# nrontsis/PILCO

Measured on AMD Instinct MI355X. Metric: moment-matching rollouts/sec (N=1000,D=10,E=10,H=40), higher is better.
Workload: dtype f64; 1 GPU; BASELINE configs[1]: N=1000 D=10 E=10 H=40 full rollout + reward, control_dim=0 (D==E read literally), ExponentialReward(W=I,t=0), factorisation cached (R-fwd); one step = one host-synchronised pilco_rollout call (what PILCO.predict makes) with its result downloaded; parallelism=pairs1, exchange=none (one rank)

## Files before the change

### include/pilco_hip_dev.h

```cpp
#ifndef PILCO_HIP_DEV_H
#define PILCO_HIP_DEV_H
#include "pilco_hip.h"

#ifdef __cplusplus
extern "C" {
#endif

int pilco_set_pair_kernel(pilco_ctx* ctx, int variant);
int pilco_set_fused_step(pilco_ctx* ctx, int on);
int pilco_set_small_step(pilco_ctx* ctx, int on);
int pilco_set_grad_mode(pilco_ctx* ctx, int mode);
int pilco_set_reverse_chain(pilco_ctx* ctx, int on_device);
int pilco_set_use_graph(pilco_ctx* ctx, int on);
int pilco_set_inline_policy(pilco_ctx* ctx, int on);

int pilco_rollout_tape(pilco_ctx* ctx, const pilco_policy* policy, const pilco_reward_term* rewards, int n_rewards,
                       const double* m0, const double* S0, int H, double* mH, double* SH, double* reward, double* traj,
                       double* tape);

int pilco_shard_owner_of_pair(const pilco_ctx* ctx, int pair_index);
int pilco_shard_plan(int E, int D, int nranks, int rank, int* out5);
int pilco_shard_pair_slot(int E, int D, int nranks, int a, int b);
int pilco_shard_output_slot(int E, int D, int nranks, int a);
int pilco_peer_attached(const pilco_ctx* ctx);
int pilco_comm_count(const pilco_ctx* ctx);

int pilco_rollout_timed(pilco_ctx* ctx, const pilco_policy* policy, const pilco_reward_term* rewards, int n_rewards,
                        const double* m0, const double* S0, int H, int reps, double* mH, double* SH, double* reward,
                        float* ms_total, float* ms_pair, int* n_pair_launches);
int pilco_set_pair_timing(pilco_ctx* ctx, int on);
int pilco_get_pair_timing(pilco_ctx* ctx, float* ms_pair, int* n_pair_launches);
int pilco_debug_timestamps(pilco_ctx* ctx, unsigned long long* out32);
int pilco_debug_last_route(const pilco_ctx* ctx, int* out, int n);
#define PILCO_GEOMETRY_WORDS 14
int pilco_debug_geometry(pilco_ctx* ctx, int* out, int n);
int pilco_debug_particle_actions(pilco_ctx* ctx, const pilco_policy* policy, const double* x, int P, double* u);
int pilco_debug_blocks(pilco_ctx* ctx, unsigned long long* out, int n);
int pilco_debug_buffer(pilco_ctx* ctx, int slot, int which, double* out, long n);
int pilco_debug_poison(pilco_ctx* ctx, int slot, int which);
int pilco_debug_sk_boundary(int w, int waves, int nd, int tdiag, int toff, int ud, int uo, int n_pairs);
int pilco_debug_sk_pair_waves(int k, int waves, int nd, int tdiag, int toff, int ud, int uo, int n_pairs, int* out3);
int pilco_factorize_timed(pilco_ctx* ctx, int slot, int reps, float* ms_each);

#ifdef __cplusplus
}
#endif
#endif
```

### pilco_amd/_lib.py

```python
from __future__ import annotations

import ctypes as C
import os

import numpy as np

_HERE = os.path.dirname(os.path.abspath(__file__))
LIB_PATH = os.environ.get("PILCO_LIB", os.path.join(_HERE, "libpilco_hip.so"))

PILCO_OK = 0
STATUS_NAMES = {1: "PILCO_E_SHAPE", 2: "PILCO_E_NOT_PD", 3: "PILCO_E_HIP", 4: "PILCO_E_RCCL",
                5: "PILCO_E_STATE", 6: "PILCO_E_ALLOC"}
SLOT_DYNAMICS, SLOT_POLICY = 0, 1
POLICY_NONE, POLICY_LINEAR, POLICY_RBF = 0, 1, 2
REWARD_EXPONENTIAL, REWARD_LINEAR = 1, 2
MAX_EVENTS, MAX_EVENT_CLAUSES = 8, 4
COMM_ID_BYTES = 128
PEER_HANDLE_BYTES = 64

_dp = C.POINTER(C.c_double)


class PilcoError(RuntimeError):
    def __init__(self, code, msg):
        super().__init__(f"{STATUS_NAMES.get(code, code)}: {msg}")
        self.code = code


class NotPositiveDefiniteError(PilcoError):
    """The reference raises tf.errors.InvalidArgumentError here (tests/test_cascade.py:22)."""


class PolicyStruct(C.Structure):
    _fields_ = [("kind", C.c_int), ("state_dim", C.c_int), ("control_dim", C.c_int),
                ("W", _dp), ("b", _dp), ("max_action", _dp), ("squash", C.c_int)]


class RewardTerm(C.Structure):
    _fields_ = [("kind", C.c_int), ("coef", C.c_double), ("W", _dp), ("t", _dp)]


class EventClause(C.Structure):
    _fields_ = [("dim", C.c_int), ("low", C.c_double), ("high", C.c_double)]


class Event(C.Structure):
    _fields_ = [("n_clauses", C.c_int), ("complement", C.c_int), ("clause", EventClause * MAX_EVENT_CLAUSES)]


def event_spec_of(ev):
    spec = ev.event_spec() if hasattr(ev, "event_spec") else ev
    if not isinstance(spec, dict) or "clauses" not in spec:
        raise TypeError("an event is a dict(clauses=[(dim, low, high), ...], complement=bool) or offers event_spec()")
    return spec


_vp = C.c_void_p
SEED_FN = C.CFUNCTYPE(None, C.c_void_p, C.c_int, C.c_int, C.POINTER(C.c_double), C.POINTER(C.c_double))
SIGNATURES = {
    "pilco_abi_version": (C.c_int, []),
    "pilco_ctx_create": (C.c_int, [C.c_int, C.POINTER(_vp)]),
    "pilco_ctx_destroy": (C.c_int, [_vp]),
    "pilco_last_error": (C.c_char_p, [_vp]),
    "pilco_last_not_pd_output": (C.c_int, [_vp]),
    "pilco_set_pair_kernel": (C.c_int, [_vp, C.c_int]),
    "pilco_set_reverse_chain": (C.c_int, [_vp, C.c_int]),
    "pilco_debug_poison": (C.c_int, [_vp, C.c_int, C.c_int]),
    "pilco_selftest": (C.c_int, [_vp]),
    "pilco_set_fused_step": (C.c_int, [_vp, C.c_int]),
    "pilco_set_grad_mode": (C.c_int, [_vp, C.c_int]),
    "pilco_set_small_step": (C.c_int, [_vp, C.c_int]),
    "pilco_set_use_graph": (C.c_int, [_vp, C.c_int]),
    "pilco_set_inline_policy": (C.c_int, [_vp, C.c_int]),
    "pilco_gp_set_data": (C.c_int, [_vp, C.c_int, _dp, _dp, C.c_int, C.c_int, C.c_int]),
    "pilco_gp_set_hyp": (C.c_int, [_vp, C.c_int, _dp, _dp, _dp]),
    "pilco_gp_set_inducing": (C.c_int, [_vp, C.c_int, _dp, C.c_int]),
    "pilco_gp_gram": (C.c_int, [_vp, C.c_int, _dp, C.c_int, _dp, C.c_int, _dp]),
    "pilco_gp_factorize": (C.c_int, [_vp, C.c_int]),
    "pilco_gp_nlml": (C.c_int, [_vp, C.c_int, _dp, _dp]),
    "pilco_gp_fitc_nlml": (C.c_int, [_vp, C.c_int, _dp, C.c_int, _dp, _dp, _dp]),
    "pilco_gp_num_points": (C.c_int, [_vp, C.c_int]),
    "pilco_gp_get_factors": (C.c_int, [_vp, C.c_int, _dp, _dp]),
    "pilco_gp_set_factors": (C.c_int, [_vp, C.c_int, _dp, _dp]),
    "pilco_gp_predict": (C.c_int, [_vp, C.c_int, _dp, _dp, _dp, _dp, _dp]),
    "pilco_gp_predict_points": (C.c_int, [_vp, C.c_int, _dp, C.c_int, C.c_int, _dp, _dp, _dp]),
    "pilco_gp_predict_points_jac": (C.c_int, [_vp, C.c_int, _dp, C.c_int, C.c_int, _dp, _dp, _dp, _dp, _dp]),
    "pilco_rollout": (C.c_int, [_vp, C.POINTER(PolicyStruct), C.POINTER(RewardTerm), C.c_int, _dp, _dp, C.c_int,
                                _dp, _dp, _dp, _dp]),
    "pilco_rollout_particles": (C.c_int, [_vp, C.POINTER(PolicyStruct), C.POINTER(RewardTerm), C.c_int, _dp, C.c_int, C.c_int,
                                          _dp, C.c_ulonglong, C.c_int, _dp, _dp, _dp, _dp, _dp]),
    "pilco_rollout_particles_events": (C.c_int, [_vp, C.POINTER(PolicyStruct), C.POINTER(RewardTerm), C.c_int, _dp, C.c_int, C.c_int,
                                                 _dp, C.c_ulonglong, C.c_int, _dp, _dp, _dp, _dp, _dp,
                                                 C.POINTER(Event), C.c_int, C.POINTER(C.c_longlong), C.POINTER(C.c_int)]),
    "pilco_gp_predict_vjp": (C.c_int, [_vp, C.c_int, _dp, _dp, _dp, _dp, _dp, _dp, _dp]),
    "pilco_rollout_tape": (C.c_int, [_vp, C.POINTER(PolicyStruct), C.POINTER(RewardTerm), C.c_int, _dp, _dp, C.c_int,
                                     _dp, _dp, _dp, _dp, _dp]),
    "pilco_rollout_grad": (C.c_int, [_vp, C.POINTER(PolicyStruct), C.POINTER(RewardTerm), C.c_int, _dp, _dp, C.c_int,
                                     _dp, _dp, _dp]),
    "pilco_rollout_grad_rbf": (C.c_int, [_vp, C.POINTER(PolicyStruct), C.POINTER(RewardTerm), C.c_int, _dp, _dp, C.c_int,
                                         _dp, _dp, _dp, _dp, C.c_int, _dp, _dp, _dp, _dp]),
    "pilco_rollout_grad_seeded": (C.c_int, [_vp, C.POINTER(PolicyStruct), C.POINTER(RewardTerm), C.c_int, _dp, _dp, C.c_int,
                                            SEED_FN, _vp, _dp, _dp, _dp]),
    "pilco_rollout_grad_rbf_seeded": (C.c_int, [_vp, C.POINTER(PolicyStruct), C.POINTER(RewardTerm), C.c_int, _dp, _dp, C.c_int,
                                                _dp, _dp, _dp, _dp, C.c_int, SEED_FN, _vp, _dp, _dp, _dp, _dp]),
    "pilco_propagate": (C.c_int, [_vp, C.POINTER(PolicyStruct), _dp, _dp, _dp, _dp]),
    "pilco_rollout_batch": (C.c_int, [_vp, C.c_int, C.POINTER(PolicyStruct), C.POINTER(RewardTerm), C.c_int, _dp, _dp, C.c_int, _dp, _dp, _dp]),
    "pilco_rollout_grad_batch": (C.c_int, [_vp, C.c_int, C.POINTER(PolicyStruct), C.POINTER(RewardTerm), C.c_int, _dp, _dp, C.c_int, _dp, _dp, _dp]),
    "pilco_rollout_grad_rbf_batch": (C.c_int, [_vp, C.c_int, C.POINTER(PolicyStruct), C.POINTER(RewardTerm), C.c_int, _dp, _dp, C.c_int,
                                               _dp, _dp, _dp, _dp, C.c_int, _dp, _dp, _dp, _dp]),
    "pilco_rollout_grad_batch_seeded": (C.c_int, [_vp, C.c_int, C.POINTER(PolicyStruct), C.POINTER(RewardTerm), C.c_int, _dp, _dp, C.c_int,
                                                  SEED_FN, C.POINTER(C.c_void_p), _dp, _dp, _dp]),
    "pilco_rollout_grad_rbf_batch_seeded": (C.c_int, [_vp, C.c_int, C.POINTER(PolicyStruct), C.POINTER(RewardTerm), C.c_int, _dp, _dp, C.c_int,
                                                      _dp, _dp, _dp, _dp, C.c_int, SEED_FN, C.POINTER(C.c_void_p), _dp, _dp, _dp, _dp]),
    "pilco_policy_action": (C.c_int, [_vp, C.POINTER(PolicyStruct), _dp, _dp, _dp, _dp, _dp]),
    "pilco_reward_eval": (C.c_int, [_vp, C.POINTER(RewardTerm), C.c_int, C.c_int, _dp, _dp, _dp, _dp]),
    "pilco_rollout_timed": (C.c_int, [_vp, C.POINTER(PolicyStruct), C.POINTER(RewardTerm), C.c_int, _dp, _dp,
                                      C.c_int, C.c_int, _dp, _dp, _dp, C.POINTER(C.c_float),
                                      C.POINTER(C.c_float), C.POINTER(C.c_int)]),
    "pilco_factorize_timed": (C.c_int, [_vp, C.c_int, C.c_int, C.POINTER(C.c_float)]),
    "pilco_set_pair_timing": (C.c_int, [_vp, C.c_int]),
    "pilco_get_pair_timing": (C.c_int, [_vp, C.POINTER(C.c_float), C.POINTER(C.c_int)]),
    "pilco_debug_timestamps": (C.c_int, [_vp, C.POINTER(C.c_ulonglong)]),
    "pilco_debug_blocks": (C.c_int, [_vp, C.POINTER(C.c_ulonglong), C.c_int]),
    "pilco_debug_last_route": (C.c_int, [_vp, C.POINTER(C.c_int), C.c_int]),
    "pilco_debug_geometry": (C.c_int, [_vp, C.POINTER(C.c_int), C.c_int]),
    "pilco_debug_particle_actions": (C.c_int, [_vp, C.POINTER(PolicyStruct), _dp, C.c_int, _dp]),
    "pilco_debug_buffer": (C.c_int, [_vp, C.c_int, C.c_int, _dp, C.c_long]),
    "pilco_debug_sk_boundary": (C.c_int, [C.c_int] * 8),
    "pilco_debug_sk_pair_waves": (C.c_int, [C.c_int] * 8 + [C.POINTER(C.c_int)]),
    "pilco_comm_unique_id": (C.c_int, [_vp]),
    "pilco_comm_init": (C.c_int, [_vp, _vp, C.c_int, C.c_int]),
    "pilco_shard_set": (C.c_int, [_vp, C.c_int, C.c_int]),
    "pilco_peer_export": (C.c_int, [_vp, _vp]),
    "pilco_peer_attach": (C.c_int, [_vp, _vp, C.c_int]),
    "pilco_group_peer_attach": (C.c_int, [_vp, C.c_int]),
    "pilco_peer_detach": (C.c_int, [_vp]),
    "pilco_peer_attached": (C.c_int, [_vp]),
    "pilco_shard_owner_of_pair": (C.c_int, [_vp, C.c_int]),
    "pilco_shard_plan": (C.c_int, [C.c_int, C.c_int, C.c_int, C.c_int, C.POINTER(C.c_int)]),
    "pilco_shard_pair_slot": (C.c_int, [C.c_int, C.c_int, C.c_int, C.c_int, C.c_int]),
    "pilco_shard_output_slot": (C.c_int, [C.c_int, C.c_int, C.c_int, C.c_int]),
    "pilco_gp_shard_pack": (C.c_int, [_vp, C.c_int, _dp, _dp, _dp]),
    "pilco_gp_shard_finish": (C.c_int, [_vp, C.c_int, _dp, _dp, _dp, _dp]),
    "pilco_rollout_grad_group": (C.c_int, [C.POINTER(_vp), C.c_int, C.POINTER(PolicyStruct), C.POINTER(RewardTerm), C.c_int, _dp, _dp, C.c_int, _dp, _dp, _dp]),
    "pilco_rollout_grad_rbf_group": (C.c_int, [C.POINTER(_vp), C.c_int, C.POINTER(PolicyStruct), C.POINTER(RewardTerm), C.c_int, _dp, _dp, C.c_int,
                                               _dp, _dp, _dp, _dp, C.c_int, _dp, _dp, _dp, _dp]),
    "pilco_rollout_group": (C.c_int, [C.POINTER(_vp), C.c_int, C.POINTER(PolicyStruct), C.POINTER(RewardTerm), C.c_int, _dp, _dp,
                            C.c_int, _dp, _dp, _dp, _dp, C.POINTER(C.c_int)]),
    "pilco_group_sync_model": (C.c_int, [C.POINTER(_vp), C.c_int, C.c_int]),
    "pilco_gp_beta_rows": (C.c_int, [_vp, C.c_int, C.POINTER(C.c_int), C.POINTER(C.c_int)]),
    "pilco_gp_beta_export": (C.c_int, [_vp, C.c_int, _dp]),
    "pilco_gp_beta_import": (C.c_int, [_vp, C.c_int, _dp]),
    "pilco_comm_rank": (C.c_int, [_vp]),
    "pilco_comm_size": (C.c_int, [_vp]),
    "pilco_comm_count": (C.c_int, [_vp]),
}

_lib = None


def load_library():
    global _lib
    if _lib is not None:
        return _lib
    if not os.path.exists(LIB_PATH):
        raise RuntimeError(
            f"{LIB_PATH} is missing: build the HIP extension first "
            "(python -c 'import __graft_entry__ as g; g.build()' or make -C pilco_amd/csrc). "
            "pilco_amd has no CPU fallback.")
    lib = C.CDLL(LIB_PATH)
    for name, (res, args) in SIGNATURES.items():
        fn = getattr(lib, name)
        fn.restype = res
        fn.argtypes = args
    _lib = lib
    return lib


def _f64(a, shape=None):
    a = np.ascontiguousarray(np.asarray(a, dtype=np.float64))
    if shape is not None:
        a = a.reshape(shape)
    return a


def _ptr(a):
    return a.ctypes.data_as(_dp) if a is not None else None


class Context:

    def __init__(self, device=None):
        self.lib = load_library()
        if device is None:
            device = int(os.environ.get("PILCO_DEVICE", os.environ.get("LOCAL_RANK", "0")))
        h = _vp()
        rc = self.lib.pilco_ctx_create(int(device), C.byref(h))
        if rc != PILCO_OK or not h:
            raise PilcoError(rc, f"cannot create a HIP context on device {device} "
                                 "(no MI355X visible?). pilco_amd has no CPU fallback.")
        self.h = h
        self.device = int(device)
        self._keep = []
        self._slot_owner = {}
        self._settings = {}
        self.nranks, self.has_comm = 1, False

    def close(self):
        if getattr(self, "h", None):
            self.lib.pilco_ctx_destroy(self.h)
            self.h = None

    def __del__(self):
        try:
            self.close()
        except Exception:
            pass

    def _chk(self, rc):
        if rc != PILCO_OK:
            msg = self.lib.pilco_last_error(self.h).decode("utf-8", "replace")
            if rc == 2:
                exc = NotPositiveDefiniteError(rc, msg)
                exc.output = int(self.lib.pilco_last_not_pd_output(self.h))
                raise exc
            raise PilcoError(rc, msg)

    def selftest(self):
        self._chk(self.lib.pilco_selftest(self.h))

    def set_fused_step(self, on):
        self._chk(self.lib.pilco_set_fused_step(self.h, 1 if on else 0))
        self._settings["set_fused_step"] = (on,)

    def set_small_step(self, on):
        self._chk(self.lib.pilco_set_small_step(self.h, 1 if on else 0))
        self._settings["set_small_step"] = (on,)

    def set_grad_mode(self, mode):
        self._chk(self.lib.pilco_set_grad_mode(self.h, int(mode)))
        self._settings["set_grad_mode"] = (mode,)

    def use_graph(self, on):
        self._chk(self.lib.pilco_set_use_graph(self.h, 1 if on else 0))
        self._settings["use_graph"] = (on,)

    def set_inline_policy(self, on):
        self._chk(self.lib.pilco_set_inline_policy(self.h, 1 if on else 0))
        self._settings["set_inline_policy"] = (on,)

    def debug_poison(self, slot, which):
        self._chk(self.lib.pilco_debug_poison(self.h, int(slot), int(which)))

    def set_reverse_chain(self, on_device):
        self._chk(self.lib.pilco_set_reverse_chain(self.h, int(bool(on_device))))
        self._settings["set_reverse_chain"] = (on_device,)

    def set_pair_kernel(self, variant):
        self._chk(self.lib.pilco_set_pair_kernel(self.h, int(variant)))
        self._settings["set_pair_kernel"] = (variant,)

    def gp_set_data(self, slot, X, Y, owner=None):
        self._slot_owner[slot] = owner
        X = _f64(X)
        Y = _f64(Y)
        if X.ndim != 2 or Y.ndim != 2 or X.shape[0] != Y.shape[0]:
            raise ValueError("data must be (X (N,D), Y (N,E))")
        self._chk(self.lib.pilco_gp_set_data(self.h, slot, _ptr(X), _ptr(Y), X.shape[0], X.shape[1], Y.shape[1]))

    def gp_set_hyp(self, slot, lengthscales, variance, noise, owner=None):
        self._slot_owner[slot] = owner
        ls, var, nz = _f64(lengthscales), _f64(variance).reshape(-1), _f64(noise).reshape(-1)
        self._chk(self.lib.pilco_gp_set_hyp(self.h, slot, _ptr(ls), _ptr(var), _ptr(nz)))

    def gp_set_inducing(self, slot, Z, owner=None):
        self._slot_owner[slot] = owner
        if Z is None:
            self._chk(self.lib.pilco_gp_set_inducing(self.h, slot, None, 0))
        else:
            Z = _f64(Z)
            self._chk(self.lib.pilco_gp_set_inducing(self.h, slot, _ptr(Z), Z.shape[0]))

    def gp_gram(self, slot, X1, X2, E):
        X1 = _f64(X1)
        X2a = None if X2 is None else _f64(X2)
        n2 = X1.shape[0] if X2a is None else X2a.shape[0]
        out = np.empty((E, X1.shape[0], n2))
        self._chk(self.lib.pilco_gp_gram(self.h, slot, _ptr(X1), X1.shape[0], _ptr(X2a), n2, _ptr(out)))
        return out

    def gp_factorize(self, slot):
        self._chk(self.lib.pilco_gp_factorize(self.h, slot))

    def gp_nlml(self, slot, D, E, want_grad=True):
        nlml = np.empty(E)
        grad = np.empty((E, D + 2)) if want_grad else None
        self._chk(self.lib.pilco_gp_nlml(self.h, slot, _ptr(nlml), _ptr(grad)))
        return nlml, grad

    def gp_fitc_nlml(self, slot, Z_all, D, E, want_grad=True):
        Z_all = _f64(Z_all)
        M = Z_all.shape[1]
        Z_all = _f64(Z_all, (E, M, D))
        nlml = np.empty(E)
        gh = np.empty((E, D + 2)) if want_grad else None
        gz = np.empty((E, M, D)) if want_grad else None
        self._chk(self.lib.pilco_gp_fitc_nlml(self.h, slot, _ptr(Z_all), M, _ptr(nlml), _ptr(gh), _ptr(gz)))
        return nlml, gh, gz

    def gp_num_points(self, slot):
        return self.lib.pilco_gp_num_points(self.h, slot)

    def gp_get_factors(self, slot, E, want_iK=True):
        n = self.gp_num_points(slot)
        iK = np.empty((E, n, n)) if want_iK else None
        beta = np.empty((E, n))
        self._chk(self.lib.pilco_gp_get_factors(self.h, slot, _ptr(iK), _ptr(beta)))
        return iK, beta

    def gp_set_factors(self, slot, iK, beta, owner=None):
        self._slot_owner[slot] = owner
        iKa = None if iK is None else _f64(iK)
        beta = _f64(beta)
        self._chk(self.lib.pilco_gp_set_factors(self.h, slot, _ptr(iKa), _ptr(beta)))

    def gp_predict(self, slot, m, s, D, E):
        m = _f64(m, (D,))
        s = _f64(s, (D, D))
        M = np.empty((1, E))
        S = np.empty((E, E))
        V = np.empty((D, E))
        self._chk(self.lib.pilco_gp_predict(self.h, slot, _ptr(m), _ptr(s), _ptr(M), _ptr(S), _ptr(V)))
        return M, S, V

    def gp_predict_points(self, slot, Xs, D, E, output=-1, Z_all=None):
        Xs = _f64(Xs)
        if Xs.ndim != 2 or Xs.shape[1] != D:
            raise ValueError(f"test inputs must be (Nt, {D})")
        Nt = Xs.shape[0]
        Za = None
        if Z_all is not None:
            Za = _f64(Z_all)
            Za = _f64(Za, (E, Za.shape[-2], D))
        rows = E if output < 0 else 1
        mean = np.empty((rows, Nt))
        var = np.empty((rows, Nt))
        self._chk(self.lib.pilco_gp_predict_points(self.h, slot, _ptr(Xs), Nt, int(output), _ptr(Za), _ptr(mean), _ptr(var)))
        return mean, var

    def gp_predict_points_jac(self, slot, Xs, D, E, output=-1, Z_all=None):
        Xs = _f64(Xs)
        if Xs.ndim != 2 or Xs.shape[1] != D:
            raise ValueError(f"test inputs must be (Nt, {D})")
        Nt = Xs.shape[0]
        Za = None
        if Z_all is not None:
            Za = _f64(Z_all)
            Za = _f64(Za, (E, Za.shape[-2], D))
        rows = E if output < 0 else 1
        mean, var = np.empty((rows, Nt)), np.empty((rows, Nt))
        dmean, dvar = np.empty((rows, Nt, D)), np.empty((rows, Nt, D))
        self._chk(self.lib.pilco_gp_predict_points_jac(self.h, slot, _ptr(Xs), Nt, int(output), _ptr(Za), _ptr(mean), _ptr(var),
                                                       _ptr(dmean), _ptr(dvar)))
        return mean, var, dmean, dvar

    def _policy(self, spec):
        keep = []
        p = PolicyStruct()
        p.kind = spec["kind"]
        p.state_dim = spec["state_dim"]
        p.control_dim = spec["control_dim"]
        p.squash = 1 if spec.get("squash", True) else 0
        U, E = p.control_dim, p.state_dim
        if spec["kind"] == POLICY_LINEAR:
            W = _f64(spec["W"], (U, E))
            b = _f64(spec["b"], (U,))
            keep += [W, b]
            p.W, p.b = _ptr(W), _ptr(b)
        ma = spec.get("max_action", None)
        if ma is not None and U > 0:
            ma = _f64(np.broadcast_to(np.asarray(ma, np.float64).reshape(-1) if np.ndim(ma) else np.float64(ma), (U,)))
            keep.append(ma)
            p.max_action = _ptr(ma)
        return p, keep

    def _rewards(self, terms, E):
        arr = (RewardTerm * max(len(terms), 1))()
        keep = []
        for i, t in enumerate(terms):
            arr[i].kind = t["kind"]
            arr[i].coef = float(t.get("coef", 1.0))
            if t["kind"] == REWARD_EXPONENTIAL:
                W = _f64(t["W"], (E, E))
                tg = _f64(t["t"], (E,)) if t.get("t") is not None else None
                keep += [W, tg]
                arr[i].W, arr[i].t = _ptr(W), _ptr(tg)
            else:
                W = _f64(t["W"], (E,))
                keep.append(W)
                arr[i].W = _ptr(W)
        return arr, keep

    def rollout(self, policy, rewards, m0, S0, H, want_traj=False):
        E = policy["state_dim"]
        p, k1 = self._policy(policy)
        r, k2 = self._rewards(rewards, E)
        m0 = _f64(m0, (E,))
        S0 = _f64(S0, (E, E))
        mH = np.empty((1, E))
        SH = np.empty((E, E))
        rew = np.zeros((1, 1))
        traj = np.empty((H + 1, E + E * E)) if want_traj else None
        self._chk(self.lib.pilco_rollout(self.h, C.byref(p), r, len(rewards), _ptr(m0), _ptr(S0), int(H),
                                         _ptr(mH), _ptr(SH), _ptr(rew), _ptr(traj)))
        if want_traj:
            return mH, SH, rew, traj
        return mH, SH, rew

    @staticmethod
    def _events(events):
        arr = (Event * max(len(events), 1))()
        for k, ev in enumerate(events):
            spec = event_spec_of(ev)
            clauses = list(spec["clauses"])
            if len(clauses) > MAX_EVENT_CLAUSES:
                raise ValueError(f"an event has at most {MAX_EVENT_CLAUSES} clauses")
            arr[k].n_clauses = len(clauses)
            arr[k].complement = 1 if spec.get("complement", False) else 0
            for j, (dim, low, high) in enumerate(clauses):
                arr[k].clause[j].dim = int(dim)
                arr[k].clause[j].low = -np.inf if low is None else float(low)
                arr[k].clause[j].high = np.inf if high is None else float(high)
        return arr

    def rollout_particles(self, policy, rewards, x0, H, eps=None, seed=0, observation_noise=False, want_particles=False,
                          events=None):
        E = policy["state_dim"]
        p, k1 = self._policy(policy)
        r, k2 = self._rewards(rewards, E)
        x0 = _f64(x0)
        if x0.ndim != 2 or x0.shape[1] != E:
            raise ValueError(f"initial particles must be (P, {E})")
        P, H = x0.shape[0], int(H)
        if eps is not None:
            eps = _f64(eps)
            if eps.shape != (H, P, E):
                raise ValueError(f"draws must be ({H}, {P}, {E})")
        mean = np.empty((H + 1, E))
        cov = np.empty((H + 1, E, E))
        rew = np.empty((max(H, 0),))
        parts = np.empty((H + 1, P, E)) if want_particles else None
        used = np.empty((H, P, E))
        args = (self.h, C.byref(p), r, len(rewards), _ptr(x0), P, H, _ptr(eps), C.c_ulonglong(int(seed) & 0xFFFFFFFFFFFFFFFF),
                1 if observation_noise else 0, _ptr(mean), _ptr(cov), _ptr(rew), _ptr(parts), _ptr(used))
        if events is None:
            self._chk(self.lib.pilco_rollout_particles(*args))
            return mean, cov, rew, parts, used
        events = list(events)
        K = len(events)
        ev = self._events(events)
        counts = np.zeros((H + 1, K), np.int64)
        first = np.full((P, K), -1, np.int32)
        self._chk(self.lib.pilco_rollout_particles_events(*args, ev, K, counts.ctypes.data_as(C.POINTER(C.c_longlong)),
                                                          first.ctypes.data_as(C.POINTER(C.c_int))))
        return mean, cov, rew, parts, used, counts, first

    def particle_actions(self, policy, x):
        E, U = policy["state_dim"], policy["control_dim"]
        p, k1 = self._policy(policy)
        x = _f64(x).reshape(-1, E)
        u = np.empty((x.shape[0], U))
        self._chk(self.lib.pilco_debug_particle_actions(self.h, C.byref(p), _ptr(x), x.shape[0], _ptr(u)))
        return u

    def rollout_batch(self, policies, rewards, m0, S0, H):
        B = len(policies)
        E = policies[0]["state_dim"]
        arr, keep = self._policy_array(policies)
        r, k2 = self._rewards(rewards, E)
        m0 = _f64(m0, (B, E))
        S0 = _f64(S0, (B, E, E))
        mH = np.empty((B, E))
        SH = np.empty((B, E, E))
        rew = np.zeros(B)
        self._chk(self.lib.pilco_rollout_batch(self.h, B, arr, r, len(rewards), _ptr(m0), _ptr(S0), int(H), _ptr(mH), _ptr(SH), _ptr(rew)))
        return mH, SH, rew

    def _policy_array(self, policies):
        arr = (PolicyStruct * len(policies))()
        keep = []
        for i, spec in enumerate(policies):
            p, k = self._policy(spec)
            keep.append((p, k))
            arr[i] = p
        return arr, keep

    @staticmethod
    def _lane_seed_callback(seed_fns, errors):
        def cb(user, H, E, traj_p, seeds_p):
            n = (H + 1) * (E + E * E)
            out = np.ctypeslib.as_array(seeds_p, shape=(n,))
            try:
                traj = np.ctypeslib.as_array(traj_p, shape=(n,)).reshape(H + 1, E + E * E).copy()
                out[:] = np.asarray(seed_fns[int(user) - 1](traj), dtype=np.float64).reshape(n)
            except BaseException as exc:
                errors.append(exc)
                out[:] = np.nan
        return SEED_FN(cb)

    lane_seeds = True

    def rollout_grad_batch(self, policies, rewards, m0, S0, H, seed_fns=None):
        B = len(policies)
        E, U = policies[0]["state_dim"], policies[0]["control_dim"]
        arr, keep = self._policy_array(policies)
        r, k2 = self._rewards(rewards, E)
        m0 = _f64(m0, (B, E)); S0 = _f64(S0, (B, E, E))
        rew = np.zeros(B); dW = np.empty((B, U, E)); db = np.empty((B, U))
        if seed_fns is None:
            self._chk(self.lib.pilco_rollout_grad_batch(self.h, B, arr, r, len(rewards), _ptr(m0), _ptr(S0), int(H), _ptr(rew), _ptr(dW), _ptr(db)))
            return rew, dW, db
        errors = []
        cb = self._lane_seed_callback(seed_fns, errors)
        users = (C.c_void_p * B)(*[i + 1 for i in range(B)])
        rc = self.lib.pilco_rollout_grad_batch_seeded(self.h, B, arr, r, len(rewards), _ptr(m0), _ptr(S0), int(H), cb, users,
                                                      _ptr(rew), _ptr(dW), _ptr(db))
        if errors:
            raise errors[0]
        self._chk(rc)
        return rew, dW, db

    def rollout_grad_rbf_batch(self, policies, rewards, m0, S0, H, Xp, Yp, lsp, noisep, seed_fns=None):
        B = len(policies)
        E, U = policies[0]["state_dim"], policies[0]["control_dim"]
        arr, keep = self._policy_array(policies)
        r, k2 = self._rewards(rewards, E)
        m0 = _f64(m0, (B, E)); S0 = _f64(S0, (B, E, E))
        Xp = _f64(Xp); bf = Xp.shape[1]
        Xp = _f64(Xp, (B, bf, E)); Yp = _f64(Yp, (B, bf, U)); lsp = _f64(lsp, (B, U, E)); noisep = _f64(noisep, (B, U))
        rew = np.zeros(B); dX = np.empty((B, bf, E)); dY = np.empty((B, bf, U)); dls = np.empty((B, U, E))
        self._slot_owner[SLOT_POLICY] = None
        if seed_fns is None:
            self._chk(self.lib.pilco_rollout_grad_rbf_batch(self.h, B, arr, r, len(rewards), _ptr(m0), _ptr(S0), int(H), _ptr(Xp), _ptr(Yp),
                                                            _ptr(lsp), _ptr(noisep), bf, _ptr(rew), _ptr(dX), _ptr(dY), _ptr(dls)))
            return rew, dX, dY, dls
        errors = []
        cb = self._lane_seed_callback(seed_fns, errors)
        users = (C.c_void_p * B)(*[i + 1 for i in range(B)])
        rc = self.lib.pilco_rollout_grad_rbf_batch_seeded(self.h, B, arr, r, len(rewards), _ptr(m0), _ptr(S0), int(H), _ptr(Xp), _ptr(Yp),
                                                          _ptr(lsp), _ptr(noisep), bf, cb, users, _ptr(rew), _ptr(dX), _ptr(dY), _ptr(dls))
        if errors:
            raise errors[0]
        self._chk(rc)
        return rew, dX, dY, dls

    def gp_predict_vjp(self, slot, m, s, Mbar, Sbar, Vbar, D, E):
        m = _f64(m, (D,)); s = _f64(s, (D, D))
        Mb = _f64(Mbar, (E,)); Sb = _f64(Sbar, (E, E)); Vb = _f64(Vbar, (D, E))
        mbar = np.empty((1, D)); sbar = np.empty((D, D))
        self._chk(self.lib.pilco_gp_predict_vjp(self.h, slot, _ptr(m), _ptr(s), _ptr(Mb), _ptr(Sb), _ptr(Vb), _ptr(mbar), _ptr(sbar)))
        return mbar, sbar

    def rollout_tape(self, policy, rewards, m0, S0, H):
        E = policy["state_dim"]; D = E + policy["control_dim"]
        p, k1 = self._policy(policy)
        r, k2 = self._rewards(rewards, E)
        m0 = _f64(m0, (E,)); S0 = _f64(S0, (E, E))
        mH = np.empty((1, E)); SH = np.empty((E, E)); rew = np.zeros((1, 1))
        traj = np.empty((H + 1, E + E * E))
        TS = D + D * D + E * D + E + E * E + D * E
        tape = np.zeros((max(H, 1), TS))
        self._chk(self.lib.pilco_rollout_tape(self.h, C.byref(p), r, len(rewards), _ptr(m0), _ptr(S0), int(H),
                                              _ptr(mH), _ptr(SH), _ptr(rew), _ptr(traj), _ptr(tape)))
        return mH, SH, rew, traj, tape[:H]

    @staticmethod
    def _seed_callback(seed_fn, errors):
        def cb(_user, H, E, traj_p, seeds_p):
            n = (H + 1) * (E + E * E)
            out = np.ctypeslib.as_array(seeds_p, shape=(n,))
            try:
                traj = np.ctypeslib.as_array(traj_p, shape=(n,)).reshape(H + 1, E + E * E).copy()
                out[:] = np.asarray(seed_fn(traj), dtype=np.float64).reshape(n)
            except BaseException as exc:
                errors.append(exc)
                out[:] = np.nan
        return SEED_FN(cb)

    def rollout_grad(self, policy, rewards, m0, S0, H, seed_fn=None):
        E = policy["state_dim"]; U = policy["control_dim"]
        p, k1 = self._policy(policy)
        r, k2 = self._rewards(rewards, E)
        m0 = _f64(m0, (E,)); S0 = _f64(S0, (E, E))
        rew = np.zeros((1, 1)); dW = np.empty((U, E)); db = np.empty((U,))
        errors = []
        cb = self._seed_callback(seed_fn, errors) if seed_fn is not None else SEED_FN()
        rc = self.lib.pilco_rollout_grad_seeded(self.h, C.byref(p), r, len(rewards), _ptr(m0), _ptr(S0), int(H), cb, None,
                                                _ptr(rew), _ptr(dW), _ptr(db))
        if errors:
            raise errors[0]
        self._chk(rc)
        return float(rew[0, 0]), dW, db

    def rollout_grad_rbf(self, policy, rewards, m0, S0, H, Xp, Yp, lsp, noisep, seed_fn=None):
        E = policy["state_dim"]; U = policy["control_dim"]
        p, k1 = self._policy(policy)
        r, k2 = self._rewards(rewards, E)
        m0 = _f64(m0, (E,)); S0 = _f64(S0, (E, E))
        Xp = _f64(Xp); bf = Xp.shape[0]
        Xp = _f64(Xp, (bf, E)); Yp = _f64(Yp, (bf, U)); lsp = _f64(lsp, (U, E)); noisep = _f64(noisep, (U,))
        rew = np.zeros((1, 1)); dX = np.empty((bf, E)); dY = np.empty((bf, U)); dls = np.empty((U, E))
        errors = []
        cb = self._seed_callback(seed_fn, errors) if seed_fn is not None else SEED_FN()
        rc = self.lib.pilco_rollout_grad_rbf_seeded(self.h, C.byref(p), r, len(rewards), _ptr(m0), _ptr(S0), int(H),
                                                    _ptr(Xp), _ptr(Yp), _ptr(lsp), _ptr(noisep), bf, cb, None,
                                                    _ptr(rew), _ptr(dX), _ptr(dY), _ptr(dls))
        if errors:
            raise errors[0]
        self._chk(rc)
        return float(rew[0, 0]), dX, dY, dls

    def propagate(self, policy, m_x, s_x):
        E = policy["state_dim"]
        p, k1 = self._policy(policy)
        m_x = _f64(m_x, (E,))
        s_x = _f64(s_x, (E, E))
        M = np.empty((1, E))
        S = np.empty((E, E))
        self._chk(self.lib.pilco_propagate(self.h, C.byref(p), _ptr(m_x), _ptr(s_x), _ptr(M), _ptr(S)))
        return M, S

    def policy_action(self, policy, m, s):
        E, U = policy["state_dim"], policy["control_dim"]
        p, k1 = self._policy(policy)
        m = _f64(m, (E,))
        s = _f64(s, (E, E))
        M = np.empty((1, U))
        S = np.empty((U, U))
        V = np.empty((E, U))
        self._chk(self.lib.pilco_policy_action(self.h, C.byref(p), _ptr(m), _ptr(s), _ptr(M), _ptr(S), _ptr(V)))
        return M, S, V

    def reward_eval(self, rewards, E, m, s):
        r, k2 = self._rewards(rewards, E)
        m = _f64(m, (E,))
        s = _f64(s, (E, E))
        mu = C.c_double()
        var = C.c_double()
        self._chk(self.lib.pilco_reward_eval(self.h, r, len(rewards), E, _ptr(m), _ptr(s), C.byref(mu), C.byref(var)))
        return np.array([[mu.value]]), np.array([[var.value]])

    def rollout_timed(self, policy, rewards, m0, S0, H, reps, time_pair=True):
        E = policy["state_dim"]
        p, k1 = self._policy(policy)
        r, k2 = self._rewards(rewards, E)
        m0 = _f64(m0, (E,))
        S0 = _f64(S0, (E, E))
        mH = np.empty((1, E))
        SH = np.empty((E, E))
        rew = np.zeros((1, 1))
        ms_total = C.c_float()
        ms_pair = C.c_float()
        npair = C.c_int()
        self._chk(self.lib.pilco_rollout_timed(self.h, C.byref(p), r, len(rewards), _ptr(m0), _ptr(S0), int(H),
                                               int(reps), _ptr(mH), _ptr(SH), _ptr(rew), C.byref(ms_total),
                                               C.byref(ms_pair) if time_pair else None, C.byref(npair)))
        return dict(mH=mH, SH=SH, reward=rew, ms_total=ms_total.value, ms_pair=ms_pair.value,
                    n_pair_launches=npair.value)

    def factorize_timed(self, slot, reps):
        ms = C.c_float()
        self._chk(self.lib.pilco_factorize_timed(self.h, slot, int(reps), C.byref(ms)))
        return ms.value

    def set_pair_timing(self, on=True):
        self._chk(self.lib.pilco_set_pair_timing(self.h, 1 if on else 0))

    def get_pair_timing(self):
        ms = C.c_float()
        n = C.c_int()
        self._chk(self.lib.pilco_get_pair_timing(self.h, C.byref(ms), C.byref(n)))
        return ms.value, n.value

    def debug_buffer(self, slot, which, n):
        out = np.empty(int(n))
        self._chk(self.lib.pilco_debug_buffer(self.h, int(slot), int(which), _ptr(out), int(n)))
        return out

    def debug_timestamps(self, read=True):
        buf = (C.c_ulonglong * 64)()
        self._chk(self.lib.pilco_debug_timestamps(self.h, buf if read else None))
        return list(buf)

    ROUTE_FIELDS = ("entry", "step", "policy", "DT", "KP", "vsep", "pair", "tape", "H", "npad", "chain", "rev_lds", "exchange")

    def last_route(self):
        buf = (C.c_int * len(self.ROUTE_FIELDS))()
        self._chk(self.lib.pilco_debug_last_route(self.h, buf, len(buf)))
        return {name: int(buf[i]) for i, name in enumerate(self.ROUTE_FIELDS)}

    GEOMETRY_FIELDS = ("npad", "PL", "EL", "NCH", "NCHM", "NT", "sk_waves", "sk_total", "sk_nd", "sk_maxw", "sk_capacity", "cus",
                       "NCS_reward", "NCS_no_reward")

    def geometry(self):
        buf = (C.c_int * len(self.GEOMETRY_FIELDS))()
        self._chk(self.lib.pilco_debug_geometry(self.h, buf, len(buf)))
        return {name: int(buf[i]) for i, name in enumerate(self.GEOMETRY_FIELDS)}

    def debug_blocks(self, n):
        buf = (C.c_ulonglong * n)()
        self._chk(self.lib.pilco_debug_blocks(self.h, buf, n))
        return list(buf)

    def comm_unique_id(self):
        buf = C.create_string_buffer(COMM_ID_BYTES)
        rc = self.lib.pilco_comm_unique_id(buf)
        if rc != PILCO_OK:
            raise PilcoError(rc, "ncclGetUniqueId failed")
        return bytes(buf.raw)

    def comm_init(self, id_bytes, rank, nranks):
        buf = C.create_string_buffer(bytes(id_bytes), COMM_ID_BYTES)
        self._chk(self.lib.pilco_comm_init(self.h, buf, int(rank), int(nranks)))
        self.nranks, self.has_comm = int(nranks), True

    def shard_pack(self, slot, m, s, D, E, nranks, rank):
        plan = shard_plan(E, D, nranks, rank)
        m = _f64(m, (D,))
        s = _f64(s, (D, D))
        seg = np.zeros(plan["SEG"])
        self._chk(self.lib.pilco_gp_shard_pack(self.h, slot, _ptr(m), _ptr(s), _ptr(seg)))
        return seg

    def shard_finish(self, slot, gathered, D, E):
        g = _f64(gathered).reshape(-1)
        M = np.empty((1, E))
        S = np.empty((E, E))
        V = np.empty((D, E))
        self._chk(self.lib.pilco_gp_shard_finish(self.h, slot, _ptr(g), _ptr(M), _ptr(S), _ptr(V)))
        return M, S, V

    def shard_set(self, rank, nranks):
        self._chk(self.lib.pilco_shard_set(self.h, int(rank), int(nranks)))
        self.nranks = int(nranks)

    def beta_export(self, slot=0):
        el, npad = C.c_int(0), C.c_int(0)
        self._chk(self.lib.pilco_gp_beta_rows(self.h, slot, C.byref(el), C.byref(npad)))
        rows = np.zeros((el.value, npad.value))
        self._chk(self.lib.pilco_gp_beta_export(self.h, slot, _ptr(rows)))
        return rows

    def beta_import(self, all_rows, slot=0):
        all_rows = np.ascontiguousarray(all_rows, dtype=np.float64)
        self._chk(self.lib.pilco_gp_beta_import(self.h, slot, _ptr(all_rows)))

    def peer_export(self):
        buf = C.create_string_buffer(PEER_HANDLE_BYTES)
        self._chk(self.lib.pilco_peer_export(self.h, buf))
        return bytes(buf.raw)

    def peer_attach(self, handles, share_gpu=False):
        blob = b"".join(bytes(h) for h in handles)
        buf = C.create_string_buffer(blob, len(blob))
        self._chk(self.lib.pilco_peer_attach(self.h, buf, 1 if share_gpu else 0))

    def comm_count(self):
        return int(self.lib.pilco_comm_count(self.h))

    def peer_detach(self):
        self._chk(self.lib.pilco_peer_detach(self.h))

    def peer_attached(self):
        return bool(self.lib.pilco_peer_attached(self.h))


def rollout_grad_group(ctxs, policy, rewards, m0, S0, H):
    c0 = ctxs[0]
    n = len(ctxs)
    E, U = policy["state_dim"], policy["control_dim"]
    p, k1 = c0._policy(policy)
    r, k2 = c0._rewards(rewards, E)
    m0 = _f64(m0, (E,)); S0 = _f64(S0, (E, E))
    arr = (_vp * n)(*[c.h for c in ctxs])
    rew, dW, db = np.zeros(n), np.empty((n, U, E)), np.empty((n, U))
    c0._chk(c0.lib.pilco_rollout_grad_group(arr, n, C.byref(p), r, len(rewards), _ptr(m0), _ptr(S0), int(H), _ptr(rew), _ptr(dW), _ptr(db)))
    return rew, dW, db


def rollout_grad_rbf_group(ctxs, policy, rewards, m0, S0, H, Xp, Yp, lsp, noisep):
    c0 = ctxs[0]
    n = len(ctxs)
    E, U = policy["state_dim"], policy["control_dim"]
    p, k1 = c0._policy(policy)
    r, k2 = c0._rewards(rewards, E)
    m0 = _f64(m0, (E,)); S0 = _f64(S0, (E, E))
    Xp = _f64(Xp); bf = Xp.shape[0]
    Xp = _f64(Xp, (bf, E)); Yp = _f64(Yp, (bf, U)); lsp = _f64(lsp, (U, E)); noisep = _f64(noisep, (U,))
    arr = (_vp * n)(*[c.h for c in ctxs])
    rew, dX, dY, dls = np.zeros(n), np.empty((n, bf, E)), np.empty((n, bf, U)), np.empty((n, U, E))
    c0._chk(c0.lib.pilco_rollout_grad_rbf_group(arr, n, C.byref(p), r, len(rewards), _ptr(m0), _ptr(S0), int(H), _ptr(Xp), _ptr(Yp), _ptr(lsp),
                                                _ptr(noisep), bf, _ptr(rew), _ptr(dX), _ptr(dY), _ptr(dls)))
    return rew, dX, dY, dls


def group_nlml(ctxs, slot, D, E):
    nlml, grad = np.full(E, np.nan), np.full((E, D + 2), np.nan)
    for c in ctxs:
        n, g = c.gp_nlml(slot, D, E)
        own = ~np.isnan(n)
        assert not np.any(own & ~np.isnan(nlml)), "two ranks claim the same output"
        nlml[own], grad[own] = n[own], g[own]
    return nlml, grad


def group_fitc_nlml(ctxs, slot, Z_all, D, E):
    Z_all = np.asarray(Z_all, np.float64)
    nlml, gh, gz = np.full(E, np.nan), np.full((E, D + 2), np.nan), np.full(Z_all.shape, np.nan)
    for c in ctxs:
        n, h, z = c.gp_fitc_nlml(slot, Z_all, D, E)
        own = ~np.isnan(n)
        assert not np.any(own & ~np.isnan(nlml)), "two ranks claim the same output"
        nlml[own], gh[own], gz[own] = n[own], h[own], z[own]
    return nlml, gh, gz


def group_sync_model(ctxs, slot=0):
    arr = (_vp * len(ctxs))(*[c.h for c in ctxs])
    ctxs[0]._chk(ctxs[0].lib.pilco_group_sync_model(arr, len(ctxs), int(slot)))


def group_peer_attach(ctxs):
    arr = (_vp * len(ctxs))(*[c.h for c in ctxs])
    ctxs[0]._chk(ctxs[0].lib.pilco_group_peer_attach(arr, len(ctxs)))


def rollout_group(ctxs, policy, rewards, m0, S0, H, want_traj=False):
    c0 = ctxs[0]
    E = policy["state_dim"]
    p, k1 = c0._policy(policy)
    r, k2 = c0._rewards(rewards, E)
    m0 = _f64(m0, (E,))
    S0 = _f64(S0, (E, E))
    mH, SH, rew = np.empty((1, E)), np.empty((E, E)), np.zeros((1, 1))
    traj = np.empty((H + 1, E + E * E)) if want_traj else None
    arr = (_vp * len(ctxs))(*[c.h for c in ctxs])
    mm = C.c_int(0)
    c0._chk(c0.lib.pilco_rollout_group(arr, len(ctxs), C.byref(p), r, len(rewards), _ptr(m0), _ptr(S0), int(H), _ptr(mH), _ptr(SH),
                                       _ptr(rew), _ptr(traj), C.byref(mm)))
    return (mH, SH, rew, traj, mm.value) if want_traj else (mH, SH, rew, mm.value)


def shard_plan(E, D, nranks, rank):
    lib = load_library()
    out = (C.c_int * 5)()
    rc = lib.pilco_shard_plan(int(E), int(D), int(nranks), int(rank), out)
    if rc != PILCO_OK:
        raise PilcoError(rc, "bad shard plan arguments")
    return dict(PL=out[0], EL=out[1], SEG=out[2], OUTOFF=out[3], P=out[4])


def shard_pair_slot(E, D, nranks, a, b):
    return load_library().pilco_shard_pair_slot(int(E), int(D), int(nranks), int(a), int(b))


def shard_output_slot(E, D, nranks, a):
    return load_library().pilco_shard_output_slot(int(E), int(D), int(nranks), int(a))


_default_ctx = None


def get_context():
    global _default_ctx
    if _default_ctx is None:
        _default_ctx = Context()
    return _default_ctx


def set_context(ctx):
    global _default_ctx
    _default_ctx = ctx
    _ctx_pool[:] = []


_ctx_pool = []


def resolve_ctx(obj):
    ref = getattr(obj, "_ctx_owner", None)
    owner = ref() if ref is not None else None
    return owner.ctx if owner is not None else get_context()


def context_adopted(ctx, owner):
    import weakref
    for ent in _ctx_pool:
        if ent[0] is ctx and (ent[1] is None or ent[1]() is None):
            ent[1] = weakref.ref(owner)


def context_for(owner):
    import weakref
    d = get_context()
    if os.environ.get("PILCO_CTX_POOL", "1") == "0":
        return d
    if getattr(d, "nranks", 1) != 1 or getattr(d, "has_comm", False):
        return d
    if not _ctx_pool or _ctx_pool[0][0] is not d:
        _ctx_pool[:] = [[d, None]]
    for ent in _ctx_pool:
        holder = ent[1]() if ent[1] is not None else None
        if holder is None or holder is owner:
            ent[1] = weakref.ref(owner)
            return ent[0]
    try:
        c = type(d)(device=getattr(d, "device", None))
    except TypeError:
        c = type(d)()
    for name, arg in getattr(d, "_settings", {}).items():
        getattr(c, name)(*arg)
    _ctx_pool.append([c, weakref.ref(owner)])
    return c
```

### pilco_amd/csrc/api.hip

```cpp
#include "ctx.h"

int fail(pilco_ctx* c, int code, const std::string& msg) {
    if (c) c->err = msg;
    return code;
}

int check_slot(pilco_ctx* ctx, int slot) {
    if (!ctx) return PILCO_E_SHAPE;
    if (slot < 0 || slot > 1) return fail(ctx, PILCO_E_SHAPE, "slot must be 0 (dynamics) or 1 (policy)");
    return PILCO_OK;
}

std::vector<int> deal_pairs(int E, int nranks) {
    const int P = E * (E + 1) / 2;
    std::vector<int> owner(P, 0);
    int k = 0;
    for (int a = 0; a < E; ++a) owner[a * (a + 1) / 2 + a] = (k++) % nranks;
    for (int a = 0; a < E; ++a)
        for (int b = 0; b < a; ++b) owner[a * (a + 1) / 2 + b] = (k++) % nranks;
    return owner;
}

int build_work(pilco_ctx* ctx, Slot& s) {
    if (s.wk_valid && s.wk_variant == ctx->variant) return PILCO_OK;
    const int E = s.E, D = s.D, npad = s.npad;
    const int P = E * (E + 1) / 2;
    const int W = ctx->nranks, rank = ctx->rank;
    s.pair_owner = deal_pairs(E, W);
    const int PLcap = (P + W - 1) / W, ELcap = (E + W - 1) / W;
    MMWork& wk = s.wk;
    wk.PL = (rank < P) ? (P - rank + W - 1) / W : 0;
    wk.EL = (rank < E) ? (E - rank + W - 1) / W : 0;
    wk.P = P;
    wk.KP = mm_kp(D);
    wk.vsep = mm_vsep(D) ? 1 : 0;
    mm_prep_chunks(npad, std::max(wk.PL, 1), wk.EL, &wk.NCH, &wk.NCHM);
    if (W > 1) {
        int nch_g;
        mm_prep_chunks(npad, P, E, &nch_g, &wk.NCHM);
        wk.NCHM = std::min(wk.NCHM, wk.NCH);
    }
    wk.NT = mm_pair_nt(npad, ctx->variant, std::max(wk.PL, 1));
    wk.OUTOFF = PLcap;
    wk.SEG = PLcap + ELcap * (1 + D);
    wk.rank = rank;
    wk.nranks = W;
#ifdef PILCO_DEV
    wk.abl = getenv("PILCO_ABL") ? atoi(getenv("PILCO_ABL")) : 0;
#else
    wk.abl = 0;
#endif
    const int PLa = std::max(wk.PL, 1);
    wk.sk_waves = 0;
    wk.sk_maxw = 0;
    wk.sk_pls = 0;
    if (ctx->variant == 0 && wk.PL > 0) {
        int tdiag, toff;
        mm_pair_sk_steps(npad, &tdiag, &toff);
        int nd = 0;
        const bool no_iK = s.iK_null || s.ignore_iK;
        if (!no_iK)
            for (int pl = 0; pl < wk.PL; ++pl)
                if (pl * W + rank < E) ++nd;
        if (no_iK) tdiag = toff;
        const long T = (long)nd * tdiag + (long)(wk.PL - nd) * toff;
        auto cut = [&](int cap) { return (long)cap > T ? (int)std::max<long>(4, (T + 3) / 4 * 4) : cap; };
        int waves = cut(mm_pair_sk_capacity(wk.KP, wk.vsep != 0, true));
        int ud = 5, uo = 4;
        if (const char* env = getenv("PILCO_SK_UNITS")) {
            int a = 0, b = 0;
            if (sscanf(env, "%d,%d", &a, &b) == 2 && a > 0 && b > 0) { ud = a; uo = b; }
        }
        if (mm_sk_max_pairs(waves, nd, tdiag, toff, wk.PL, ud, uo) > 2) {
            waves = cut(mm_pair_sk_capacity(wk.KP, wk.vsep != 0, false));
            ud = 5;
            uo = 4;
            if (mm_sk_max_pairs(waves, nd, tdiag, toff, wk.PL, ud, uo) > 2) waves = (int)std::max<long>(4, (T + 3) / 4 * 4);
        }
        wk.sk_waves = waves;
        wk.sk_total = (int)T;
        wk.sk_nd = nd;
        wk.sk_tdiag = tdiag;
        wk.sk_toff = toff;
        wk.sk_ud = ud;
        wk.sk_uo = uo;
        wk.sk_maxw = mm_sk_maxw(wk);
        wk.sk_pls = round_up(wk.PL, 16);
    }
    ENSURE(s.w_in, (size_t)D + D * D + E + E * E + D * E);
    const size_t wt_blocks = npad <= 256 ? (size_t)std::max(E, PLa) : (size_t)E;
    ENSURE(s.w_At, (size_t)PLa * wk.KP * npad);
    ENSURE(s.w_Wt, (wt_blocks * wk.KP + PLa) * npad);
    const size_t n_small = (size_t)PLa + (size_t)E * wk.NCHM * (1 + D);
    ENSURE(s.w_small, 2 * n_small);
    ENSURE(s.w_part, std::max((size_t)PLa * wk.NT * 2, (size_t)std::max(wk.sk_pls, 16) * std::max(wk.sk_maxw, 4)));
    ENSURE(s.w_fpart, (size_t)2 * PLa * wk.NCH * 4 * 2);
    wk.fuse_pair = 0;
    wk.wt_R = wt_rows_per_pair_of(E, D, wk.PL);
    wk.wt_deal = (wk.wt_R <= mm_prep_dt(D) && npad / wk.NCH <= 256) ? 1 : 0;
    wk.NCS = 1;
    wk.share_cu = 0;
    ENSURE(s.w_gath, (size_t)W * wk.SEG);
    ENSURE(s.w_out, (size_t)E + E * E + D * E);
    wk.in_m = s.w_in.p;
    wk.in_s = s.w_in.p + D;
    wk.At = s.w_At.p;
    wk.Wt = s.w_Wt.p;
    wk.vcol = wk.Wt + wt_blocks * wk.KP * npad;
    HIPCHK(hipMemsetAsync(wk.At, 0, sizeof(double) * (size_t)PLa * wk.KP * npad, ctx->st));
    HIPCHK(hipMemsetAsync(wk.Wt, 0, sizeof(double) * (wt_blocks * wk.KP + PLa) * npad, ctx->st));
    launch_const_rows(ctx->st, wk.vsep ? nullptr : wk.At + (size_t)(D + 1) * npad, PLa, wk.Wt + (size_t)D * npad, (int)wt_blocks, (long)wk.KP * npad, npad,
                      s.n);
    wk.pair_isdet = s.w_small.p;
    wk.mean_part = wk.pair_isdet + PLa;
    s.alt_isdet = s.w_small.p + n_small;
    s.alt_mean = s.alt_isdet + PLa;
    wk.pair_part = s.w_part.p;
    wk.sk_part = s.w_part.p;
    wk.gath = s.w_gath.p;
    wk.out_M = s.w_out.p;
    wk.out_S = wk.out_M + E;
    wk.out_V = wk.out_S + E * E;
    wk.exp_tab = ctx->exp_tab.p;
    wk.dbg = ctx->dbg;
    HIPCHK(hipMemsetAsync(s.w_gath.p, 0, sizeof(double) * W * wk.SEG, ctx->st));
    if (wk.sk_waves > 0) HIPCHK(hipMemsetAsync(s.w_part.p, 0, sizeof(double) * wk.sk_pls * wk.sk_maxw, ctx->st));
    s.wk_valid = true;
    s.wk_variant = ctx->variant;
    return PILCO_OK;
}

MMModel model_of(const Slot& s) {
    MMModel md{};
    md.Pt = s.M > 0 ? s.Zt.p : s.Xt.p;
    md.ls = s.ls.p;
    md.var = s.var.p;
    md.lvar = s.var.p + s.E;
    md.beta = s.beta.p;
    md.iK = (s.iK_null || s.ignore_iK) ? nullptr : s.iK.p;
    md.bW = s.shW > 0 ? s.shW : 1;
    md.bEL = s.shW > 1 ? s.shEL : s.E;
    md.n = s.n;
    md.npad = s.npad;
    md.D = s.D;
    md.E = s.E;
    return md;
}

static int group_exchange(pilco_ctx* ctx, Slot& s) {
    PeerGroup& grp = *ctx->group;
    const int slot_idx = (int)(&s - &ctx->slot[0]);
    HIPCHK(hipStreamSynchronize(ctx->st));
    if (!grp.arrive_and_wait()) return fail(ctx, PILCO_E_STATE, "group exchange: another member failed");
    const size_t seg = (size_t)s.wk.SEG;
    for (int j = 0; j < (int)grp.ctxs.size(); ++j) {
        if (j == ctx->rank) continue;
        const double* src = grp.ctxs[j]->slot[slot_idx].wk.gath + (size_t)j * seg;
        HIPCHK(hipMemcpyAsync(s.wk.gath + (size_t)j * seg, src, sizeof(double) * seg, hipMemcpyDefault, ctx->st));
    }
    HIPCHK(hipStreamSynchronize(ctx->st));
    if (!grp.arrive_and_wait()) return fail(ctx, PILCO_E_STATE, "group exchange: another member failed");
    return PILCO_OK;
}

int all_gather_segments(pilco_ctx* ctx, Slot& s) {
    if (ctx->nranks == 1 && !ctx->comm) return PILCO_OK;
    if (ctx->group) return group_exchange(ctx, s);
    if (!ctx->comm) return fail(ctx, PILCO_E_STATE, "sharded context without communicator: use pilco_gp_shard_pack / pilco_gp_shard_finish");
    double* base = s.wk.gath;
    ncclResult_t r = ncclAllGather(base + (size_t)ctx->rank * s.wk.SEG, base, s.wk.SEG, ncclDouble, ctx->comm, ctx->st);
    if (r != ncclSuccess) return fail(ctx, PILCO_E_RCCL, std::string("ncclAllGather: ") + ncclGetErrorString(r));
    return PILCO_OK;
}

int prepare_own(pilco_ctx* ctx, Slot& s, OwnView& o) {
    o.W = ctx->nranks;
    o.rank = ctx->rank;
    if (&s == &ctx->slot[PILCO_SLOT_POLICY]) {
        o.W = 1;
        o.rank = 0;
    }
    const int E = s.E, D = s.D, Np = s.Npad;
    o.ELcap = (E + o.W - 1) / o.W;
    o.EL = (o.rank < E) ? (E - o.rank + o.W - 1) / o.W : 0;
    if (o.W == 1) {
        o.ls = s.ls.p; o.var = s.var.p; o.noise = s.noise.p; o.Yt = s.Yt.p;
        return PILCO_OK;
    }
    const int ELa = std::max(o.EL, 1);
    ENSURE(s.own, (size_t)ELa * (D + 2) + (size_t)ELa * Np);
    double* pls = s.own.p;
    double* pvar = pls + (size_t)ELa * D;
    double* pnz = pvar + ELa;
    double* pY = pnz + ELa;
    if (o.EL > 0) {
        hipStream_t st = ctx->st;
        HIPCHK(hipMemcpy2DAsync(pls, sizeof(double) * D, s.ls.p + (size_t)o.rank * D, sizeof(double) * D * o.W, sizeof(double) * D, o.EL, hipMemcpyDeviceToDevice, st));
        HIPCHK(hipMemcpy2DAsync(pvar, sizeof(double), s.var.p + o.rank, sizeof(double) * o.W, sizeof(double), o.EL, hipMemcpyDeviceToDevice, st));
        HIPCHK(hipMemcpy2DAsync(pnz, sizeof(double), s.noise.p + o.rank, sizeof(double) * o.W, sizeof(double), o.EL, hipMemcpyDeviceToDevice, st));
        HIPCHK(hipMemcpy2DAsync(pY, sizeof(double) * Np, s.Yt.p + (size_t)o.rank * Np, sizeof(double) * Np * o.W, sizeof(double) * Np, o.EL, hipMemcpyDeviceToDevice, st));
    }
    o.ls = pls; o.var = pvar; o.noise = pnz; o.Yt = pY;
    return PILCO_OK;
}

static int gather_beta(pilco_ctx* ctx, Slot& s, const OwnView& o, int npad) {
    s.shW = o.W; s.shEL = o.ELcap; s.shOwn = o.EL; s.shRank = o.rank;
    s.beta_complete = true;
    if (o.W == 1) return PILCO_OK;
    if (ctx->comm) {
        const size_t blk = (size_t)o.ELcap * npad;
        ncclResult_t r = ncclAllGather(s.beta.p + (size_t)o.rank * blk, s.beta.p, blk, ncclDouble, ctx->comm, ctx->st);
        if (r != ncclSuccess) return fail(ctx, PILCO_E_RCCL, std::string("ncclAllGather(beta): ") + ncclGetErrorString(r));
        HIPCHK(hipStreamSynchronize(ctx->st));
        return PILCO_OK;
    }
    s.beta_complete = false;
    return PILCO_OK;
}

int agree_not_pd(pilco_ctx* ctx, int W, int bad, int* agreed) {
    *agreed = bad;
    if (W <= 1 || !ctx->comm) return PILCO_OK;
    int* d = ctx->d_info + 64;
    const int mine = bad + 1;
    HIPCHK(hipMemcpyAsync(d, &mine, sizeof(int), hipMemcpyHostToDevice, ctx->st));
    ncclResult_t r = ncclAllReduce(d, d + 1, 1, ncclInt, ncclMax, ctx->comm, ctx->st);
    if (r != ncclSuccess) return fail(ctx, PILCO_E_RCCL, std::string("ncclAllReduce(not positive definite): ") + ncclGetErrorString(r));
    int all = 0;
    HIPCHK(hipMemcpyAsync(&all, d + 1, sizeof(int), hipMemcpyDeviceToHost, ctx->st));
    HIPCHK(hipStreamSynchronize(ctx->st));
    *agreed = all - 1;
    return PILCO_OK;
}

int factorize_exact(pilco_ctx* ctx, Slot& s) {
    OwnView o{};
    if (int r = prepare_own(ctx, s, o)) return r;
    const int EL = o.EL, ELa = std::max(EL, 1), npad = s.Npad;
    const size_t mat = (size_t)npad * npad;
    ENSURE(s.K, ELa * mat);
    ENSURE(s.Linv, ELa * mat);
    ENSURE(s.iK, ELa * mat);
    ENSURE(s.beta, (size_t)o.W * o.ELcap * npad);
    ENSURE(s.vec, (size_t)ELa * npad);
    hipStream_t st = ctx->st;
    double* beta_own = s.beta.p + (size_t)o.rank * o.ELcap * npad;
    const std::vector<unsigned long long> key = {(unsigned long long)(uintptr_t)s.K.p, (unsigned long long)(uintptr_t)s.Linv.p,
        (unsigned long long)(uintptr_t)s.iK.p, (unsigned long long)(uintptr_t)s.beta.p,
        (unsigned long long)(uintptr_t)s.vec.p, (unsigned long long)(uintptr_t)s.Xt.p, (unsigned long long)(uintptr_t)o.ls,
        (unsigned long long)(uintptr_t)o.var, (unsigned long long)(uintptr_t)o.noise, (unsigned long long)(uintptr_t)o.Yt,
        (unsigned long long)(uintptr_t)ctx->d_info, (unsigned long long)npad, (unsigned long long)s.N, (unsigned long long)s.D,
        (unsigned long long)EL, (unsigned long long)o.W, (unsigned long long)o.rank, (unsigned long long)o.ELcap};
    auto chain = [&]() -> int {
    HIPCHK(hipMemsetAsync(ctx->d_info, 0, sizeof(int) * 64, st));
    if (o.W > 1) HIPCHK(hipMemsetAsync(s.beta.p, 0, sizeof(double) * (size_t)o.W * o.ELcap * npad, st));
    if (EL > 0) {
        launch_gram(st, s.Xt.p, npad, s.N, s.Xt.p, npad, s.N, s.D, o.ls, o.var, EL, s.K.p, npad, npad, 1, o.noise, 0.0);
        launch_potrf(st, s.K.p, npad, EL, s.Linv.p, ctx->d_info, false);
        launch_trtri(st, s.K.p, npad, EL, s.Linv.p, s.iK.p, (long)mat);
        GemmDesc g{};
        g.A = s.Linv.p; g.lda = npad; g.sA = (long)mat;
        g.B = s.Linv.p; g.ldb = npad; g.sB = (long)mat;
        g.C = s.iK.p; g.ldc = npad; g.sC = (long)mat;
        g.M = npad; g.N = npad; g.K = npad; g.alpha = 1.0; g.beta = 0.0; g.k_mode = 1;
        g.tile_mode = 2;
        launch_gemm(st, g, true, false, EL);
        launch_clear_padding(st, s.iK.p, npad, s.N, EL);
        launch_matvec(st, s.Linv.p, npad, EL, o.Yt, s.vec.p, false);
        launch_matvec(st, s.Linv.p, npad, EL, s.vec.p, beta_own, true);
    }
    return PILCO_OK;
    };
    if (int r = run_chain_graph(ctx, s.g_fact, key, chain)) return r;
    int info[64];
    HIPCHK(hipMemcpyAsync(info, ctx->d_info, sizeof(int) * std::min(ELa, 64), hipMemcpyDeviceToHost, st));
    HIPCHK(hipStreamSynchronize(st));
    int bad = -1, pivot = 0, agreed = -1;
    for (int al = 0; al < std::min(EL, 64) && bad < 0; ++al)
        if (info[al] != 0) bad = al * o.W + o.rank, pivot = info[al];
    if (int r = agree_not_pd(ctx, o.W, bad, &agreed)) return r;
    if (agreed >= 0) {
        ctx->not_pd = agreed;
        return fail(ctx, PILCO_E_NOT_PD, "Cholesky failed: K + noise*I of output " + std::to_string(agreed) + " is not positive definite" +
                                             (agreed == bad ? " (pivot " + std::to_string(pivot) + ")" : std::string(" (on another rank)")));
    }
    s.n = s.N;
    s.npad = npad;
    s.iK_null = false;
    return gather_beta(ctx, s, o, npad);
}


extern "C" {

int pilco_abi_version(void) { return PILCO_HIP_ABI_VERSION; }

int pilco_ctx_create(int device, pilco_ctx** out) {
    if (!out) return PILCO_E_SHAPE;
    *out = nullptr;
    int count = 0;
    if (hipGetDeviceCount(&count) != hipSuccess || count <= 0) return PILCO_E_HIP;
    if (device < 0 || device >= count) return PILCO_E_SHAPE;
    if (hipSetDevice(device) != hipSuccess) return PILCO_E_HIP;
    pilco_ctx* ctx = new pilco_ctx();
    ctx->device = device;
    ctx->slot[PILCO_SLOT_POLICY].ignore_iK = true;
    if (hipStreamCreateWithFlags(&ctx->st, hipStreamNonBlocking) != hipSuccess ||
        hipMalloc(&ctx->d_info, 72 * sizeof(int)) != hipSuccess || hipEventCreate(&ctx->ev0) != hipSuccess ||
        hipEventCreate(&ctx->ev1) != hipSuccess) {
        delete ctx;
        return PILCO_E_HIP;
    }
    {
        const int tn = mm_exp_table_size();
        std::vector<double> tab(tn);
        mm_exp_table_fill(tab.data());
        if (ctx->exp_tab.ensure(tn) != hipSuccess ||
            hipMemcpy(ctx->exp_tab.p, tab.data(), sizeof(double) * tn, hipMemcpyHostToDevice) != hipSuccess) {
            delete ctx;
            return PILCO_E_HIP;
        }
    }
    if (const char* eg = getenv("PILCO_NO_GRAPH")) ctx->use_graph = (atoi(eg) == 0);
    if (const char* ei = getenv("PILCO_INLINE_POLICY")) ctx->inline_policy = (atoi(ei) != 0);
    if (const char* ef = getenv("PILCO_FUSED")) ctx->fused = (atoi(ef) != 0);
    if (const char* ef = getenv("PILCO_SMALL_STEP")) ctx->fuse_small = (atoi(ef) != 0);
    if (const char* ef = getenv("PILCO_HOST_CHAIN")) ctx->dev_chain = (atoi(ef) == 0);
    if (const char* env = getenv("PILCO_PAIR_KERNEL")) {
        ctx->variant = (atoi(env) >= 0 && atoi(env) <= 2) ? atoi(env) : 0;
#ifndef PILCO_DEV
        if (ctx->variant == 1) ctx->variant = 0;
#endif
        ctx->variant_user = true;
    }
    *out = ctx;
    return PILCO_OK;
}

int pilco_ctx_destroy(pilco_ctx* ctx) {
    if (!ctx) return PILCO_OK;
    for (pilco_ctx* lane : ctx->lanes) (void)pilco_ctx_destroy(lane);
    ctx->lanes.clear();
    (void)hipSetDevice(ctx->device);
    (void)hipStreamSynchronize(ctx->st);
    (void)peer_detach(ctx);
    for (auto& ge : ctx->graph_cache) (void)hipGraphExecDestroy(ge.second);
    for (Slot& sl : ctx->slot)
        for (ChainGraph* cg : {&sl.g_fact, &sl.g_fitc, &sl.g_fitc_nlml}) chain_graph_release(*cg);
    if (ctx->comm) ncclCommDestroy(ctx->comm);
    for (Slot& s : ctx->slot) {
        predict_release(s);
        for (DevBuf* b : {&s.Xt, &s.Yt, &s.Zt, &s.ls, &s.var, &s.noise, &s.K, &s.Linv, &s.iK, &s.beta, &s.Tscr, &s.ksplit_ws,
                          &s.vec, &s.Kmn, &s.V2, &s.bwd_mom, &s.bwd_cp, &s.bwd_part, &s.bwd_out, &s.bwd_cnt, &s.jac_rowmom, &s.jac_cpart, &s.jac_head, &s.jac_part, &s.jac_np, &s.own, &s.Am, &s.AmInv, &s.iAt, &s.G, &s.w_in, &s.w_At, &s.w_Wt, &s.w_small, &s.w_fpart,
                          &s.w_part, &s.w_gath, &s.w_out, &s.ft_P, &s.ft_T3, &s.ft_Z})
            b->release();
    }
    ctx->state.release();
    ctx->params.release();
    ctx->traj.release();
    ctx->tape.release();
    ctx->jrec.release();
    ctx->jgath.release();
    ctx->revloc.release();
    ctx->revseeds.release();
    ctx->revmat.release();
    ctx->selftest.release();
    ctx->exp_tab.release();
    for (hipEvent_t e : ctx->pair_events) (void)hipEventDestroy(e);
    if (ctx->ev0) (void)hipEventDestroy(ctx->ev0);
    if (ctx->ev1) (void)hipEventDestroy(ctx->ev1);
    if (ctx->d_info) (void)hipFree(ctx->d_info);
    if (ctx->pin) (void)hipHostFree(ctx->pin);
    if (ctx->pin_io) (void)hipHostFree(ctx->pin_io);
    if (ctx->jpin) (void)hipHostFree(ctx->jpin);
    for (hipEvent_t e : ctx->jwait_ev)
        if (e) (void)hipEventDestroy(e);
    if (ctx->st) (void)hipStreamDestroy(ctx->st);
    delete ctx;
    return PILCO_OK;
}

const char* pilco_last_error(const pilco_ctx* ctx) { return ctx ? ctx->err.c_str() : "null context"; }
int pilco_last_not_pd_output(const pilco_ctx* ctx) { return ctx ? ctx->not_pd : -1; }

int pilco_set_pair_kernel(pilco_ctx* ctx, int variant) {
    if (!ctx || variant < 0 || variant > 2) return PILCO_E_SHAPE;
#ifndef PILCO_DEV
// ... 610 lines not shown
```

### pilco_amd/csrc/ctx.h

```cpp
#pragma once
#include <rccl/rccl.h>

#include <algorithm>
#include <array>
#include <chrono>
#include <condition_variable>
#include <memory>
#include <mutex>
#include <cmath>
#include <cstdint>

#include "grad_layout.h"
#include "moment.h"

using namespace pilco;

struct ChainGraph {
    std::vector<unsigned long long> key;
    hipGraphExec_t exec = nullptr;
    bool failed = false;
};

struct PredictWork;

enum RouteWord {
    ROUTE_ENTRY = 0,
    ROUTE_STEP = 1,
    ROUTE_POLICY = 2,
    ROUTE_DT = 3,
    ROUTE_KP = 4,
    ROUTE_VSEP = 5,
    ROUTE_PAIR = 6,
    ROUTE_TAPE = 7,
    ROUTE_H = 8,
    ROUTE_NPAD = 9,
    ROUTE_CHAIN = 10,
    ROUTE_REV_LDS = 11,
    ROUTE_EXCHANGE = 12,
    PILCO_ROUTE_WORDS = 13,
};
enum StepKind { STEP_NONE = 0, STEP_FUSED = 1, STEP_SMALL = 2, STEP_THREE = 3, STEP_FUSED_RBF = 4, STEP_PEER = 5 };

struct Slot {
    ChainGraph g_fact, g_fitc, g_fitc_nlml;
    int N = 0, D = 0, E = 0, M = 0;
    int Npad = 0;
    int n = 0, npad = 0;
    bool has_data = false, has_hyp = false, factor_valid = false, user_factors = false, iK_null = false;
    bool ignore_iK = false;
    DevBuf bwd_mom, bwd_cp, bwd_part, bwd_out, bwd_cnt;
    DevBuf jac_rowmom, jac_cpart, jac_head, jac_part, jac_np;
    DevBuf Xt, Yt, Zt, ls, var, noise;
    DevBuf K, Linv, iK, beta, Tscr, vec;
    DevBuf ksplit_ws;
    DevBuf Kmn, V2, Am, AmInv, iAt, G;
    DevBuf ft_P, ft_T3, ft_Z;
    long Zstride = 0;
    PredictWork* pred = nullptr;
    DevBuf own;
    int shW = 1, shEL = 0, shOwn = 0, shRank = 0;
    bool beta_complete = true;
    DevBuf w_in, w_At, w_Wt, w_small, w_part, w_gath, w_out;
    DevBuf w_fpart;
    MMWork wk{};
    double* alt_isdet = nullptr;
    double* alt_mean = nullptr;
    bool wk_valid = false;
    int wk_variant = -1;
    std::vector<int> pair_owner;
};


struct PeerGroup {
    std::vector<struct pilco_ctx*> ctxs;
    std::mutex mu;
    std::condition_variable cv;
    int waiting = 0;
    unsigned long generation = 0;
    bool failed = false;
    int first_failed = -1;
    bool arrive_and_wait() {
        std::unique_lock<std::mutex> lk(mu);
        if (failed) return false;
        const unsigned long gen = generation;
        if (++waiting == (int)ctxs.size()) {
            waiting = 0;
            ++generation;
            cv.notify_all();
            return true;
        }
        cv.wait(lk, [&] { return generation != gen || failed; });
        return !failed;
    }
    void fail_all(int rank) {
        std::lock_guard<std::mutex> lk(mu);
        if (!failed) first_failed = rank;
        failed = true;
        cv.notify_all();
    }
};

struct PeerXch {
    int W = 0, cap = 0;
    unsigned long long* local = nullptr;
    std::vector<unsigned long long*> mapped;
    std::vector<char> opened;
    unsigned long long** d_peers = nullptr;
    unsigned long long epoch = 0;
    unsigned long long* pin = nullptr;
    unsigned ring = 0;
    bool ready = false, wait_kernel = false;
    std::shared_ptr<std::vector<struct pilco_ctx*>> members;
};

constexpr int PILCO_DBG_WORDS = 16384;
struct pilco_ctx {
    int device = 0;
    hipStream_t st = nullptr;
    std::string err;
    int not_pd = -1;
    int variant = 0;
    bool variant_user = false;
    int rank = 0, nranks = 1;
    ncclComm_t comm = nullptr;
    std::shared_ptr<PeerGroup> group;
    PeerXch xq;
    Slot slot[2];
    int* d_info = nullptr;
    DevBuf state;
    DevBuf params;
    DevBuf traj;
    DevBuf tape;
    DevBuf jrec;
    DevBuf jgath;
    DevBuf revloc, revseeds, revmat;
    bool dev_chain = true;
    double* jpin = nullptr;
    size_t jpin_cap = 0;
    hipEvent_t jwait_ev[8] = {nullptr, nullptr, nullptr, nullptr, nullptr, nullptr, nullptr, nullptr};
    DevBuf selftest;
    DevBuf exp_tab;
    unsigned long long* dbg = nullptr;
    hipGraphExec_t graph = nullptr;
    std::vector<unsigned long long> graph_key;
    std::vector<std::pair<std::vector<unsigned long long>, hipGraphExec_t>> graph_cache;
    bool use_graph = true;
    std::array<int, PILCO_ROUTE_WORDS> route{};
    bool inline_policy = true;
    bool fused = true;
    bool fuse_small = true;
    bool graph_rccl_failed = false;
    int grad_mode = 1;
    hipEvent_t ev0 = nullptr, ev1 = nullptr;
    std::vector<hipEvent_t> pair_events;
    bool time_pairs = false;
    int timed_pairs = 0;
    double* pin = nullptr;
    size_t pin_cap = 0;
    double* pin_io = nullptr;
    size_t pin_io_cap = 0;
    const double* params_dev = nullptr;
    std::vector<double> params_host;
    std::vector<pilco_ctx*> lanes;
    bool is_lane = false;
    int share_cu = 0;
};

int fail(pilco_ctx* c, int code, const std::string& msg);
int agree_not_pd(pilco_ctx* ctx, int W, int bad, int* agreed);

#define HIPCHK(call)                                                                                       \
    do {                                                                                                   \
        hipError_t e_ = (call);                                                                            \
        if (e_ != hipSuccess)                                                                              \
            return fail(ctx, PILCO_E_HIP, std::string(#call) + ": " + hipGetErrorString(e_));              \
    } while (0)

#define ENSURE(buf, count)                                                                                 \
    do {                                                                                                   \
        if ((buf).ensure(count) != hipSuccess) return fail(ctx, PILCO_E_ALLOC, "hipMalloc failed: " #buf); \
    } while (0)

inline void chain_graph_release(ChainGraph& cg) {
    if (cg.exec) (void)hipGraphExecDestroy(cg.exec);
    cg.exec = nullptr;
    cg.key.clear();
}
inline void chain_graph_note() {
    static bool said = false;
    if (!said) fprintf(stderr, "libpilco_hip: a launch chain could not be captured as a hipGraph; it stays on eager launches\n");
    said = true;
}
template <class F>
int run_chain_graph(pilco_ctx* ctx, ChainGraph& cg, const std::vector<unsigned long long>& key, F&& enqueue) {
    if (!ctx->use_graph || ctx->dbg || cg.failed) return enqueue();
    if (cg.exec && cg.key == key) {
        HIPCHK(hipGraphLaunch(cg.exec, ctx->st));
        return PILCO_OK;
    }
    chain_graph_release(cg);
    if (int r = enqueue()) return r;
    hipGraph_t graph = nullptr;
    if (hipStreamBeginCapture(ctx->st, hipStreamCaptureModeThreadLocal) != hipSuccess) {
        (void)hipGetLastError();
        cg.failed = true;
        chain_graph_note();
        return PILCO_OK;
    }
    const int rc = enqueue();
    const hipError_t e = hipStreamEndCapture(ctx->st, &graph);
    if (rc != PILCO_OK || e != hipSuccess || !graph || hipGraphInstantiate(&cg.exec, graph, nullptr, nullptr, 0) != hipSuccess) {
        (void)hipGetLastError();
        cg.exec = nullptr;
        cg.failed = true;
        chain_graph_note();
    } else {
        cg.key = key;
    }
    if (graph) (void)hipGraphDestroy(graph);
    return PILCO_OK;
}

struct OwnView {
    int W, rank, EL, ELcap;
    const double *ls, *var, *noise, *Yt;
};
int prepare_own(pilco_ctx* ctx, Slot& s, OwnView& o);
int check_slot(pilco_ctx* ctx, int slot);
int build_work(pilco_ctx* ctx, Slot& s);
MMModel model_of(const Slot& s);
int all_gather_segments(pilco_ctx* ctx, Slot& s);
int pilco_factorize_fitc(pilco_ctx* ctx, void* slot_ptr);
void predict_release(Slot& s);

struct StepRoute {
    int step = STEP_NONE;
    int policy = 0;
    int pair = -1;
    int ncs = 0;
    bool timed = false;
};
struct RolloutPlan {
    GlueArgs g{};
    double* st[2] = {nullptr, nullptr};
    double* s1b[2] = {nullptr, nullptr};
    int E = 0, D = 0, U = 0;
    double* jrec = nullptr;
    size_t jstride = 0;
    StepRoute route;
};
int rollout_run(pilco_ctx* ctx, RolloutPlan& plan, int H, const double* m0, const double* S0);
enum GradChain {
    GRAD_CHAIN_DEVICE,
    GRAD_CHAIN_RECORDS,
    GRAD_CHAIN_ADJOINT,
};
enum GradExchange { GRAD_XCH_NONE, GRAD_XCH_COMM, GRAD_XCH_GROUP };
struct GradRoute {
    GradChain chain = GRAD_CHAIN_RECORDS;
    GradExchange exchange = GRAD_XCH_NONE;
    bool seeds = false;
    int rev_lds = 0;
};
struct GradCall {
    GradRoute route;
    RolloutPlan plan;
    int H = 0;
    double *traj = nullptr, *tape = nullptr, *jrec = nullptr, *reward = nullptr;
    size_t JS = 0;
    std::vector<double> traj_v, tape_v;
    bool arrived = false;
    int wait_t0[8] = {0, 0, 0, 0, 0, 0, 0, 0}, wait_n = 0, wait_next = 0, wait_from = 0;
    RevArgs ra{};
    size_t n_seeds = 0;
    double* h_seeds = nullptr;
    const double* h_out = nullptr;
    std::chrono::steady_clock::time_point tm0, tm1;
};
int plan_grad(pilco_ctx* ctx, const pilco_policy* policy, const pilco_reward_term* rewards, int n_rewards, int H, bool linear, bool seeds,
              const GradRoute* decided, GradCall& gc);
int grad_forward(pilco_ctx* ctx, const pilco_policy* policy, const pilco_reward_term* rewards, int n_rewards, const double* m0, const double* S0,
                 double* reward, bool defer, GradCall& gc);
int grad_arrive(pilco_ctx* ctx, GradCall& gc, double* reward);
int grad_wait(pilco_ctx* ctx, GradCall& gc, int t);
int grad_device_finish(pilco_ctx* ctx, GradCall& gc, pilco_seed_fn seed_fn, void* seed_user, double* reward, double* dW, double* db);
void grad_route_record(pilco_ctx* ctx, const GradRoute& route);
int rollout_lanes(pilco_ctx* ctx, int B, std::vector<pilco_ctx*>& lane, const char* who);
void rollout_lanes_done(pilco_ctx* ctx);
struct LanesGuard {
    pilco_ctx* c;
    ~LanesGuard() { rollout_lanes_done(c); }
};
template <class Begin, class Finish>
int run_lanes(pilco_ctx* ctx, const std::vector<pilco_ctx*>& lane, bool drain, Begin&& begin, Finish&& finish) {
    const int B = (int)lane.size();
    int err = PILCO_OK, begun = 0;
    auto note = [&](int i, int r) {
        if (!r || err) return;
        err = r;
        if (i > 0) ctx->err = "lane " + std::to_string(i) + ": " + lane[i]->err;
    };
    for (; begun < B; ++begun) {
        note(begun, begin(begun));
        if (err) break;
    }
    for (int i = 0; i < begun; ++i) note(i, finish(i));
    if (err && drain)
        for (pilco_ctx* l : lane) (void)hipStreamSynchronize(l->st);
    return err;
}
int setup_rollout(pilco_ctx* ctx, const pilco_policy* pol, const pilco_reward_term* rw, int n_rw, int H, bool want_traj,
                  RolloutPlan& plan);
void launch_peer_wait(hipStream_t st, unsigned long long* area, int k, int W, int spin);
int peer_detach(pilco_ctx* ctx);
```

### pilco_amd/csrc/glue.hip

```cpp
#include "glue_device.h"

namespace pilco {

size_t glue_lds_doubles_for(const GlueArgs& g) {
    double* const base = reinterpret_cast<double*>(uintptr_t{1} << 20);
    GlueLds L;
    glue_lds_carve(g, base, L);
    return (size_t)(L.pol - base) + (((g.flags & GF_POLICY) && g.pol_inline) ? (size_t)g.pol_lds : 0);
}
size_t glue_lds_bytes(int E, int D) {
    GlueArgs g{};
    g.E = E;
    g.D = D;
    return sizeof(double) * glue_lds_doubles_for(g);
}

int rbf_inline_lds_doubles(int E, int U, int bf) { return link_rbf_inline_lds_doubles(E, U, bf); }

__global__ __launch_bounds__(256) void k_const_rows(double* a_row, int nA, double* b_row, int nB, long bs, int npad, int n) {
    const int i = blockIdx.x * 256 + threadIdx.x, blk = blockIdx.y;
    if (i >= npad) return;
    const double v = i < n ? 1.0 : 0.0;
    if (a_row && blk < nA) a_row[(long)blk * bs + i] = v;
    if (blk < nB) b_row[(long)blk * bs + i] = v;
}
void launch_const_rows(hipStream_t st, double* a_row, int nA, double* b_row, int nB, long bs, int npad, int n) {
    const int nb = nA > nB ? nA : nB;
    if (nb <= 0) return;
    hipLaunchKernelGGL(k_const_rows, dim3((npad + 255) / 256, nb), dim3(256), 0, st, a_row, nA, b_row, nB, bs, npad, n);
}

__global__ __launch_bounds__(256) void k_glue(GlueArgs g) {
    extern __shared__ __attribute__((aligned(16))) double sm[];
    kernarg_warm<(int)sizeof(GlueArgs) + 64>();
    const int E = g.E, t = threadIdx.x;
    GlueLds L;
    glue_lds_carve(g, sm, L);
    if (blockIdx.x == 1) {
        DBG_STAMP(g.wk, 20, t == 0);
        double* ws = L.seg;
        const LoadSeg sg[2] = {{0, g.m_x, E}, {L.o_sx, g.s_x, E * E}};
        multi_load<2, 4>(L.mx, sg);
        __syncthreads();
        double mu, var;
        reward_eval(g.n_rewards, g.rw, E, L.mx, L.sx, ws, g.rew_out != nullptr, mu, var);
        if (t == 0) {
            if (g.rew_out) {
                g.rew_out[0] = mu;
                g.rew_out[1] = var;
            } else {
                g.reward[0] += mu;
            }
        }
        DBG_STAMP(g.wk, 21, t == 0);
        return;
    }
    glue_body(g, L, true);
}

__global__ void k_stamp(unsigned long long* dbg, int slot) {
    if (threadIdx.x == 0) dbg[slot] = wall_clock64();
}
void launch_stamp(hipStream_t st, unsigned long long* dbg, int slot) {
    hipLaunchKernelGGL(k_stamp, dim3(1), dim3(64), 0, st, dbg, slot);
}

void launch_glue(hipStream_t st, const GlueArgs& g, bool with_reward_block) {
    launch_lds<k_glue>(dim3(with_reward_block ? 2 : 1), dim3(256), sizeof(double) * glue_lds_doubles_for(g), st, g);
}

}
```

### pilco_amd/csrc/moment.h

```cpp
#pragma once
#include "common.h"

namespace pilco {

constexpr int MAX_REWARD_TERMS = 4;
#ifdef PILCO_DEV
#define MM_ABL(wk_, bit_) (((wk_).abl & (bit_)) != 0)
#else
#define MM_ABL(wk_, bit_) false
#endif
constexpr int MAX_D = 32;

struct MMModel {
    const double* Pt;
    const double* ls;
    const double* var;
    const double* lvar;
    const double* beta;
    const double* iK;
    int n, npad, D, E;
    int bW, bEL;
};

struct MMWork {
    double* in_m;
    double* in_s;
    double* At;
    double* Wt;
    double* vcol;
    int vsep;
    int wt_R, wt_deal;
    double* pair_isdet;
    double* mean_part;
    double* pair_part;
    double* gath;
    double* out_M;
    double* out_S;
    double* out_V;
    double* sk_part;
    int sk_waves, sk_total, sk_nd, sk_tdiag, sk_toff, sk_maxw;
    int sk_pls;
    unsigned long long* dbg;
    int abl;
    int sk_ud, sk_uo;
    int fuse_pair;
    double* sw_gpart;
    int share_cu;
    int NCS;
    const double* exp_tab;
    int PL, EL, P, KP, NCH, NCHM, NT, SEG, OUTOFF, rank, nranks;
};

struct RewardDev {
    int kind;
    double coef;
    const double* W;
    const double* t;
    const double* F;
    int rank;
};

struct PrepReward {
    int n;
    int E;
    RewardDev rw[MAX_REWARD_TERMS];
    const double* m_x;
    const double* s_x;
    double* reward;
};

enum GlueFlags {
    GF_PACK = 1,
    GF_ASSEMBLE = 2,
    GF_PROPAGATE = 4,
    GF_TRAJ = 8,
    GF_POLICY = 32,
    GF_RBF_POST = 64,
    GF_RBF_PRE = 128
};

struct GlueArgs {
    int flags;
    int E;
    int D;
    int U;
    MMWork wk;
    const double* var;
    MMWork pwk;
    const double* pvar;
    const double* m_x;
    const double* s_x;
    double* m_out;
    double* s_out;
    double* s1;
    double* s1_out;
    double* reward;
    double* traj;
    double* tape;
    int step;
    int dbg_off;
    MMModel pmd;
    int pol_inline;
    int pol_lds;
    int pol_kind;
    const double* W;
    const double* b;
    const double* maxact;
    int squash;
    int n_rewards;
    RewardDev rw[MAX_REWARD_TERMS];
    double* act_out;
    double* rew_out;
    unsigned long long* xq;
    unsigned long long** xq_peers;
    int xq_k;
    int xq_W;
    int xq_cap;
    int xq_spin;
};

__host__ __device__ inline int xq_data_off(int W) { return (8 + 2 * W + 7) & ~7; }
__host__ __device__ inline size_t xq_area_words(int W, int cap) { return (size_t)xq_data_off(W) + (size_t)2 * W * cap; }

bool mm_fused_head_fits(const MMModel& md, int reward_E, const GlueArgs& ga);
void launch_mm_prep(hipStream_t st, const MMModel& md, const MMWork& wk, const PrepReward* pr = nullptr,
                    const GlueArgs* fused = nullptr);
size_t glue_lds_doubles_for(const GlueArgs& g);
int rbf_inline_lds_doubles(int state_dim, int control_dim, int bf);
void launch_mm_pair(hipStream_t st, const MMModel& md, const MMWork& wk, int variant);
int mm_pair_sk_capacity(int KP, bool vsep, bool allow_env = true);
void mm_pair_sk_steps(int npad, int* tdiag, int* toff);
int mm_sk_boundary(int w, int waves, int nd_steps, int total, int ud, int uo);
int mm_sk_maxw(const MMWork& wk);
int mm_sk_max_pairs(int waves, int nd, int tdiag, int toff, int n_pairs, int ud, int uo);
void mm_sk_pair_waves(int k, int waves, int nd, int tdiag, int toff, int total, int ud, int uo, int* wlo, int* fslot, int* whi);
void launch_glue(hipStream_t st, const GlueArgs& g, bool with_reward_block = false);
size_t glue_lds_bytes(int E, int D);
int mm_pair_nt(int npad, int variant, int PL);
void mm_prep_chunks(int npad, int PL, int EL, int* nch, int* nchm);
inline int wt_rows_per_pair_of(int E, int D, int PL) { return (E * D + (PL > 1 ? PL : 1) - 1) / (PL > 1 ? PL : 1); }
int mm_prep_dt(int D);
__host__ __device__ constexpr bool mm_vsep(int D) { return (D + 2) % 4 == 1; }
__host__ __device__ constexpr int mm_kp(int D) { return mm_vsep(D) ? D + 1 : (D + 2 + 3) / 4 * 4; }
void launch_stamp(hipStream_t st, unsigned long long* dbg, int slot);
void launch_const_rows(hipStream_t st, double* a_row, int nA, double* b_row, int nB, long bs, int npad, int n);
void launch_mm_bwd(hipStream_t st, const MMModel& md, const MMWork& wk, double* rowmom, double* cpart, double* part,
                   const double* bars, double* head, double* out, unsigned* done, double* sum_out);
void mm_bwd_geometry(int npad, int Pg, int* njs, int* nrb);
void mm_bwd_split(int npad, int Pg, int kp, int* njs, int* nrb);
void launch_mm_sweep(hipStream_t st, const MMModel& md, const MMWork& wk, double* rowmom, double* cpart, double* head,
                     double* npart);
void launch_mm_jac_finish(hipStream_t st, const MMModel& md, const MMWork& wk, int H, const double* rowmom, const double* cpart,
                          double* head, double* part, const double* tape, size_t tape_stride, double* jrec, int small_nch = 0,
                          const struct RevLocalArgs* rl = nullptr);
size_t mm_jac_rec_size(int D, int E, int P);
size_t mm_jac_part_size(int D, int E, int P, int npad);
size_t mm_jac_rowmom_size(int npad, int P);
size_t mm_bwd_gpart_size(int npad, int P, int D);
size_t mm_bwd_cpart_size(int npad, int P);
size_t mm_jac_cpart_size(int npad, int P, int E);
size_t mm_jac_head_size(int D, int E, int P);
int mm_jac_nt(int npad, int Pg, int kp);
int mm_jac_ns(int D);
int mm_bwd_rc(int npad);
struct RevRewards {
    RewardDev rw[MAX_REWARD_TERMS];
};
struct RevLocalArgs {
    int n, E, U;
    RevRewards rs;
    const double *traj, *Wp, *bp, *maxact;
    double* loc;
};
struct RevArgs {
    int E, U, D, H, P;
    const double* jrec;
    int W;
    long gblk, gstep, out_off;
    const double* traj;
    const double* tape;
    long TS;
    const double* loc;
    const double* seeds;
    const double* Wp;
    const double* reward_dev;
    double* amat;
    double* out;
};
bool rev_chain_supported(int E, int U, int D);
size_t rev_step_lds_bytes(int E, int U, int D);
size_t rev_loc_doubles(int E, int U);
RevLocalArgs rev_local_args(int n, const RewardDev* rw, int E, int U, const double* traj, const double* Wp, const double* bp, const double* maxact,
                            double* loc);
void launch_rev_chain(hipStream_t st, const RevArgs& a);
int mm_exp_table_size();
void mm_exp_table_fill(double* tab);
int launch_selftest_mfma(hipStream_t st, double* dbuf, double* hbuf, const double* exp_tab);

}
```

### pilco_amd/csrc/pair.hip

```cpp
#include "pair_device.h"

namespace pilco {

template <int KC, bool VSEP>
__global__ __launch_bounds__(256, PAIR_MINW) void k_mm_pair_tiled(MMModel md, MMWork wk, int NJB) {
    __shared__ double red[4];
    __shared__ double tab[FEXP_TN];
    kernarg_warm<(int)(sizeof(MMModel) + sizeof(MMWork)) + 8 + 64>();
    for (int e = threadIdx.x; e < FEXP_TN; e += blockDim.x) tab[e] = wk.exp_tab[e];
    __syncthreads();
    const int npad = md.npad;
    const int lane = threadIdx.x & 63, w = threadIdx.x >> 6;
    const int jb = blockIdx.x % NJB, ti = blockIdx.x / NJB, pl = blockIdx.y;
    int a, b;
    local_pair_ab(wk, md.E, pl, a, b);
    const bool diag = (a == b) && (md.iK != nullptr);
    const PairOps po = pair_ops(wk, md.D, npad, pl, b);
    const double* beta_a = md.beta + mm_beta_row(md, a) * npad;
    const double* beta_b = md.beta + mm_beta_row(md, b) * npad;
    const int i0 = ti * 16 * PAIR_RT;
    const int JB = npad / NJB, JW = JB / 4;
    const int jbeg = jb * JB + w * JW;
    double t1;
    if (diag)
        t1 = pair_wave<KC, true, VSEP>(po, nullptr, nullptr, nullptr, beta_a, beta_b, md.iK + mm_ik_blk(md, a) * npad * npad, tab, npad, i0, jbeg, jbeg + JW, lane);
    else
        t1 = pair_wave<KC, false, VSEP>(po, nullptr, nullptr, nullptr, beta_a, beta_b, nullptr, tab, npad, i0, jbeg, jbeg + JW, lane);
    for (int off = 32; off > 0; off >>= 1) t1 += __shfl_down(t1, off);
    if (lane == 0) red[w] = t1;
    __syncthreads();
    if (threadIdx.x == 0) {
        double* out = wk.pair_part + ((long)pl * wk.NT + ti * NJB + jb) * 2;
        out[0] = (red[0] + red[1]) + (red[2] + red[3]);
        out[1] = 0.0;
    }
}

int mm_sk_maxw(const MMWork& wk) {
    int m = 4;
    for (int k = 0; k < wk.PL; ++k) {
        int wlo, fs, whi;
        sk_pair_waves(k, wk.sk_waves, wk.sk_nd, wk.sk_tdiag, wk.sk_toff, wk.sk_total, wk.sk_ud, wk.sk_uo, wlo, fs, whi);
        m = std::max(m, whi - wlo + 1);
    }
    return (m + 3) / 4 * 4;
}
int mm_sk_boundary(int w, int waves, int nd_steps, int total, int ud, int uo) {
    return sk_boundary_of(w, waves, nd_steps, total, ud, uo);
}
int mm_sk_max_pairs(int waves, int nd, int tdiag, int toff, int n_pairs, int ud, int uo) {
    return sk_max_pairs_per_wave(waves, nd, tdiag, toff, n_pairs, ud, uo);
}
void mm_sk_pair_waves(int k, int waves, int nd, int tdiag, int toff, int total, int ud, int uo, int* wlo, int* fslot, int* whi) {
    sk_pair_waves(k, waves, nd, tdiag, toff, total, ud, uo, *wlo, *fslot, *whi);
}

template <int KC, bool VSEP>
__global__ __launch_bounds__(256, (KC <= 4 && PAIR_MINW < 3) ? 3 : PAIR_MINW) void k_mm_pair_sk(MMModel md, MMWork wk) {
    __shared__ double tab[FEXP_TN];
    kernarg_warm<(int)(sizeof(MMModel) + sizeof(MMWork)) + 64>();
    TabArrival ta;
    ta.request(wk.exp_tab, tab);
    const int lane = threadIdx.x & 63;
    int bpos = blockIdx.x;
    if ((gridDim.x & 7) == 0) bpos = (blockIdx.x & 7) * (gridDim.x >> 3) + (blockIdx.x >> 3);
    const int w = __builtin_amdgcn_readfirstlane(bpos * 4 + (threadIdx.x >> 6));
#ifdef PAIR_WAVE_TRACE
    if (wk.dbg && lane == 0) {
        unsigned hw, xcc;
        asm volatile("s_getreg_b32 %0, hwreg(HW_REG_HW_ID)" : "=s"(hw));
        asm volatile("s_getreg_b32 %0, hwreg(HW_REG_XCC_ID)" : "=s"(xcc));
        wk.dbg[4096 + w] = wall_clock64();
        wk.dbg[4096 + 2 * 3072 + w] = ((unsigned long long)xcc << 32) | hw;
    }
#endif
    DBG_STAMP(wk, 16, w == 0 && lane == 0);
    if (wk.dbg && w == 0 && lane == 0) wk.dbg[32] = clock64();
    const int nd_steps = wk.sk_nd * wk.sk_tdiag;
    double out0, out1;
    int p0, p1;
    sk_wave_range<KC, VSEP>(md, wk, tab, w, lane, out0, out1, p0, p1, &ta, PAIR_FAIR != 0);
    ta.land();
    for (int off = 32; off > 0; off >>= 1) {
        out0 += __shfl_down(out0, off);
        out1 += __shfl_down(out1, off);
    }
    if (lane == 0) {
        if (p0 >= 0) {
            const long S0 = (p0 < wk.sk_nd) ? (long)p0 * wk.sk_tdiag : (long)wk.sk_nd * wk.sk_tdiag + (long)(p0 - wk.sk_nd) * wk.sk_toff;
            const int wlo = sk_wave_of(S0, wk.sk_waves, nd_steps, wk.sk_total, wk.sk_ud, wk.sk_uo);
            wk.sk_part[(long)(w - wlo) * wk.sk_pls + p0] = out0;
        }
        if (p1 >= 0) wk.sk_part[p1] = out1;
    }
    DBG_STAMP(wk, 17, w == 0 && lane == 0);
    if (wk.dbg && w == 0 && lane == 0) wk.dbg[33] = clock64();
    DBG_STAMP(wk, 18, w == wk.sk_waves - 1 && lane == 0);
    if (wk.dbg && lane == 0 && (w & 7) == 0) wk.dbg[1024 + (w >> 3)] = wall_clock64();
#ifdef PAIR_WAVE_TRACE
    if (wk.dbg && lane == 0) wk.dbg[4096 + 3072 + w] = wall_clock64();
#endif
}


#ifdef PILCO_DEV
template <int KPT>
__global__ __launch_bounds__(256) void k_mm_pair_valu(MMModel md, MMWork wk) {
    __shared__ double Bs[KPT][64];
    __shared__ double bbs[64];
    __shared__ double vs[64];
    __shared__ double red[8];
    const int npad = md.npad;
    const int t = threadIdx.x, lane = t & 63, w = t >> 6;
    const int ncb = npad / 64;
    const int tj = blockIdx.x % ncb, ti = blockIdx.x / ncb, pl = blockIdx.y;
    int a, b;
    local_pair_ab(wk, md.E, pl, a, b);
    const bool diag = (a == b) && (md.iK != nullptr);
    const int KP = wk.KP;
    const PairOps po = pair_ops(wk, md.D, npad, pl, b);
    const int i = ti * 256 + t;
    const bool rowok = i < npad;
    double av[KPT];
#pragma unroll
    for (int k = 0; k < KPT; ++k) av[k] = (k < KP && rowok) ? po.At[(long)k * npad + i] : 0.0;
    const int j0 = tj * 64;
    for (int e = t; e < KPT * 64; e += 256) {
        const int k = e >> 6, j = e & 63;
        Bs[k][j] = (k < KP) ? (wk.vsep ? colop_row<true>(po, npad, k) : colop_row<false>(po, npad, k))[j0 + j] : 0.0;
    }
    if (t < 64) {
        bbs[t] = md.beta[mm_beta_row(md, b) * npad + j0 + t];
        vs[t] = wk.vsep ? wk.vcol[(long)pl * npad + j0 + t] : 0.0;
    }
    __syncthreads();
    double s1 = 0.0, s2 = 0.0;
    if (rowok) {
        const double* iKrow = diag ? md.iK + (mm_ik_blk(md, a) * npad + i) * npad + j0 : nullptr;
        for (int j = 0; j < 64; ++j) {
            double e = vs[j];
#pragma unroll
            for (int k = 0; k < KPT; ++k) e = fma(av[k], Bs[k][j], e);
            const double L = exp(e);
            s1 = fma(bbs[j], L, s1);
            if (diag) s2 = fma(iKrow[j], L, s2);
        }
        s1 *= md.beta[mm_beta_row(md, a) * npad + i];
    }
    for (int off = 32; off > 0; off >>= 1) {
        s1 += __shfl_down(s1, off);
        s2 += __shfl_down(s2, off);
    }
    if (lane == 0) {
        red[2 * w] = s1;
        red[2 * w + 1] = s2;
    }
    __syncthreads();
    if (t == 0) {
        double* out = wk.pair_part + ((long)pl * wk.NT + ti * ncb + tj) * 2;
        out[0] = ((red[0] + red[2]) + red[4]) + red[6];
        out[1] = ((red[1] + red[3]) + red[5]) + red[7];
    }
}
#endif

static int pair_njb(int npad, int PL) {
    const int nb = npad / 64;
    int njb = 1;
    while (njb * 2 <= nb && nb % (njb * 2) == 0 && (long)PL * (npad / (16 * PAIR_RT)) * njb < 1536) njb *= 2;
    const char* env = getenv("PILCO_PAIR_NJB");
    if (env) {
        const int v = atoi(env);
        if (v >= 1 && v <= nb && nb % v == 0) njb = v;
    }
    return njb;
}

int mm_pair_nt(int npad, int variant, int PL) {
    if (variant == 1) return ((npad + 255) / 256) * (npad / 64);
    if (variant == 2) {
        const int nb = npad / 64;
        int njb = 1;
        while (njb * 2 <= nb && nb % (njb * 2) == 0 && njb < 4) njb *= 2;
        return (npad / (16 * PAIR_RT)) * njb;
    }
    return (npad / (16 * PAIR_RT)) * pair_njb(npad, PL);
}

void mm_pair_sk_steps(int npad, int* tdiag, int* toff) {
    const int NS = npad / 16, NTI = npad / (16 * PAIR_RT);
    *toff = NTI * NS;
    *tdiag = NTI * NS - PAIR_RT * NTI * (NTI - 1) / 2;
}

template <int KC, bool VSEP>
static int sk_capacity_of() {
    int nb = 0;
    if (hipOccupancyMaxActiveBlocksPerMultiprocessor(&nb, k_mm_pair_sk<KC, VSEP>, 256, 0) != hipSuccess || nb <= 0) nb = 2;
    return nb * device_cus() * 4;
}

int mm_pair_sk_capacity(int KP, bool vsep, bool allow_env) {
    const char* env = allow_env ? getenv("PILCO_SK_WAVES") : nullptr;
    if (env && atoi(env) >= 4) return atoi(env) / 4 * 4;
    switch (KP / 4) {
        case 1: return vsep ? sk_capacity_of<1, true>() : sk_capacity_of<1, false>();
        case 2: return vsep ? sk_capacity_of<2, true>() : sk_capacity_of<2, false>();
        case 3: return vsep ? sk_capacity_of<3, true>() : sk_capacity_of<3, false>();
        case 4: return vsep ? sk_capacity_of<4, true>() : sk_capacity_of<4, false>();
        case 5: return vsep ? sk_capacity_of<5, true>() : sk_capacity_of<5, false>();
        case 6: return vsep ? sk_capacity_of<6, true>() : sk_capacity_of<6, false>();
        case 7: return vsep ? sk_capacity_of<7, true>() : sk_capacity_of<7, false>();
        case 8: return vsep ? sk_capacity_of<8, true>() : sk_capacity_of<8, false>();
        default: return vsep ? sk_capacity_of<9, true>() : sk_capacity_of<9, false>();
    }
}

void launch_mm_pair(hipStream_t st, const MMModel& md, const MMWork& wk, int variant) {
    const int KP = wk.KP;
#ifdef PILCO_DEV
    if (variant == 1) {
        dim3 grid(((md.npad + 255) / 256) * (md.npad / 64), wk.PL);
#define PV(K_) hipLaunchKernelGGL((k_mm_pair_valu<K_>), grid, dim3(256), 0, st, md, wk)
        if (KP <= 4) PV(4);
        else if (KP <= 8) PV(8);
        else if (KP <= 12) PV(12);
        else if (KP <= 16) PV(16);
        else if (KP <= 24) PV(24);
        else PV(36);
#undef PV
        return;
    }
#endif
    if (variant == 2) {
        const int NJB = wk.NT / (md.npad / (16 * PAIR_RT));
        dim3 grid((md.npad / (16 * PAIR_RT)) * NJB, wk.PL);
#define PM(K_)                                                                                        \
    do {                                                                                              \
        if (wk.vsep) hipLaunchKernelGGL((k_mm_pair_tiled<K_, true>), grid, dim3(256), 0, st, md, wk, NJB);  \
        else hipLaunchKernelGGL((k_mm_pair_tiled<K_, false>), grid, dim3(256), 0, st, md, wk, NJB);         \
    } while (0)
        switch (KP / 4) {
            case 1: PM(1); break;
            case 2: PM(2); break;
            case 3: PM(3); break;
            case 4: PM(4); break;
            case 5: PM(5); break;
            case 6: PM(6); break;
            case 7: PM(7); break;
            case 8: PM(8); break;
            default: PM(9); break;
        }
#undef PM
        return;
    }
    dim3 grid(wk.sk_waves / 4);
#define PS(K_)                                                                                 \
    do {                                                                                       \
        if (wk.vsep) hipLaunchKernelGGL((k_mm_pair_sk<K_, true>), grid, dim3(256), 0, st, md, wk);   \
        else hipLaunchKernelGGL((k_mm_pair_sk<K_, false>), grid, dim3(256), 0, st, md, wk);          \
    } while (0)
    switch (KP / 4) {
        case 1: PS(1); break;
        case 2: PS(2); break;
        case 3: PS(3); break;
        case 4: PS(4); break;
        case 5: PS(5); break;
        case 6: PS(6); break;
        case 7: PS(7); break;
        case 8: PS(8); break;
        default: PS(9); break;
    }
#undef PS
}

__global__ void k_selftest_mfma(double* out) {
    const int lane = threadIdx.x;
    const int i = lane & 15, k = lane >> 4;
    const double a = (double)(i + 1 + 100 * k);
    const double b = (k == 0) ? (double)((lane & 15) + 1) : 0.0;
    d4 acc = {0.0, 0.0, 0.0, 0.0};
    acc = __builtin_amdgcn_mfma_f64_16x16x4f64(a, b, acc, 0, 0, 0);
    MFMA_KEEP_ALIVE(a);
    MFMA_KEEP_ALIVE(b);
    for (int r = 0; r < 4; ++r) out[lane * 4 + r] = acc[r];
}

__global__ void k_selftest_fexp(const double* tab_g, double* out) {
    __shared__ double tab[FEXP_TN];
    for (int e = threadIdx.x; e < FEXP_TN; e += blockDim.x) tab[e] = tab_g[e];
    __syncthreads();
    double worst = 0.0;
    for (int i = threadIdx.x; i < 200000; i += blockDim.x) {
        const double x = -720.0 + 1420.0 * ((double)i + 0.37) / 200000.0;
        const double ref = exp(fmax(x, -700.0));
        const double got = fexp(x, tab);
        const double rel = fabs(got - ref) / ref / (2.3e-16 + 1.2e-16 * fabs(x));
        worst = fmax(worst, rel);
    }
    for (int off = 32; off > 0; off >>= 1) worst = fmax(worst, __shfl_down(worst, off));
    if ((threadIdx.x & 63) == 0) out[threadIdx.x >> 6] = worst;
}

int mm_exp_table_size() { return FEXP_TN; }

void mm_exp_table_fill(double* tab) {
    for (int j = 0; j < FEXP_TN; ++j) {
        const double v = std::exp2((double)j / (double)FEXP_TN);
        uint64_t u;
        std::memcpy(&u, &v, 8);
        const uint32_t hi = (uint32_t)(u >> 32) - ((uint32_t)j << (20 - FEXP_TB));
        u = ((uint64_t)hi << 32) | (u & 0xffffffffull);
        std::memcpy(&tab[j], &u, 8);
    }
}

int launch_selftest_mfma(hipStream_t st, double* dbuf, double* hbuf, const double* exp_tab) {
    hipLaunchKernelGGL(k_selftest_fexp, dim3(1), dim3(256), 0, st, exp_tab, dbuf);
    if (hipMemcpyAsync(hbuf, dbuf, 4 * sizeof(double), hipMemcpyDeviceToHost, st) != hipSuccess) return -1;
    if (hipStreamSynchronize(st) != hipSuccess) return -1;
    for (int w = 0; w < 4; ++w)
        if (!(hbuf[w] < 1.0)) return 100000;
    hipLaunchKernelGGL(k_selftest_mfma, dim3(1), dim3(64), 0, st, dbuf);
    if (hipMemcpyAsync(hbuf, dbuf, 256 * sizeof(double), hipMemcpyDeviceToHost, st) != hipSuccess) return -1;
    if (hipStreamSynchronize(st) != hipSuccess) return -1;
    for (int lane = 0; lane < 64; ++lane)
        for (int r = 0; r < 4; ++r) {
            const int row = (lane >> 4) + 4 * r, col = lane & 15;
            if (hbuf[lane * 4 + r] != (double)((row + 1) * (col + 1))) return 1 + lane * 4 + r;
        }
    return 0;
}

}
```

### pilco_amd/csrc/pair_device.h

```cpp
#pragma once
#include "mm_device.h"

namespace pilco {

#ifndef PAIR_RT
#define PAIR_RT 2
#endif
#if !defined(PILCO_DEV) && defined(PAIR_ABL)
#error "PAIR_ABL is a developer experiment: build with -DPILCO_DEV (tools/ only)"
#endif
#ifndef PAIR_ABL
#define PAIR_ABL 0
#endif
#if PAIR_ABL == 2
#define PAIR_ABL_TAB(v) (1.0 + 1e-9 * (double)(__double2loint(tt[i]) & (FEXP_TN - 1)))
#else
#define PAIR_ABL_TAB(v) (v)
#endif
#if PAIR_ABL == 3
#define PAIR_ABL_MFMA(a_, b_, e_) (d4{e_[0] + a_ * b_, e_[1] - a_, e_[2] + b_, e_[3] * 0.5})
#else
#define PAIR_ABL_MFMA(a_, b_, e_) __builtin_amdgcn_mfma_f64_16x16x4f64(a_, b_, e_, 0, 0, 0)
#endif
#ifndef PAIR_PF
#define PAIR_PF 2
#endif
#ifndef PAIR_FAIR
#define PAIR_FAIR 1
#endif
#ifndef PAIR_MINW
#define PAIR_MINW 1
#endif
struct TabArrival {
    static constexpr int NV = (FEXP_TN + 255) / 256;
    double v[NV];
    double* lds;
    bool pending;
    __device__ __forceinline__ void request(const double* __restrict__ g, double* l) {
#pragma unroll
        for (int k = 0; k < NV; ++k) v[k] = (FEXP_TN % 256 == 0 || threadIdx.x + 256 * k < FEXP_TN) ? g[threadIdx.x + 256 * k] : 0.0;
        lds = l;
        pending = true;
    }
    __device__ __forceinline__ void land() {
        if (pending) {
#pragma unroll
            for (int k = 0; k < NV; ++k)
                if (FEXP_TN % 256 == 0 || threadIdx.x + 256 * k < FEXP_TN) lds[threadIdx.x + 256 * k] = v[k];
            __syncthreads();
            pending = false;
        }
    }
};
#ifndef PAIR_FAIR_LEVELS
#define PAIR_FAIR_LEVELS 4
#endif
struct WaveProgress {
    int done, total, level;
    __device__ __forceinline__ void tick(int steps) {
        done += steps;
        const int lv = (PAIR_FAIR_LEVELS - 1) - min(PAIR_FAIR_LEVELS - 1, (PAIR_FAIR_LEVELS * done) / max(total, 1));
        if (lv != level) {
            level = lv;
            if (lv == 3) __builtin_amdgcn_s_setprio(3);
            else if (lv == 2) __builtin_amdgcn_s_setprio(2);
            else if (lv == 1) __builtin_amdgcn_s_setprio(1);
            else __builtin_amdgcn_s_setprio(0);
        }
    }
};
template <int KC, bool DIAG, bool VSEP, bool FENCE = false, bool LDSOP = false, bool BTAB = true>
__device__ __forceinline__ double pair_wave(const PairOps& po, const double* __restrict__ At, const double* __restrict__ Bt,
                                            const double* __restrict__ vcol,
                                            const double* __restrict__ beta_a, const double* __restrict__ beta_b,
                                            const double* __restrict__ iKa, const double* __restrict__ tab, int npad, int i0,
                                            int jbeg, int jend, int lane, int lda = 0, int ldb = 0, int i0l = 0, TabArrival* ta = nullptr, WaveProgress* wp = nullptr) {
    constexpr int NE = 4 * PAIR_RT;
    static_assert(PAIR_PF == 2, "the column loop is unrolled over a two-slot operand ring");
    const int lr = lane >> 4, lc = lane & 15;
    double af[PAIR_RT][KC];
#pragma unroll
    for (int rt = 0; rt < PAIR_RT; ++rt)
#pragma unroll
        for (int c = 0; c < KC; ++c) {
            if (LDSOP) af[rt][c] = At[(4 * c + lr) * lda + i0l + 16 * rt + lc];
            else af[rt][c] = po.At[(long)(4 * c + lr) * npad + i0 + 16 * rt + lc];
        }
    double acc[NE];
    double bi[NE];
    unsigned ik_off[NE];
#pragma unroll
    for (int i = 0; i < NE; ++i) {
        acc[i] = 0.0;
        const int row = i0 + 16 * (i >> 2) + lr + 4 * (i & 3);
        bi[i] = beta_a[row];
        ik_off[i] = ((unsigned)(row - i0) * (unsigned)npad + (unsigned)lc) * 8u;
    }
    unsigned b_off[KC];
#pragma unroll
    for (int c = 0; c < KC; ++c) {
        b_off[c] = ((unsigned)(4 * c + lr) * (unsigned)npad + (unsigned)lc) * 8u;
        if (!VSEP && !LDSOP && 4 * c + lr == po.D + 1) b_off[c] = po.v0 - po.w0 + (unsigned)lc * 8u;
    }
    const unsigned bb_off = (unsigned)lc * 8u;
    const unsigned sB = LDSOP ? 0u : po.w0, sV = LDSOP ? 0u : po.v0;
    const __amdgpu_buffer_rsrc_t rB = buf_rsrc(LDSOP ? beta_b : po.Wt), rbeta = buf_rsrc(beta_b);
    const __amdgpu_buffer_rsrc_t rIK = buf_rsrc(DIAG ? iKa + (long)i0 * npad : beta_b);
    if (DIAG && jbeg < i0) jbeg = i0;
    double total = 0.0;
    double ring[2][KC + 2];
#pragma unroll
    for (int p = 0; p < 2; ++p) {
#pragma unroll
        for (int c = 0; c <= KC + 1; ++c) ring[p][c] = 0.0;
        if (jbeg + 16 * p < jend) {
#pragma unroll
            for (int c = 0; c < KC; ++c) {
                if (LDSOP) ring[p][c] = Bt[(4 * c + lr) * ldb + jbeg + 16 * p + lc];
                else ring[p][c] = buf_ld(rB, b_off[c], sB + (unsigned)(jbeg + 16 * p) * 8u);
            }
            ring[p][KC] = buf_ld(rbeta, bb_off, (unsigned)(jbeg + 16 * p) * 8u);
            if (VSEP) {
                if (LDSOP) ring[p][KC + 1] = vcol[jbeg + 16 * p + lc];
                else ring[p][KC + 1] = buf_ld(rB, bb_off, sV + (unsigned)(jbeg + 16 * p) * 8u);
            }
        }
    }
    if (ta) ta->land();
    auto step = [&](double (&rg)[KC + 2], const int j0) {
        double bf[KC];
#pragma unroll
        for (int c = 0; c < KC; ++c) bf[c] = rg[c];
        const double bb = rg[KC];
        const double vv = rg[KC + 1];
        double ik[NE];
        if (DIAG) {
#pragma unroll
            for (int i = 0; i < NE; ++i) ik[i] = buf_ld(rIK, ik_off[i], (unsigned)j0 * 8u);
        }
        double x[NE], tt[NE], tv[NE], pm[NE];
#pragma unroll
        for (int rt = 0; rt < PAIR_RT; ++rt) {
            d4 e = {0.0, 0.0, 0.0, 0.0};
#pragma unroll
            for (int c = 0; c < KC; ++c) e = PAIR_ABL_MFMA(af[rt][c], bf[c], e);
            MFMA_KEEP_ALIVE(af[rt][0]);
            MFMA_KEEP_ALIVE(bf[0]);
            if (FENCE) MFMA_RESULT_FENCE(e);
#pragma unroll
            for (int r = 0; r < 4; ++r) x[4 * rt + r] = VSEP ? e[r] + vv : e[r];
        }
        if (PAIR_ABL != 4 && j0 + 32 < jend) {
#pragma unroll
            for (int c = 0; c < KC; ++c) {
                if (LDSOP) rg[c] = Bt[(4 * c + lr) * ldb + j0 + 32 + lc];
                else rg[c] = buf_ld(rB, b_off[c], sB + (unsigned)(j0 + 32) * 8u);
            }
            rg[KC] = buf_ld(rbeta, bb_off, (unsigned)(j0 + 32) * 8u);
            if (VSEP) {
                if (LDSOP) rg[KC + 1] = vcol[j0 + 32 + lc];
                else rg[KC + 1] = buf_ld(rB, bb_off, sV + (unsigned)(j0 + 32) * 8u);
            }
        }
#pragma unroll
        for (int i = 0; i < NE; ++i) {
            x[i] = fexp_clamp(x[i]);
            tt[i] = fexp_t(x[i]);
        }
#pragma unroll
        for (int i = 0; i < NE; ++i) tv[i] = PAIR_ABL_TAB(tab[__double2loint(tt[i]) & (FEXP_TN - 1)]);
#if !(PAIR_OPT & 4)
        __builtin_amdgcn_sched_barrier(0);
#endif
        double rr[NE];
#pragma unroll
        for (int i = 0; i < NE; ++i) rr[i] = fma(tt[i] - FEXP_MAGIC, -FEXP_LN2_64, x[i]);
        if (FEXP_DEG == 5) {
#pragma unroll
            for (int i = 0; i < NE; ++i) pm[i] = fma(rr[i], 1.0 / 120.0, 1.0 / 24.0);
#pragma unroll
            for (int i = 0; i < NE; ++i) pm[i] = fma(rr[i], pm[i], 1.0 / 6.0);
#pragma unroll
            for (int i = 0; i < NE; ++i) pm[i] = fma(rr[i], pm[i], 0.5);
        } else if (FEXP_DEG == 4) {
#pragma unroll
            for (int i = 0; i < NE; ++i) pm[i] = fma(rr[i], 1.0 / 24.0, 1.0 / 6.0);
#pragma unroll
            for (int i = 0; i < NE; ++i) pm[i] = fma(rr[i], pm[i], 0.5);
        } else {
#pragma unroll
            for (int i = 0; i < NE; ++i) pm[i] = fma(rr[i], 1.0 / 6.0, 0.5);
        }
#pragma unroll
        for (int i = 0; i < NE; ++i) pm[i] = fma(rr[i], pm[i], 1.0);
#pragma unroll
        for (int i = 0; i < NE; ++i) pm[i] = rr[i] * pm[i];
        __builtin_amdgcn_sched_barrier(0);
#if PAIR_ABL == 1
#pragma unroll
        for (int i = 0; i < NE; ++i) { tv[i] = x[i]; pm[i] = 0.0; tt[i] = 0.0; }
#define FEXP_FINISH(a_, b_, c_) (a_)
#else
#define FEXP_FINISH(a_, b_, c_) (BTAB ? fexp_finish(a_, b_, c_) : fexp_finish_ub(a_, b_, c_))
#endif
        if (DIAG) {
            double st[4] = {0.0, 0.0, 0.0, 0.0};
#pragma unroll
            for (int i = 0; i < NE; ++i)
                st[i & 3] = fma(fma(bi[i], bb, -ik[i]), FEXP_FINISH(tv[i], pm[i], tt[i]), st[i & 3]);
            const double wgt = (j0 >= i0 + 16 * PAIR_RT) ? 2.0 : 1.0;
            total = fma(wgt, (st[0] + st[1]) + (st[2] + st[3]), total);
        } else {
#pragma unroll
            for (int i = 0; i < NE; ++i) acc[i] = fma(bb, FEXP_FINISH(tv[i], pm[i], tt[i]), acc[i]);
        }
    };
    for (int j0 = jbeg; j0 < jend; j0 += 32) {
        if (wp) wp->tick(2);
        step(ring[0], j0);
        if (j0 + 16 < jend) step(ring[1], j0 + 16);
    }
    if (!DIAG) {
#pragma unroll
        for (int i = 0; i < NE; ++i) total = fma(bi[i], acc[i], total);
    }
    return total;
}

__host__ __device__ inline long div_floor(long a, long b) {
    long q = (long)((double)a / (double)b);
    while (q * b > a) --q;
    while ((q + 1) * b <= a) ++q;
    return q;
}
__host__ __device__ inline int sk_boundary_of(int w, int waves, int nd_steps, int total, int ud, int uo) {
    const long Ud = (long)nd_steps * ud;
    const long C = Ud + (long)(total - nd_steps) * uo;
    if (w >= waves) return total;
    const long x = div_floor((long)w * C, waves);
    if (x <= Ud) return (int)div_floor(x + ud - 1, ud);
    return nd_steps + (int)div_floor(x - Ud + uo - 1, uo);
}
__host__ __device__ inline int sk_wave_of(long x, int waves, int nd_steps, int total, int ud, int uo) {
    const long Ud = (long)nd_steps * ud;
    const long C = Ud + (long)(total - nd_steps) * uo;
    const long cx = (x <= nd_steps) ? x * ud : Ud + (x - nd_steps) * uo;
    long w = div_floor((cx + 1) * waves + C - 1, C) - 1;
    if (w > waves - 1) w = waves - 1;
    return (int)w;
}
__host__ __device__ inline void sk_pair_waves(int k, int waves, int nd, int tdiag, int toff, int total, int ud, int uo,
                                              int& wlo, int& fslot, int& whi) {
    const long S0 = (k < nd) ? (long)k * tdiag : (long)nd * tdiag + (long)(k - nd) * toff;
    const long S1 = S0 + ((k < nd) ? tdiag : toff);
    const int nd_steps = nd * tdiag;
    wlo = sk_wave_of(S0, waves, nd_steps, total, ud, uo);
    fslot = sk_boundary_of(wlo, waves, nd_steps, total, ud, uo) < S0 ? 1 : 0;
    whi = sk_wave_of(S1 - 1, waves, nd_steps, total, ud, uo);
}
inline int sk_max_pairs_per_wave(int waves, int nd, int tdiag, int toff, int n_pairs, int ud, int uo) {
    const int nd_steps = nd * tdiag, total = nd_steps + (n_pairs - nd) * toff;
    auto pair_of = [&](int step) { return step < nd_steps ? step / tdiag : nd + (step - nd_steps) / toff; };
    int most = 0;
    for (int w = 0; w < waves; ++w) {
        const int b0 = sk_boundary_of(w, waves, nd_steps, total, ud, uo), b1 = sk_boundary_of(w + 1, waves, nd_steps, total, ud, uo);
        const int n = pair_of(b1 - 1) - pair_of(b0) + 1;
        if (b1 > b0 && n > most) most = n;
    }
    return most;
}
__device__ __forceinline__ int sk_boundary(const MMWork& wk, int w) {
    return sk_boundary_of(w, wk.sk_waves, wk.sk_nd * wk.sk_tdiag, wk.sk_total, wk.sk_ud, wk.sk_uo);
}
template <int KC, bool VSEP, bool FENCE = false>
__device__ __forceinline__ void sk_wave_range(const MMModel& md, const MMWork& wk, const double* __restrict__ tab, int w, int lane,
                                              double& out0, double& out1, int& p0, int& p1, TabArrival* ta = nullptr, bool fair = false) {
    const int npad = md.npad, NS = npad / 16;
    const int nd_steps = wk.sk_nd * wk.sk_tdiag;
    int step = sk_boundary(wk, w);
    const int end = sk_boundary(wk, w + 1);
    WaveProgress prog{0, end - step, -1};
    WaveProgress* wp = fair ? &prog : nullptr;
    out0 = 0.0;
    out1 = 0.0;
    p0 = -1;
    p1 = -1;
    double cur = 0.0;
    int cur_pl = -1;
    while (step < end) {
        int pl, q, ti, sidx, cnt;
        const bool dg = step < nd_steps;
        if (dg) {
            pl = step / wk.sk_tdiag;
            q = step - pl * wk.sk_tdiag;
            ti = 0;
            int c = NS;
            while (q >= c) {
                q -= c;
                ++ti;
                c -= PAIR_RT;
            }
            sidx = ti * PAIR_RT + q;
            cnt = c - q;
        } else {
            const int r = step - nd_steps;
            pl = wk.sk_nd + r / wk.sk_toff;
            q = r - (pl - wk.sk_nd) * wk.sk_toff;
            ti = q / NS;
            sidx = q - ti * NS;
            cnt = NS - sidx;
        }
        const int seg = (cnt < end - step) ? cnt : (end - step);
        if (pl != cur_pl) {
            if (cur_pl >= 0) {
                out0 = cur;
                p0 = cur_pl;
            }
            cur_pl = pl;
            cur = 0.0;
        }
        int a, b;
        local_pair_ab(wk, md.E, pl, a, b);
        const PairOps po = pair_ops(wk, md.D, npad, pl, b);
        const double* beta_a = md.beta + mm_beta_row(md, a) * npad;
        const double* beta_b = md.beta + mm_beta_row(md, b) * npad;
        const int i0 = ti * 16 * PAIR_RT, jbeg = sidx * 16, jend = jbeg + seg * 16;
        if (dg)
            cur += pair_wave<KC, true, VSEP, FENCE>(po, nullptr, nullptr, nullptr, beta_a, beta_b, md.iK + mm_ik_blk(md, a) * npad * npad, tab, npad, i0, jbeg, jend, lane, 0, 0, 0, ta, wp);
        else
            cur += pair_wave<KC, false, VSEP, FENCE>(po, nullptr, nullptr, nullptr, beta_a, beta_b, nullptr, tab, npad, i0, jbeg, jend, lane, 0, 0, 0, ta, wp);
        step += seg;
    }
    if (cur_pl >= 0) {
        if (p0 < 0) {
            out0 = cur;
            p0 = cur_pl;
        } else {
            out1 = cur;
            p1 = cur_pl;
        }
    }
}

}
```

### pilco_amd/csrc/rollout.hip

```cpp
#include "ctx.h"
#include "reward_factor.h"

namespace {

constexpr size_t GLUE_LDS_LIMIT = 160 * 1024;

int stage_rewards(pilco_ctx* ctx, const pilco_reward_term* rw, int n_rw, int E, std::vector<double>& hp, size_t& off,
                  const double* dev_base, RewardDev* out) {
    for (int i = 0; i < n_rw; ++i) {
        out[i].kind = rw[i].kind;
        out[i].coef = rw[i].coef;
        out[i].F = nullptr;
        out[i].rank = -1;
        if (!rw[i].W) return fail(ctx, PILCO_E_SHAPE, "reward: W is required");
        if (rw[i].kind == PILCO_REWARD_EXPONENTIAL) {
            hp.resize(std::max(hp.size(), off + (size_t)2 * E * E + E));
            memcpy(&hp[off], rw[i].W, sizeof(double) * E * E);
            out[i].W = dev_base + off; off += (size_t)E * E;
            if (rw[i].t) memcpy(&hp[off], rw[i].t, sizeof(double) * E);
            else std::fill(hp.begin() + off, hp.begin() + off + E, 0.0);
            out[i].t = dev_base + off; off += E;
            std::vector<double> F;
            const int r = pilco::psd_factor(rw[i].W, E, F);
            out[i].rank = r;
            if (r > 0) {
                memcpy(&hp[off], F.data(), sizeof(double) * E * r);
                out[i].F = dev_base + off;
            } else if (r == 0) {
                out[i].F = dev_base + off;
            }
            off += (size_t)E * E;
        } else if (rw[i].kind == PILCO_REWARD_LINEAR) {
            hp.resize(std::max(hp.size(), off + (size_t)E));
            memcpy(&hp[off], rw[i].W, sizeof(double) * E);
            out[i].W = dev_base + off; off += E;
            out[i].t = out[i].W;
        } else {
            return fail(ctx, PILCO_E_SHAPE, "reward: unknown kind");
        }
    }
    return PILCO_OK;
}

}

int setup_rollout(pilco_ctx* ctx, const pilco_policy* pol, const pilco_reward_term* rw, int n_rw, int H, bool want_traj,
                  RolloutPlan& plan) {
    Slot& s = ctx->slot[0];
    if (!s.factor_valid) return fail(ctx, PILCO_E_STATE, "rollout: dynamics model has no current factorisation");
    if (!s.beta_complete) return fail(ctx, PILCO_E_STATE, "rollout: beta of the other ranks is missing (attach a communicator before factorising, or pilco_group_sync_model)");
    if (s.shW != ctx->nranks || s.shRank != ctx->rank) return fail(ctx, PILCO_E_STATE, "rollout: the model was factorised under a different rank layout; factorise again");
    if (!pol) return fail(ctx, PILCO_E_SHAPE, "rollout: null policy");
    const int E = s.E, D = s.D, U = D - E;
    if (pol->state_dim != E || pol->control_dim != U || U < 0)
        return fail(ctx, PILCO_E_SHAPE, "rollout: policy dims do not match the model (state_dim must be E, control_dim D-E)");
    if (pol->kind == PILCO_POLICY_NONE && U != 0) return fail(ctx, PILCO_E_SHAPE, "rollout: policy NONE needs D == E");
    if (pol->kind == PILCO_POLICY_LINEAR && (U == 0 || !pol->W || !pol->b)) return fail(ctx, PILCO_E_SHAPE, "rollout: linear policy needs W, b and control_dim > 0");
    if (pol->kind == PILCO_POLICY_RBF) {
        Slot& ps = ctx->slot[PILCO_SLOT_POLICY];
        if (!ps.factor_valid) return fail(ctx, PILCO_E_STATE, "rollout: RBF policy slot has no current factorisation");
        if (ps.D != E || ps.E != U || U == 0) return fail(ctx, PILCO_E_SHAPE, "rollout: RBF policy GP must map state_dim -> control_dim");
        if (ctx->nranks != 1 && !(ctx->inline_policy && rbf_inline_lds_doubles(E, U, ps.n) > 0))
            return fail(ctx, PILCO_E_STATE, "rollout: with several ranks an RbfController must be small enough for the inline evaluation (pilco_set_inline_policy)");
        if (int r = build_work(ctx, ps)) return r;
    }
    if (pol->kind < 0 || pol->kind > 2) return fail(ctx, PILCO_E_SHAPE, "rollout: unknown policy kind");
    if (n_rw < 0 || n_rw > MAX_REWARD_TERMS || (n_rw > 0 && !rw)) return fail(ctx, PILCO_E_SHAPE, "rollout: 0..4 reward terms supported");
    if (int r = build_work(ctx, s)) return r;
    ctx->route.fill(0);
    ctx->route[ROUTE_ENTRY] = 1;
    const size_t n_state = 2 * ((size_t)E + E * E) + 2 * (size_t)E * D + 1 + 8;
    ENSURE(ctx->state, n_state);
    const size_t n_par = (size_t)U * E + 2 * U + (size_t)MAX_REWARD_TERMS * (2 * E * E + E) + 8;
    ENSURE(ctx->params, n_par);
    if (want_traj) ENSURE(ctx->traj, (size_t)(H + 1) * (E + E * E));
    std::vector<double> hp(n_par, 0.0);
    size_t off = 0;
    GlueArgs& g = plan.g;
    g = GlueArgs{};
    g.E = E; g.D = D; g.U = U;
    g.wk = s.wk;
    g.var = s.var.p;
    plan.st[0] = ctx->state.p;
    plan.st[1] = ctx->state.p + (E + E * E);
    g.s1 = ctx->state.p + 2 * (E + E * E);
    plan.s1b[0] = g.s1;
    plan.s1b[1] = g.s1 + (size_t)E * D;
    g.reward = g.s1 + 2 * (size_t)E * D;
    g.traj = want_traj ? ctx->traj.p : nullptr;
    g.pol_kind = pol->kind;
    g.squash = pol->squash;
    if (pol->kind == PILCO_POLICY_RBF) {
        g.pwk = ctx->slot[PILCO_SLOT_POLICY].wk;
        g.pvar = ctx->slot[PILCO_SLOT_POLICY].var.p;
        g.pmd = model_of(ctx->slot[PILCO_SLOT_POLICY]);
        g.pol_lds = rbf_inline_lds_doubles(E, U, ctx->slot[PILCO_SLOT_POLICY].n);
        for (int u = 0; u < U; ++u) hp[off + u] = pol->max_action ? pol->max_action[u] : 1.0;
        g.maxact = ctx->params.p + off; off += U;
    }
    if (pol->kind == PILCO_POLICY_LINEAR) {
        memcpy(&hp[off], pol->W, sizeof(double) * U * E);
        g.W = ctx->params.p + off; off += (size_t)U * E;
        memcpy(&hp[off], pol->b, sizeof(double) * U);
        g.b = ctx->params.p + off; off += U;
        for (int u = 0; u < U; ++u) hp[off + u] = pol->max_action ? pol->max_action[u] : 1.0;
        g.maxact = ctx->params.p + off; off += U;
    }
    g.n_rewards = n_rw;
    g.rew_out = nullptr;
    if (int r = stage_rewards(ctx, rw, n_rw, E, hp, off, ctx->params.p, g.rw)) return r;
    if (hp.size() > n_par) return fail(ctx, PILCO_E_ALLOC, "rollout: parameter staging overflow");
    if (ctx->params_dev != ctx->params.p || ctx->params_host.size() != n_par ||
        memcmp(ctx->params_host.data(), hp.data(), sizeof(double) * n_par) != 0) {
        HIPCHK(hipMemcpyAsync(ctx->params.p, hp.data(), sizeof(double) * n_par, hipMemcpyHostToDevice, ctx->st));
        HIPCHK(hipStreamSynchronize(ctx->st));
        ctx->params_host = hp;
        ctx->params_dev = ctx->params.p;
    }
    plan.E = E; plan.D = D; plan.U = U;
    return PILCO_OK;
}

static int xq_begin(pilco_ctx* ctx) {
    PeerXch& x = ctx->xq;
    unsigned long long* slot = x.pin + (x.ring++ & 127u);
    *slot = x.epoch;
    HIPCHK(hipMemcpyAsync(x.local, slot, sizeof(unsigned long long), hipMemcpyHostToDevice, ctx->st));
    return PILCO_OK;
}

static int small_col_splits(pilco_ctx* ctx, const Slot& s, bool rew) {
    if (s.npad / s.wk.NCH != 64 || s.wk.KP > 16) return 1;
    static const int forced = getenv("PILCO_SMALL_NCS") ? atoi(getenv("PILCO_SMALL_NCS")) : 0;
    const int cus = device_cus_of(ctx->device), spare = s.wk.EL * s.wk.NCHM + (rew ? 1 : 0);
    int ncs = 1;
    while (ncs * 2 <= s.wk.NCH && ncs * 2 <= 4 && s.wk.PL * s.wk.NCH * ncs * 2 + spare <= cus) ncs *= 2;
    if (forced > 0 && forced <= s.wk.NCH && (forced & (forced - 1)) == 0 && forced <= 4) ncs = forced;
    return ncs;
}

static int plan_route(pilco_ctx* ctx, RolloutPlan& plan, int H, bool timed) {
    const Slot& s = ctx->slot[0];
    const GlueArgs& g = plan.g;
    const bool rbf = g.pol_kind == PILCO_POLICY_RBF, jac = plan.jrec != nullptr;
    const bool one = ctx->nranks == 1 && !ctx->comm, steps = s.wk.PL > 0 && H > 0;
    auto fits = [&](bool inline_pol) {
        GlueArgs gl = g;
        gl.pol_inline = inline_pol ? 1 : 0;
        if (ctx->nranks > 1) {
            const int W = ctx->nranks, P = s.E * (s.E + 1) / 2;
            gl.wk.PL = (P + W - 1) / W;
            gl.wk.EL = (s.E + W - 1) / W;
            mm_prep_chunks(s.npad, std::max(gl.wk.PL, 1), gl.wk.EL, &gl.wk.NCH, &gl.wk.NCHM);
        } else if (s.wk.PL <= 0) {
            return true;
        }
        const bool rbf_k = rbf && !inline_pol;
        gl.flags = GF_TRAJ | GF_POLICY | GF_PACK | GF_ASSEMBLE | GF_PROPAGATE | (rbf_k ? (GF_RBF_PRE | GF_RBF_POST) : 0);
        const int rew_E = g.n_rewards > 0 ? plan.E : 0;
        return mm_fused_head_fits(model_of(s), rew_E, gl) &&
               (!rbf_k || mm_fused_head_fits(model_of(ctx->slot[PILCO_SLOT_POLICY]), rew_E, gl));
    };
    const bool eligible = rbf && ctx->inline_policy && g.pol_lds > 0;
    if (rbf && !one && !eligible)
        return fail(ctx, PILCO_E_STATE, "rollout: several ranks run an RbfController only with the inline policy (at most 256 basis functions, see pilco_set_inline_policy)");
    const bool inl = eligible && (!one || (ctx->fused && steps && fits(true)));
    const bool fit = fits(inl);
    StepRoute r;
    int step = STEP_THREE;
    if (one && ctx->fused && fit && steps && (!rbf || inl)) {
        step = STEP_FUSED;
        const int dt = mm_prep_dt(s.D);
        const bool small = ctx->fuse_small && !timed && !MM_ABL(s.wk, 255) && s.npad <= 256 && s.wk.KP == mm_kp(dt) &&
                           (s.wk.vsep != 0) == mm_vsep(dt) &&
                           (jac ? s.npad / s.wk.NCH == 64 && s.wk.KP <= 16 : (s.npad / s.wk.NCH) % 32 == 0 && ctx->variant == 0);
        if (small) {
            step = STEP_SMALL;
            r.ncs = small_col_splits(ctx, s, g.n_rewards > 0 && !MM_ABL(s.wk, 8));
        }
    } else if (ctx->xq.ready && ctx->nranks > 1 && ctx->xq.W == ctx->nranks && H > 0 && (!rbf || inl) && s.wk.SEG <= ctx->xq.cap &&
               !g.tape && !jac && fit) {
        step = STEP_PEER;
    } else if (one && ctx->fused && fit && rbf && steps && ctx->slot[PILCO_SLOT_POLICY].wk.PL > 0) {
        step = STEP_FUSED_RBF;
    }
    r.step = H > 0 ? step : STEP_NONE;
    r.policy = rbf ? (inl ? 1 : 2) : 0;
    r.pair = !steps ? -1 : step == STEP_SMALL ? (jac ? 5 : 3) : jac ? 4 : ctx->variant;
    r.timed = timed;
    plan.route = r;
    plan.g.pol_inline = inl ? 1 : 0;
    auto& w = ctx->route;
    w[ROUTE_STEP] = r.step;
    w[ROUTE_POLICY] = r.policy;
    w[ROUTE_DT] = mm_prep_dt(s.D);
    w[ROUTE_KP] = s.wk.KP;
    w[ROUTE_VSEP] = s.wk.vsep ? 1 : 0;
    w[ROUTE_PAIR] = r.pair;
    w[ROUTE_TAPE] = jac ? 2 : (g.tape ? 1 : 0);
    w[ROUTE_H] = H;
    w[ROUTE_NPAD] = s.npad;
    return PILCO_OK;
}

static PrepReward reward_arg(const RolloutPlan& plan, const double* m_x = nullptr) {
    PrepReward pr{};
    pr.n = plan.g.n_rewards;
    pr.E = plan.E;
    for (int i = 0; i < plan.g.n_rewards; ++i) pr.rw[i] = plan.g.rw[i];
    if (m_x) {
        pr.m_x = m_x;
        pr.s_x = m_x + plan.E;
    }
    pr.reward = plan.g.reward;
    return pr;
}
static GlueArgs head_args(const RolloutPlan& plan, const GlueArgs& g, int h, int flags) {
    GlueArgs gh = g;
    gh.step = h;
    gh.flags = flags;
    gh.m_x = plan.st[h > 0 ? (h - 1) & 1 : 0];
    gh.s_x = gh.m_x + plan.E;
    gh.m_out = h > 0 ? plan.st[h & 1] : nullptr;
    gh.s_out = h > 0 ? plan.st[h & 1] + plan.E : nullptr;
    gh.s1 = plan.s1b[(h + 1) & 1];
    gh.s1_out = plan.s1b[h & 1];
    return gh;
}
static GlueArgs closing_args(const RolloutPlan& plan, const GlueArgs& g, int H, int flags) {
    GlueArgs gf = g;
    gf.step = H;
    gf.flags = flags;
    gf.m_x = plan.st[(H - 1) & 1];
    gf.s_x = gf.m_x + plan.E;
    gf.m_out = plan.st[H & 1];
    gf.s_out = gf.m_out + plan.E;
    gf.s1 = plan.s1b[(H - 1) & 1];
    gf.s1_out = nullptr;
    return gf;
}
static int dyn_pairs(pilco_ctx* ctx, const RolloutPlan& plan, const MMModel& md, const MMWork& w, int t) {
    const Slot& s = ctx->slot[0];
    if (plan.route.timed) HIPCHK(hipEventRecord(ctx->pair_events[2 * t], ctx->st));
    if (plan.jrec)
        launch_mm_sweep(ctx->st, md, w, s.jac_rowmom.p + (size_t)t * mm_jac_rowmom_size(s.npad, s.wk.PL),
                        s.jac_cpart.p + (size_t)t * mm_jac_cpart_size(s.npad, s.wk.PL, s.wk.EL),
                        s.jac_head.p + (size_t)t * mm_jac_head_size(s.D, s.E, s.wk.PL), s.jac_np.p);
    else
        launch_mm_pair(ctx->st, md, w, ctx->variant);
    if (plan.route.timed) HIPCHK(hipEventRecord(ctx->pair_events[2 * t + 1], ctx->st));
    return PILCO_OK;
}

static int enqueue_fused(pilco_ctx* ctx, const RolloutPlan& plan, const GlueArgs& g, int H) {
    Slot& s = ctx->slot[0];
    const MMModel md = model_of(s);
    const bool small = plan.route.step == STEP_SMALL, jac = plan.jrec != nullptr, rew = g.n_rewards > 0 && !MM_ABL(s.wk, 8);
    MMWork wkb[2] = {g.wk, g.wk};
    wkb[1].pair_isdet = s.alt_isdet;
    wkb[1].mean_part = s.alt_mean;
    if (small)
        for (int k = 0; k < 2; ++k) {
            wkb[k].fuse_pair = jac ? 2 : 1;
            wkb[k].sk_waves = 0;
            wkb[k].NCS = plan.route.ncs;
            wkb[k].share_cu = ctx->share_cu;
            wkb[k].NT = g.wk.NCH * plan.route.ncs;
            wkb[k].pair_part = s.w_fpart.p + (size_t)k * std::max(g.wk.PL, 1) * g.wk.NCH * 4 * 2;
        }
    const PrepReward pr = reward_arg(plan);
    for (int h = 0; h < H; ++h) {
        GlueArgs gh = head_args(plan, g, h, GF_TRAJ | GF_POLICY | (h > 0 ? (GF_PACK | GF_ASSEMBLE | GF_PROPAGATE) : 0));
        gh.dbg_off = h > 0 ? 48 : 0;
        gh.wk = wkb[(h + 1) & 1];
        MMWork wh = wkb[h & 1];
        if (small && jac) wh.sw_gpart = s.jac_rowmom.p + (size_t)h * mm_jac_rowmom_size(s.npad, s.wk.PL);
        launch_mm_prep(ctx->st, md, wh, rew ? &pr : nullptr, &gh);
        if (!small)
            if (int r = dyn_pairs(ctx, plan, md, wkb[h & 1], h)) return r;
    }
    GlueArgs gf = closing_args(plan, g, H, GF_PACK | GF_ASSEMBLE | GF_PROPAGATE | GF_TRAJ);
    gf.wk = wkb[(H - 1) & 1];
    launch_glue(ctx->st, gf);
    return PILCO_OK;
}

static int enqueue_peer(pilco_ctx* ctx, const RolloutPlan& plan, const GlueArgs& g, int H) {
    Slot& s = ctx->slot[0];
    const MMModel md = model_of(s);
    const bool rew = g.n_rewards > 0 && !MM_ABL(s.wk, 8);
    PeerXch& x = ctx->xq;
    {
        hipStreamCaptureStatus cs = hipStreamCaptureStatusNone;
        HIPCHK(hipStreamIsCapturing(ctx->st, &cs));
        if (cs == hipStreamCaptureStatusNone) {
            if (int r = xq_begin(ctx)) return r;
            x.epoch += (unsigned long long)H;
        }
    }
    const int spin = 2000000;
    PeerGroup* lockstep = (x.wait_kernel && ctx->group) ? ctx->group.get() : nullptr;
    auto with_xq = [&](GlueArgs& ga, int k) {
        ga.xq = x.local;
        ga.xq_k = k;
        ga.xq_W = x.W;
        ga.xq_cap = x.cap;
        ga.xq_spin = x.wait_kernel ? 1000 : spin;
    };
    const PrepReward pr = reward_arg(plan);
    for (int h = 0; h < H; ++h) {
        GlueArgs gh = head_args(plan, g, h, GF_TRAJ | GF_POLICY | (h > 0 ? (GF_ASSEMBLE | GF_PROPAGATE) : 0));
        gh.wk = s.wk;
        if (h > 0) {
            with_xq(gh, h - 1);
            if (x.wait_kernel) launch_peer_wait(ctx->st, x.local, h - 1, x.W, spin);
        }
        if (s.wk.PL > 0) {
            launch_mm_prep(ctx->st, md, s.wk, rew ? &pr : nullptr, &gh);
            if (int r = dyn_pairs(ctx, plan, md, s.wk, h)) return r;
        } else {
            launch_glue(ctx->st, gh, rew && h > 0);
        }
        GlueArgs gp = g;
        gp.step = h + 1;
        gp.wk = s.wk;
        gp.flags = GF_PACK;
        with_xq(gp, h);
        gp.xq_peers = x.d_peers;
        launch_glue(ctx->st, gp);
        if (lockstep && !lockstep->arrive_and_wait()) return fail(ctx, PILCO_E_STATE, "rollout: another rank of the group failed");
    }
    GlueArgs gf = closing_args(plan, g, H, GF_ASSEMBLE | GF_PROPAGATE | GF_TRAJ);
    gf.wk = s.wk;
    with_xq(gf, H - 1);
    if (x.wait_kernel) launch_peer_wait(ctx->st, x.local, H - 1, x.W, spin);
    launch_glue(ctx->st, gf, rew && s.wk.PL == 0);
    return PILCO_OK;
}

static int enqueue_fused_rbf(pilco_ctx* ctx, const RolloutPlan& plan, const GlueArgs& g, int H) {
    Slot& s = ctx->slot[0];
    Slot& ps = ctx->slot[PILCO_SLOT_POLICY];
    const MMModel md = model_of(s), pmd = model_of(ps);
    const bool rew = g.n_rewards > 0 && !MM_ABL(s.wk, 8);
    const PrepReward pr = reward_arg(plan);
    for (int h = 0; h < H; ++h) {
        GlueArgs ga = head_args(plan, g, h, GF_TRAJ | GF_RBF_PRE | (h > 0 ? (GF_PACK | GF_ASSEMBLE | GF_PROPAGATE) : 0));
        ga.dbg_off = h > 0 ? 48 : 0;
        ga.s1 = g.s1;
        ga.s1_out = g.s1_out;
        launch_mm_prep(ctx->st, pmd, ps.wk, rew ? &pr : nullptr, &ga);
        launch_mm_pair(ctx->st, pmd, ps.wk, ctx->variant);
        GlueArgs gc = g;
        gc.step = h;
        gc.flags = GF_RBF_POST | GF_POLICY;
        gc.m_x = plan.st[h & 1];
        gc.s_x = gc.m_x + plan.E;
        gc.m_out = nullptr;
        gc.s_out = nullptr;
        launch_mm_prep(ctx->st, md, s.wk, nullptr, &gc);
        if (int r = dyn_pairs(ctx, plan, md, s.wk, h)) return r;
    }
    GlueArgs gf = closing_args(plan, g, H, GF_PACK | GF_ASSEMBLE | GF_PROPAGATE | GF_TRAJ);
    gf.s1 = g.s1;
    launch_glue(ctx->st, gf);
    return PILCO_OK;
}

static int enqueue_three_kernel(pilco_ctx* ctx, const RolloutPlan& plan, GlueArgs g, int H) {
    Slot& s = ctx->slot[0];
    Slot& ps = ctx->slot[PILCO_SLOT_POLICY];
    const bool rbf = g.pol_kind == PILCO_POLICY_RBF, rew = g.n_rewards > 0 && !MM_ABL(s.wk, 8);
    const MMModel md = model_of(s), pmd = rbf ? model_of(ps) : MMModel{};
    auto policy_stage = [&](GlueArgs& ga) {
        launch_mm_prep(ctx->st, pmd, ps.wk);
        launch_mm_pair(ctx->st, pmd, ps.wk, ctx->variant);
        const int keep = ga.flags;
        ga.flags = GF_RBF_POST | GF_POLICY;
        launch_glue(ctx->st, ga);
        ga.flags = keep;
    };
    const bool rbf_l = rbf && !g.pol_inline;
    g.flags = GF_TRAJ | (H > 0 ? (rbf_l ? GF_RBF_PRE : GF_POLICY) : 0);
    launch_glue(ctx->st, g);
    if (rbf_l && H > 0) policy_stage(g);
    for (int t = 0; t < H; ++t) {
        if (s.wk.PL > 0) {
            const PrepReward pr = reward_arg(plan, plan.st[t & 1]);
            launch_mm_prep(ctx->st, md, s.wk, rew ? &pr : nullptr);
            if (ctx->dbg && MM_ABL(s.wk, 64)) launch_stamp(ctx->st, ctx->dbg, 30);
            if (int r = dyn_pairs(ctx, plan, md, s.wk, t)) return r;
        }
        g.step = t + 1;
        g.m_x = plan.st[t & 1];
        g.s_x = plan.st[t & 1] + plan.E;
        g.m_out = plan.st[(t + 1) & 1];
        g.s_out = plan.st[(t + 1) & 1] + plan.E;
        const bool more = t + 1 < H;
        const int tail = GF_ASSEMBLE | GF_PROPAGATE | GF_TRAJ | (more ? (rbf_l ? GF_RBF_PRE : GF_POLICY) : 0);
        if (ctx->nranks == 1 && !ctx->comm) {
            g.flags = GF_PACK | tail;
        } else {
            g.flags = GF_PACK;
            launch_glue(ctx->st, g);
            if (int r = all_gather_segments(ctx, s)) return r;
            g.flags = tail;
        }
        launch_glue(ctx->st, g, rew && s.wk.PL == 0);
        if (rbf_l && more) {
            g.m_x = g.m_out;
            g.s_x = g.s_out;
            policy_stage(g);
        }
    }
    return PILCO_OK;
}

static int enqueue_rollout_steps(pilco_ctx* ctx, const RolloutPlan& plan, int H) {
    Slot& s = ctx->slot[0];
    while (plan.route.timed && ctx->pair_events.size() < (size_t)2 * std::max(H, 1)) {
        hipEvent_t e;
        HIPCHK(hipEventCreate(&e));
        ctx->pair_events.push_back(e);
    }
    HIPCHK(hipMemsetAsync(plan.g.reward, 0, sizeof(double), ctx->st));
    GlueArgs g = plan.g;
    g.step = 0;
    g.m_x = plan.st[0];
    g.s_x = plan.st[0] + plan.E;
    g.m_out = nullptr;
    g.s_out = nullptr;
    if (plan.jrec) {
        g.wk.sk_waves = 0;
        g.wk.NT = mm_jac_nt(s.npad, s.wk.P, s.wk.KP);
        g.wk.pair_part = s.jac_np.p;
    }
    switch (plan.route.step) {
        case STEP_FUSED:
        case STEP_SMALL: return enqueue_fused(ctx, plan, g, H);
        case STEP_PEER: return enqueue_peer(ctx, plan, g, H);
        case STEP_FUSED_RBF: return enqueue_fused_rbf(ctx, plan, g, H);
        default: return enqueue_three_kernel(ctx, plan, g, H);
    }
}

template <class Upload>
static int run_rollout(pilco_ctx* ctx, RolloutPlan& plan, int H, Upload&& upload) {
    Slot& s = ctx->slot[0];
    if (int r = plan_route(ctx, plan, H, ctx->time_pairs)) return r;
    const StepRoute& rt = plan.route;
    const bool peer = rt.step == STEP_PEER;
    const bool sharded = (ctx->nranks != 1 || ctx->comm) && !peer;
    auto eager = [&] {
        if (int r = upload()) return r;
        return enqueue_rollout_steps(ctx, plan, H);
    };
    if (ctx->time_pairs) {
        ctx->timed_pairs = 0;
        if (int r = eager()) return r;
        ctx->timed_pairs = (s.wk.PL > 0) ? H : 0;
        return PILCO_OK;
    }
    const bool lockstep = peer && ctx->group && ctx->xq.wait_kernel;
    if (!ctx->use_graph || lockstep || (sharded && (!ctx->comm || ctx->graph_rccl_failed)) || (ctx->dbg && !getenv("PILCO_DBG_GRAPH")))
        return eager();
    const GlueArgs& g = plan.g;
    std::vector<unsigned long long> key = {
        (unsigned long long)H, (unsigned long long)g.pol_kind, (unsigned long long)g.n_rewards, (unsigned long long)g.squash,
        (unsigned long long)ctx->variant, (unsigned long long)rt.step, (unsigned long long)rt.policy, (unsigned long long)(long long)rt.pair,
        (unsigned long long)rt.ncs, (unsigned long long)(ctx->share_cu != 0), (unsigned long long)(uintptr_t)plan.st[0], (unsigned long long)(uintptr_t)g.s1,
        (unsigned long long)(uintptr_t)g.traj, (unsigned long long)(uintptr_t)g.tape, (unsigned long long)(uintptr_t)g.W, (unsigned long long)(uintptr_t)g.maxact,
        (unsigned long long)(uintptr_t)s.w_part.p, (unsigned long long)(uintptr_t)s.w_At.p, (unsigned long long)(uintptr_t)s.w_Wt.p,
        (unsigned long long)(uintptr_t)s.w_small.p, (unsigned long long)(uintptr_t)s.w_gath.p, (unsigned long long)(uintptr_t)s.w_out.p,
        (unsigned long long)(uintptr_t)s.w_in.p, (unsigned long long)(uintptr_t)s.beta.p,
        (unsigned long long)(uintptr_t)s.iK.p, (unsigned long long)s.iK_null, (unsigned long long)(uintptr_t)s.Xt.p,
        (unsigned long long)(uintptr_t)s.Zt.p, (unsigned long long)(uintptr_t)s.ls.p, (unsigned long long)s.n,
        (unsigned long long)s.wk.sk_waves, (unsigned long long)s.wk.NT, (unsigned long long)s.wk.NCH, (unsigned long long)s.wk.NCHM, (unsigned long long)s.wk.KP, (unsigned long long)s.wk.abl,
        (unsigned long long)(uintptr_t)ctx->slot[1].w_part.p, (unsigned long long)(uintptr_t)ctx->slot[1].w_At.p,
        (unsigned long long)(uintptr_t)ctx->slot[1].beta.p, (unsigned long long)(uintptr_t)ctx->slot[1].Xt.p,
        (unsigned long long)ctx->slot[1].n,
        (unsigned long long)ctx->slot[1].wk.sk_waves, (unsigned long long)(uintptr_t)ctx->slot[1].w_small.p,
        (unsigned long long)(uintptr_t)ctx->slot[1].w_in.p, (unsigned long long)(uintptr_t)ctx->slot[1].ls.p,
        (unsigned long long)(uintptr_t)ctx->xq.local, (unsigned long long)ctx->nranks, (unsigned long long)ctx->rank,
        (unsigned long long)(uintptr_t)ctx->slot[1].var.p,
        (unsigned long long)(uintptr_t)plan.jrec, (unsigned long long)plan.jstride, (unsigned long long)(uintptr_t)s.jac_rowmom.p,
        (unsigned long long)(uintptr_t)s.jac_cpart.p, (unsigned long long)(uintptr_t)s.jac_part.p, (unsigned long long)(uintptr_t)s.jac_head.p,
        (unsigned long long)(uintptr_t)s.jac_np.p};
    const Slot& ps = ctx->slot[PILCO_SLOT_POLICY];
    for (long v : {(long)s.N, (long)s.M, (long)s.n, (long)s.npad, (long)s.Npad, (long)s.D, (long)s.E, (long)plan.U, (long)s.wk.PL,
                   (long)s.wk.EL, (long)s.wk.P, (long)s.wk.sk_total, (long)s.wk.sk_nd, (long)s.ignore_iK, (long)ps.n, (long)ps.npad,
                   (long)ps.D, (long)ps.E, (long)ps.M})
        key.push_back((unsigned long long)v);
    for (int i = 0; i < g.n_rewards; ++i) {
        key.push_back((unsigned long long)g.rw[i].kind);
        key.push_back((unsigned long long)(long long)g.rw[i].rank);
        key.push_back((unsigned long long)(uintptr_t)g.rw[i].W);
        unsigned long long cbits;
        memcpy(&cbits, &g.rw[i].coef, sizeof(cbits));
        key.push_back(cbits);
    }
    size_t i = 0;
    while (i < ctx->graph_cache.size() && ctx->graph_cache[i].first != key) ++i;
    if (i == ctx->graph_cache.size()) {
        ctx->graph = nullptr;
        if (ctx->graph_cache.size() >= 4) {
            (void)hipGraphExecDestroy(ctx->graph_cache.back().second);
            ctx->graph_cache.pop_back();
        }
        if (int r = upload()) return r;
        if (int r = enqueue_rollout_steps(ctx, plan, H > 0 ? 1 : 0)) return r;
        HIPCHK(hipStreamSynchronize(ctx->st));
        hipGraph_t graph = nullptr;
        HIPCHK(hipStreamBeginCapture(ctx->st, hipStreamCaptureModeThreadLocal));
        const int rc = enqueue_rollout_steps(ctx, plan, H);
        hipError_t e = hipStreamEndCapture(ctx->st, &graph);
        auto eager_for_good = [&] {
            ctx->graph_rccl_failed = true;
            (void)hipGetLastError();
            return eager();
        };
        if (rc != PILCO_OK) {
            if (graph) (void)hipGraphDestroy(graph);
            return sharded ? eager_for_good() : rc;
        }
        if (e != hipSuccess)
            return sharded ? eager_for_good() : fail(ctx, PILCO_E_HIP, std::string("hipStreamEndCapture: ") + hipGetErrorString(e));
        e = hipGraphInstantiate(&ctx->graph, graph, nullptr, nullptr, 0);
        (void)hipGraphDestroy(graph);
        if (e != hipSuccess) {
            ctx->graph = nullptr;
            return sharded ? eager_for_good() : fail(ctx, PILCO_E_HIP, std::string("hipGraphInstantiate: ") + hipGetErrorString(e));
        }
        ctx->graph_cache.insert(ctx->graph_cache.begin(), std::make_pair(key, ctx->graph));
    } else if (i != 0) {
        std::swap(ctx->graph_cache[i], ctx->graph_cache[0]);
    }
    ctx->graph = ctx->graph_cache[0].second;
    ctx->graph_key = key;
    if (int r = upload()) return r;
    if (peer) {
        if (int r = xq_begin(ctx)) return r;
        ctx->xq.epoch += (unsigned long long)H;
    }
    HIPCHK(hipGraphLaunch(ctx->graph, ctx->st));
    return PILCO_OK;
}

int rollout_run(pilco_ctx* ctx, RolloutPlan& plan, int H, const double* m0, const double* S0) {
    auto upload = [&]() -> int {
        HIPCHK(hipMemcpyAsync(plan.st[0], m0, sizeof(double) * plan.E, hipMemcpyHostToDevice, ctx->st));
        HIPCHK(hipMemcpyAsync(plan.st[0] + plan.E, S0, sizeof(double) * plan.E * plan.E, hipMemcpyHostToDevice, ctx->st));
        return PILCO_OK;
    };
    return run_rollout(ctx, plan, H, upload);
}

struct RolloutCall {
    RolloutPlan plan;
    size_t nst = 0;
    double* pin_out = nullptr;
    bool peer = false;
};
static int rollout_begin(pilco_ctx* ctx, const pilco_policy* policy, const pilco_reward_term* rewards, int n_rewards, const double* m0,
                         const double* S0, int H, double* traj, RolloutCall& rc) {
    HIPCHK(hipSetDevice(ctx->device));
    RolloutPlan& plan = rc.plan;
    if (int r = setup_rollout(ctx, policy, rewards, n_rewards, H, traj != nullptr, plan)) return r;
    const int E = plan.E;
    const size_t nst = (size_t)E + (size_t)E * E;
    if (ctx->pin_io_cap < 2 * nst + 8) {
        if (ctx->pin_io) (void)hipHostFree(ctx->pin_io);
        ctx->pin_io = nullptr;
        ctx->pin_io_cap = 0;
        HIPCHK(hipHostMalloc((void**)&ctx->pin_io, sizeof(double) * (2 * nst + 8), hipHostMallocDefault));
        ctx->pin_io_cap = 2 * nst + 8;
    }
    double* pin_in = ctx->pin_io;
    double* pin_out = ctx->pin_io + nst;
    memcpy(pin_in, m0, sizeof(double) * E);
    memcpy(pin_in + E, S0, sizeof(double) * E * E);
    auto upload = [&]() -> int {
        HIPCHK(hipMemcpyAsync(plan.st[0], pin_in, sizeof(double) * nst, hipMemcpyHostToDevice, ctx->st));
        return PILCO_OK;
    };
    if (int r = run_rollout(ctx, plan, H, upload)) return r;
    HIPCHK(hipMemcpyAsync(pin_out, plan.st[H & 1], sizeof(double) * nst, hipMemcpyDeviceToHost, ctx->st));
    HIPCHK(hipMemcpyAsync(pin_out + nst, plan.g.reward, sizeof(double), hipMemcpyDeviceToHost, ctx->st));
    if (traj)
        HIPCHK(hipMemcpyAsync(traj, ctx->traj.p, sizeof(double) * (size_t)(H + 1) * (E + E * E), hipMemcpyDeviceToHost, ctx->st));
    rc.peer = plan.route.step == STEP_PEER;
    if (rc.peer) HIPCHK(hipMemcpyAsync(ctx->xq.pin + 128, ctx->xq.local + 1, sizeof(unsigned long long), hipMemcpyDeviceToHost, ctx->st));
    rc.nst = nst;
    rc.pin_out = pin_out;
    return PILCO_OK;
}
static int rollout_end(pilco_ctx* ctx, RolloutCall& rc, double* mH, double* SH, double* reward) {
    HIPCHK(hipSetDevice(ctx->device));
    HIPCHK(hipStreamSynchronize(ctx->st));
    HIPCHK(hipGetLastError());
    if (rc.peer && ctx->xq.pin[128] != 0ULL) {
        const unsigned long long ep = ctx->xq.pin[128];
        (void)hipMemsetAsync(ctx->xq.local + 1, 0, sizeof(unsigned long long), ctx->st);
        return fail(ctx, PILCO_E_STATE, "rollout: peer exchange " + std::to_string(ep) + " timed out on rank " + std::to_string(ctx->rank) +
                                            " (the ranks must make the same sequence of rollout calls)");
    }
    const int E = rc.plan.E;
    memcpy(mH, rc.pin_out, sizeof(double) * E);
    memcpy(SH, rc.pin_out + E, sizeof(double) * E * E);
    *reward = rc.pin_out[rc.nst];
    return PILCO_OK;
}

static int lane_sync_model(pilco_ctx* parent, pilco_ctx* lane) {
    const Slot& p = parent->slot[0];
    Slot& l = lane->slot[0];
    const bool same = l.N == p.N && l.D == p.D && l.E == p.E && l.M == p.M && l.Npad == p.Npad && l.n == p.n && l.npad == p.npad &&
                      l.iK_null == p.iK_null && l.Xt.p == p.Xt.p && l.Zt.p == p.Zt.p && l.beta.p == p.beta.p && l.iK.p == p.iK.p &&
                      l.ls.p == p.ls.p && l.var.p == p.var.p;
    l.N = p.N; l.D = p.D; l.E = p.E; l.M = p.M; l.Npad = p.Npad; l.n = p.n; l.npad = p.npad;
    l.has_data = p.has_data; l.has_hyp = p.has_hyp; l.factor_valid = p.factor_valid; l.user_factors = p.user_factors;
    l.iK_null = p.iK_null; l.ignore_iK = p.ignore_iK;
    l.shW = p.shW; l.shEL = p.shEL; l.shOwn = p.shOwn; l.shRank = p.shRank; l.beta_complete = p.beta_complete;
    l.Xt.borrow(p.Xt); l.Yt.borrow(p.Yt); l.Zt.borrow(p.Zt); l.ls.borrow(p.ls); l.var.borrow(p.var); l.noise.borrow(p.noise);
    l.beta.borrow(p.beta); l.iK.borrow(p.iK);
    lane->variant = parent->variant;
    lane->fused = parent->fused;
    lane->use_graph = parent->use_graph;
    lane->fuse_small = parent->fuse_small;
    lane->inline_policy = parent->inline_policy;
    lane->grad_mode = parent->grad_mode;
    lane->dev_chain = parent->dev_chain;
    if (!same) {
        l.wk_valid = false;
        for (auto& ge : lane->graph_cache) (void)hipGraphExecDestroy(ge.second);
        lane->graph_cache.clear();
        lane->graph = nullptr;
    }
    return PILCO_OK;
}

int rollout_lanes(pilco_ctx* ctx, int B, std::vector<pilco_ctx*>& lane, const char* who) {
    while ((int)ctx->lanes.size() < B - 1) {
        pilco_ctx* l = nullptr;
        if (int r = pilco_ctx_create(ctx->device, &l)) return fail(ctx, r, std::string(who) + ": could not create a lane context");
        l->is_lane = true;
        ctx->lanes.push_back(l);
    }
    lane.resize((size_t)B);
    for (int i = 0; i < B; ++i) {
        lane[i] = i == 0 ? ctx : ctx->lanes[i - 1];
        lane[i]->share_cu = B > 1 ? 1 : 0;
        if (i > 0) {
            HIPCHK(hipStreamSynchronize(lane[i]->st));
            if (int r = lane_sync_model(ctx, lane[i])) return r;
        }
    }
    HIPCHK(hipStreamSynchronize(ctx->st));
    return PILCO_OK;
}

void rollout_lanes_done(pilco_ctx* ctx) { ctx->share_cu = 0; }

extern "C" {

int pilco_rollout(pilco_ctx* ctx, const pilco_policy* policy, const pilco_reward_term* rewards, int n_rewards,
                  const double* m0, const double* S0, int H, double* mH, double* SH, double* reward, double* traj) {
    if (!ctx) return PILCO_E_SHAPE;
    if (!m0 || !S0 || !mH || !SH || !reward || H < 0) return fail(ctx, PILCO_E_SHAPE, "rollout: bad arguments");
    RolloutCall rc;
    if (int r = rollout_begin(ctx, policy, rewards, n_rewards, m0, S0, H, traj, rc)) return r;
    return rollout_end(ctx, rc, mH, SH, reward);
}

int pilco_rollout_batch(pilco_ctx* ctx, int B, const pilco_policy* policies, const pilco_reward_term* rewards, int n_rewards,
                        const double* m0, const double* S0, int H, double* mH, double* SH, double* reward) {
    if (!ctx) return PILCO_E_SHAPE;
    if (B <= 0 || B > 64 || !policies || !m0 || !S0 || !mH || !SH || !reward || H < 0) return fail(ctx, PILCO_E_SHAPE, "rollout_batch: bad arguments");
    if (ctx->nranks != 1 || ctx->comm) return fail(ctx, PILCO_E_STATE, "rollout_batch: single rank only (shard OR batch)");
    for (int i = 0; i < B; ++i)
        if (policies[i].kind == PILCO_POLICY_RBF) return fail(ctx, PILCO_E_SHAPE, "rollout_batch: RbfController lanes are not supported (one policy GP slot per context)");
    HIPCHK(hipSetDevice(ctx->device));
    const Slot& s = ctx->slot[0];
    if (!s.factor_valid) return fail(ctx, PILCO_E_STATE, "rollout_batch: dynamics model has no current factorisation");
    const int E = s.E;
    std::vector<RolloutCall> rc((size_t)B);
    std::vector<pilco_ctx*> lane;
    LanesGuard lanes_guard{ctx};
    if (int r = rollout_lanes(ctx, B, lane, "rollout_batch")) return r;
    return run_lanes(
        ctx, lane, false,
        [&](int i) { return rollout_begin(lane[i], &policies[i], rewards, n_rewards, m0 + (size_t)i * E, S0 + (size_t)i * E * E, H, nullptr, rc[i]); },
        [&](int i) { return rollout_end(lane[i], rc[i], mH + (size_t)i * E, SH + (size_t)i * E * E, reward + i); });
}

int pilco_propagate(pilco_ctx* ctx, const pilco_policy* policy, const double* m_x, const double* s_x, double* M_x, double* S_x) {
    double r = 0.0;
    return pilco_rollout(ctx, policy, nullptr, 0, m_x, s_x, 1, M_x, S_x, &r, nullptr);
}

int pilco_policy_action(pilco_ctx* ctx, const pilco_policy* policy, const double* m, const double* s_in, double* M, double* S, double* V) {
    if (!ctx) return PILCO_E_SHAPE;
    if (!policy || !m || !s_in || !M || !S || !V) return fail(ctx, PILCO_E_SHAPE, "policy_action: null pointer");
    if (policy->kind != PILCO_POLICY_LINEAR && policy->kind != PILCO_POLICY_RBF) return fail(ctx, PILCO_E_SHAPE, "policy_action: policy kind must be LINEAR or RBF");
    HIPCHK(hipSetDevice(ctx->device));
    const int E = policy->state_dim, U = policy->control_dim;
    if (E <= 0 || U <= 0 || E > MAX_D || U > MAX_D) return fail(ctx, PILCO_E_SHAPE, "policy_action: bad dims");
    if (policy->kind == PILCO_POLICY_RBF) {
        Slot& ps = ctx->slot[PILCO_SLOT_POLICY];
        if (!ps.factor_valid) return fail(ctx, PILCO_E_STATE, "policy_action: RBF policy slot has no current factorisation");
        if (ps.D != E || ps.E != U) return fail(ctx, PILCO_E_SHAPE, "policy_action: RBF policy GP must map state_dim -> control_dim");
        if (int r = build_work(ctx, ps)) return r;
        const size_t n_st = (size_t)E + E * E + U + (U + U * U + (size_t)E * U);
        ENSURE(ctx->state, n_st + 8);
        std::vector<double> h(n_st, 0.0);
        memcpy(&h[0], m, sizeof(double) * E);
        memcpy(&h[E], s_in, sizeof(double) * E * E);
        size_t off = (size_t)E + E * E;
        GlueArgs g{};
        g.E = E; g.D = E + U; g.U = U;
        g.m_x = ctx->state.p;
        g.s_x = ctx->state.p + E;
        for (int u = 0; u < U; ++u) h[off + u] = policy->max_action ? policy->max_action[u] : 1.0;
        g.maxact = ctx->state.p + off; off += U;
        g.act_out = ctx->state.p + off;
        g.pol_kind = PILCO_POLICY_RBF;
        g.squash = policy->squash;
        g.pwk = ps.wk;
        g.pvar = ps.var.p;
        g.flags = GF_RBF_POST | GF_POLICY;
        if (sizeof(double) * glue_lds_doubles_for(g) > GLUE_LDS_LIMIT) return fail(ctx, PILCO_E_SHAPE, "policy_action: state_dim + control_dim too large for the link's LDS");
        HIPCHK(hipMemcpyAsync(ctx->state.p, h.data(), sizeof(double) * n_st, hipMemcpyHostToDevice, ctx->st));
        HIPCHK(hipMemcpyAsync(ps.wk.in_m, m, sizeof(double) * E, hipMemcpyHostToDevice, ctx->st));
        HIPCHK(hipMemcpyAsync(ps.wk.in_s, s_in, sizeof(double) * E * E, hipMemcpyHostToDevice, ctx->st));
        const MMModel pmd = model_of(ps);
        launch_mm_prep(ctx->st, pmd, ps.wk);
        launch_mm_pair(ctx->st, pmd, ps.wk, ctx->variant);
        launch_glue(ctx->st, g);
        std::vector<double> o((size_t)U + U * U + (size_t)E * U);
        HIPCHK(hipMemcpyAsync(o.data(), g.act_out, sizeof(double) * o.size(), hipMemcpyDeviceToHost, ctx->st));
        HIPCHK(hipStreamSynchronize(ctx->st));
        HIPCHK(hipGetLastError());
        memcpy(M, &o[0], sizeof(double) * U);
        memcpy(S, &o[U], sizeof(double) * U * U);
        memcpy(V, &o[(size_t)U + U * U], sizeof(double) * E * U);
        return PILCO_OK;
    }
    if (!policy->W || !policy->b) return fail(ctx, PILCO_E_SHAPE, "policy_action: linear policy needs W and b");
    if (glue_lds_bytes(E, E + U) > GLUE_LDS_LIMIT) return fail(ctx, PILCO_E_SHAPE, "policy_action: state_dim + control_dim too large for the link's LDS");
    const size_t n_state = (size_t)E + E * E + (size_t)U * E + 2 * U + (U + U * U + (size_t)E * U);
    ENSURE(ctx->state, n_state + 8);
    std::vector<double> h(n_state, 0.0);
    memcpy(&h[0], m, sizeof(double) * E);
    memcpy(&h[E], s_in, sizeof(double) * E * E);
    size_t off = (size_t)E + E * E;
    GlueArgs g{};
    g.E = E; g.D = E + U; g.U = U;
    g.m_x = ctx->state.p;
    g.s_x = g.m_x + E;
    memcpy(&h[off], policy->W, sizeof(double) * U * E);
    g.W = ctx->state.p + off; off += (size_t)U * E;
    memcpy(&h[off], policy->b, sizeof(double) * U);
    g.b = ctx->state.p + off; off += U;
    for (int u = 0; u < U; ++u) h[off + u] = policy->max_action ? policy->max_action[u] : 1.0;
    g.maxact = ctx->state.p + off; off += U;
    g.act_out = ctx->state.p + off;
    g.pol_kind = PILCO_POLICY_LINEAR;
    g.squash = policy->squash;
    g.flags = GF_POLICY;
    HIPCHK(hipMemcpyAsync(ctx->state.p, h.data(), sizeof(double) * n_state, hipMemcpyHostToDevice, ctx->st));
    launch_glue(ctx->st, g);
    std::vector<double> o((size_t)U + U * U + (size_t)E * U);
    HIPCHK(hipMemcpyAsync(o.data(), g.act_out, sizeof(double) * o.size(), hipMemcpyDeviceToHost, ctx->st));
    HIPCHK(hipStreamSynchronize(ctx->st));
    HIPCHK(hipGetLastError());
    memcpy(M, &o[0], sizeof(double) * U);
    memcpy(S, &o[U], sizeof(double) * U * U);
    memcpy(V, &o[(size_t)U + U * U], sizeof(double) * E * U);
    return PILCO_OK;
}

int pilco_reward_eval(pilco_ctx* ctx, const pilco_reward_term* rewards, int n_rewards, int state_dim, const double* m,
                      const double* s_in, double* muR, double* sR) {
    if (!ctx) return PILCO_E_SHAPE;
    if (!rewards || n_rewards <= 0 || n_rewards > MAX_REWARD_TERMS || !m || !s_in || !muR || !sR || state_dim <= 0 || state_dim > MAX_D)
        return fail(ctx, PILCO_E_SHAPE, "reward_eval: bad arguments");
    HIPCHK(hipSetDevice(ctx->device));
    const int E = state_dim;
    const size_t n = (size_t)E + E * E + (size_t)n_rewards * (2 * E * E + E) + 2;
    ENSURE(ctx->state, n + 8);
    std::vector<double> h(n, 0.0);
    memcpy(&h[0], m, sizeof(double) * E);
    memcpy(&h[E], s_in, sizeof(double) * E * E);
    size_t off = (size_t)E + E * E;
    GlueArgs g{};
    g.E = E; g.D = E; g.U = 0;
    g.m_x = ctx->state.p;
    g.s_x = ctx->state.p + E;
    g.n_rewards = n_rewards;
    if (int r = stage_rewards(ctx, rewards, n_rewards, E, h, off, ctx->state.p, g.rw)) return r;
    if (h.size() < off + 2) h.resize(off + 2, 0.0);
    if (h.size() + 8 > ctx->state.cap) return fail(ctx, PILCO_E_ALLOC, "reward_eval: staging overflow");
    g.rew_out = ctx->state.p + off;
    g.flags = 0;
    HIPCHK(hipMemcpyAsync(ctx->state.p, h.data(), sizeof(double) * h.size(), hipMemcpyHostToDevice, ctx->st));
    launch_glue(ctx->st, g, true);
    double o[2];
    HIPCHK(hipMemcpyAsync(o, g.rew_out, sizeof(double) * 2, hipMemcpyDeviceToHost, ctx->st));
    HIPCHK(hipStreamSynchronize(ctx->st));
    HIPCHK(hipGetLastError());
    *muR = o[0];
    *sR = o[1];
    return PILCO_OK;
}

int pilco_rollout_timed(pilco_ctx* ctx, const pilco_policy* policy, const pilco_reward_term* rewards, int n_rewards,
                        const double* m0, const double* S0, int H, int reps, double* mH, double* SH, double* reward,
                        float* ms_total, float* ms_pair, int* n_pair_launches) {
    if (!ctx) return PILCO_E_SHAPE;
    if (!m0 || !S0 || !mH || !SH || !reward || H < 0 || reps <= 0 || !ms_total) return fail(ctx, PILCO_E_SHAPE, "rollout_timed: bad arguments");
    HIPCHK(hipSetDevice(ctx->device));
    RolloutPlan plan;
    if (int r = setup_rollout(ctx, policy, rewards, n_rewards, H, false, plan)) return r;
    const int E = plan.E;
    ENSURE(ctx->selftest, (size_t)E + E * E + 256);
    double* init = ctx->selftest.p + 256;
    HIPCHK(hipMemcpyAsync(init, m0, sizeof(double) * E, hipMemcpyHostToDevice, ctx->st));
    HIPCHK(hipMemcpyAsync(init + E, S0, sizeof(double) * E * E, hipMemcpyHostToDevice, ctx->st));
    HIPCHK(hipStreamSynchronize(ctx->st));
    auto upload = [&]() -> int {
        HIPCHK(hipMemcpyAsync(plan.st[0], init, sizeof(double) * (E + E * E), hipMemcpyDeviceToDevice, ctx->st));
        return PILCO_OK;
    };
    if (int r = run_rollout(ctx, plan, H, upload)) return r;
    HIPCHK(hipStreamSynchronize(ctx->st));
    HIPCHK(hipEventRecord(ctx->ev0, ctx->st));
    for (int rep = 0; rep < reps; ++rep)
        if (int r = run_rollout(ctx, plan, H, upload)) return r;
    HIPCHK(hipEventRecord(ctx->ev1, ctx->st));
    HIPCHK(hipEventSynchronize(ctx->ev1));
    HIPCHK(hipEventElapsedTime(ms_total, ctx->ev0, ctx->ev1));
    if (ms_pair) {
        if (int r = upload()) return r;
        if (int r = plan_route(ctx, plan, H, true)) return r;
        if (int r = enqueue_rollout_steps(ctx, plan, H)) return r;
        HIPCHK(hipStreamSynchronize(ctx->st));
        float tot = 0.f;
        int cnt = 0;
        if (ctx->slot[0].wk.PL > 0)
            for (int t = 0; t < H; ++t) {
                float ms = 0.f;
                HIPCHK(hipEventElapsedTime(&ms, ctx->pair_events[2 * t], ctx->pair_events[2 * t + 1]));
                tot += ms;
                ++cnt;
            }
        *ms_pair = tot;
        if (n_pair_launches) *n_pair_launches = cnt;
    }
    HIPCHK(hipMemcpyAsync(mH, plan.st[H & 1], sizeof(double) * E, hipMemcpyDeviceToHost, ctx->st));
    HIPCHK(hipMemcpyAsync(SH, plan.st[H & 1] + E, sizeof(double) * E * E, hipMemcpyDeviceToHost, ctx->st));
    HIPCHK(hipMemcpyAsync(reward, plan.g.reward, sizeof(double), hipMemcpyDeviceToHost, ctx->st));
    HIPCHK(hipStreamSynchronize(ctx->st));
    HIPCHK(hipGetLastError());
    return PILCO_OK;
}

int pilco_rollout_tape(pilco_ctx* ctx, const pilco_policy* policy, const pilco_reward_term* rewards, int n_rewards,
                       const double* m0, const double* S0, int H, double* mH, double* SH, double* reward, double* traj,
                       double* tape) {
    if (!ctx) return PILCO_E_SHAPE;
    if (!m0 || !S0 || !mH || !SH || !reward || !tape || H < 0) return fail(ctx, PILCO_E_SHAPE, "rollout_tape: bad arguments");
    HIPCHK(hipSetDevice(ctx->device));
    RolloutPlan plan;
    if (int r = setup_rollout(ctx, policy, rewards, n_rewards, H, traj != nullptr, plan)) return r;
    const int E = plan.E;
    const size_t TS = tape_rec(plan.D, E).size;
    ENSURE(ctx->tape, std::max<size_t>(1, (size_t)H * TS));
    plan.g.tape = ctx->tape.p;
    if (int r = rollout_run(ctx, plan, H, m0, S0)) return r;
    HIPCHK(hipMemcpyAsync(mH, plan.st[H & 1], sizeof(double) * E, hipMemcpyDeviceToHost, ctx->st));
    HIPCHK(hipMemcpyAsync(SH, plan.st[H & 1] + E, sizeof(double) * E * E, hipMemcpyDeviceToHost, ctx->st));
    HIPCHK(hipMemcpyAsync(reward, plan.g.reward, sizeof(double), hipMemcpyDeviceToHost, ctx->st));
    if (traj) HIPCHK(hipMemcpyAsync(traj, ctx->traj.p, sizeof(double) * (size_t)(H + 1) * (E + E * E), hipMemcpyDeviceToHost, ctx->st));
    if (H > 0) HIPCHK(hipMemcpyAsync(tape, ctx->tape.p, sizeof(double) * (size_t)H * TS, hipMemcpyDeviceToHost, ctx->st));
    HIPCHK(hipStreamSynchronize(ctx->st));
    HIPCHK(hipGetLastError());
    return PILCO_OK;
}

}

int pilco_debug_geometry(pilco_ctx* ctx, int* out, int n) {
    if (!ctx || !out || n <= 0) return PILCO_E_SHAPE;
    Slot& s = ctx->slot[PILCO_SLOT_DYNAMICS];
    if (!s.wk_valid) return fail(ctx, PILCO_E_STATE, "debug_geometry: the dynamics slot has no step workspace (run a rollout first)");
    const MMWork& wk = s.wk;
    const int sk_cap = (ctx->variant == 0 && wk.PL > 0) ? mm_pair_sk_capacity(wk.KP, wk.vsep != 0, false) : 0;
    const int v[PILCO_GEOMETRY_WORDS] = {s.npad, wk.PL, wk.EL, wk.NCH, wk.NCHM, wk.NT, wk.sk_waves, wk.sk_total, wk.sk_nd, wk.sk_maxw,
                                         sk_cap, device_cus_of(ctx->device), small_col_splits(ctx, s, true), small_col_splits(ctx, s, false)};
    for (int i = 0; i < std::min(n, (int)PILCO_GEOMETRY_WORDS); ++i) out[i] = v[i];
    return PILCO_OK;
}
```

Before: 422.1 rollouts/s.

## Write rollout results to pinned host memory from glue kernel; magic-division stream-K decode

The final glue kernel now writes the closing mean, covariance and reward straight into the pinned host output buffer, which removes two device-to-host copies after each rollout on the fused and small step routes. Separately, the stream-K pair kernel's wave-boundary and step decoding now uses precomputed magic-number division, closed-form sqrt tile lookup and pair indexing. These values are passed in the kernel arguments and reread from them. A debug probe kernel and Python binding are added to inspect the cut. Writing to host memory from a kernel depends on visibility at stream synchronisation, and the float-sqrt paths need correction steps to stay exact.

```diff
diff --git a/include/pilco_hip_dev.h b/include/pilco_hip_dev.h
--- a/include/pilco_hip_dev.h
+++ b/include/pilco_hip_dev.h
@@ -40,6 +40,9 @@
 int pilco_debug_poison(pilco_ctx* ctx, int slot, int which);
 int pilco_debug_sk_boundary(int w, int waves, int nd, int tdiag, int toff, int ud, int uo, int n_pairs);
 int pilco_debug_sk_pair_waves(int k, int waves, int nd, int tdiag, int toff, int ud, int uo, int n_pairs, int* out3);
+#define PILCO_SK_PROBE_HEAD 10
+#define PILCO_SK_PROBE_WORDS 9
+int pilco_debug_sk_cut_probe(pilco_ctx* ctx, int* out, int n);
 int pilco_factorize_timed(pilco_ctx* ctx, int slot, int reps, float* ms_each);
 
 #ifdef __cplusplus
diff --git a/pilco_amd/_lib.py b/pilco_amd/_lib.py
--- a/pilco_amd/_lib.py
+++ b/pilco_amd/_lib.py
@@ -128,6 +128,7 @@
     "pilco_debug_buffer": (C.c_int, [_vp, C.c_int, C.c_int, _dp, C.c_long]),
     "pilco_debug_sk_boundary": (C.c_int, [C.c_int] * 8),
     "pilco_debug_sk_pair_waves": (C.c_int, [C.c_int] * 8 + [C.POINTER(C.c_int)]),
+    "pilco_debug_sk_cut_probe": (C.c_int, [_vp, C.POINTER(C.c_int), C.c_int]),
     "pilco_comm_unique_id": (C.c_int, [_vp]),
     "pilco_comm_init": (C.c_int, [_vp, _vp, C.c_int, C.c_int]),
     "pilco_shard_set": (C.c_int, [_vp, C.c_int, C.c_int]),
@@ -707,6 +708,18 @@
         self._chk(self.lib.pilco_debug_geometry(self.h, buf, len(buf)))
         return {name: int(buf[i]) for i, name in enumerate(self.GEOMETRY_FIELDS)}
 
+    SK_PROBE_HEAD = ("waves", "nd", "tdiag", "toff", "total", "ud", "uo", "PL", "fast", "npad")
+    SK_PROBE_WORDS = ("begin", "end", "pl", "ti", "sidx", "cnt", "slot", "a", "b")
+
+    def sk_cut_probe(self):
+        g = self.geometry()
+        n = len(self.SK_PROBE_HEAD) + max(g["sk_waves"], 0) * len(self.SK_PROBE_WORDS)
+        buf = (C.c_int * n)()
+        self._chk(self.lib.pilco_debug_sk_cut_probe(self.h, buf, n))
+        a = np.ctypeslib.as_array(buf).copy()
+        head = {name: int(a[i]) for i, name in enumerate(self.SK_PROBE_HEAD)}
+        return head, a[len(self.SK_PROBE_HEAD):].reshape(head["waves"], len(self.SK_PROBE_WORDS))
+
     def debug_blocks(self, n):
         buf = (C.c_ulonglong * n)()
         self._chk(self.lib.pilco_debug_blocks(self.h, buf, n))
diff --git a/pilco_amd/csrc/api.hip b/pilco_amd/csrc/api.hip
--- a/pilco_amd/csrc/api.hip
+++ b/pilco_amd/csrc/api.hip
@@ -54,6 +54,7 @@
     wk.sk_waves = 0;
     wk.sk_maxw = 0;
     wk.sk_pls = 0;
+    wk.skm = SkMagic{};
     if (ctx->variant == 0 && wk.PL > 0) {
         int tdiag, toff;
         mm_pair_sk_steps(npad, &tdiag, &toff);
@@ -84,6 +85,7 @@
         wk.sk_toff = toff;
         wk.sk_ud = ud;
         wk.sk_uo = uo;
+        wk.skm = mm_sk_magic(wk, npad);
         wk.sk_maxw = mm_sk_maxw(wk);
         wk.sk_pls = round_up(wk.PL, 16);
     }
diff --git a/pilco_amd/csrc/ctx.h b/pilco_amd/csrc/ctx.h
--- a/pilco_amd/csrc/ctx.h
+++ b/pilco_amd/csrc/ctx.h
@@ -248,6 +248,7 @@
     double* jrec = nullptr;
     size_t jstride = 0;
     StepRoute route;
+    double* host_out = nullptr;
 };
 int rollout_run(pilco_ctx* ctx, RolloutPlan& plan, int H, const double* m0, const double* S0);
 enum GradChain {
diff --git a/pilco_amd/csrc/glue.hip b/pilco_amd/csrc/glue.hip
--- a/pilco_amd/csrc/glue.hip
+++ b/pilco_amd/csrc/glue.hip
@@ -30,9 +30,9 @@
     hipLaunchKernelGGL(k_const_rows, dim3((npad + 255) / 256, nb), dim3(256), 0, st, a_row, nA, b_row, nB, bs, npad, n);
 }
 
-__global__ __launch_bounds__(256) void k_glue(GlueArgs g) {
+__global__ __launch_bounds__(256) void k_glue(GlueArgs g, double* host_out) {
     extern __shared__ __attribute__((aligned(16))) double sm[];
-    kernarg_warm<(int)sizeof(GlueArgs) + 64>();
+    kernarg_warm<(int)sizeof(GlueArgs) + 8 + 64>();
     const int E = g.E, t = threadIdx.x;
     GlueLds L;
     glue_lds_carve(g, sm, L);
@@ -56,6 +56,12 @@
         return;
     }
     glue_body(g, L, true);
+    if (host_out) {
+        __syncthreads();
+        if (t < E) host_out[t] = L.mx[t];
+        for (int e = t; e < E * E; e += blockDim.x) host_out[E + e] = L.sx[e];
+        if (t == 0) host_out[E + E * E] = g.reward[0];
+    }
 }
 
 __global__ void k_stamp(unsigned long long* dbg, int slot) {
@@ -65,8 +71,8 @@
     hipLaunchKernelGGL(k_stamp, dim3(1), dim3(64), 0, st, dbg, slot);
 }
 
-void launch_glue(hipStream_t st, const GlueArgs& g, bool with_reward_block) {
-    launch_lds<k_glue>(dim3(with_reward_block ? 2 : 1), dim3(256), sizeof(double) * glue_lds_doubles_for(g), st, g);
+void launch_glue(hipStream_t st, const GlueArgs& g, bool with_reward_block, double* host_out) {
+    launch_lds<k_glue>(dim3(with_reward_block ? 2 : 1), dim3(256), sizeof(double) * glue_lds_doubles_for(g), st, g, host_out);
 }
 
 }
diff --git a/pilco_amd/csrc/moment.h b/pilco_amd/csrc/moment.h
--- a/pilco_amd/csrc/moment.h
+++ b/pilco_amd/csrc/moment.h
@@ -20,6 +20,26 @@
     const double* iK;
     int n, npad, D, E;
     int bW, bEL;
+};
+
+struct SkMagic {
+    unsigned fast;
+    unsigned cq, cr;
+    unsigned Ud;
+    unsigned m_waves, m_ud, m_uo, m_tdiag, m_toff, m_ns;
+    unsigned m_inv;
+    unsigned sh0;
+    unsigned sh1;
+    unsigned pad_[3];
+};
+static_assert(sizeof(SkMagic) == 64, "SkMagic is one 64-byte line of the kernel arguments");
+struct SkCut {
+    unsigned fast;
+    int waves, total, nd, tdiag, toff, ud, uo;
+    unsigned cq, cr, Ud;
+    unsigned nd_steps;
+    unsigned ns;
+    unsigned m_waves, m_ud, m_uo, m_tdiag, m_toff, m_ns, m_inv, sh0, sh1;
 };
 
 struct MMWork {
@@ -49,6 +69,7 @@
     int NCS;
     const double* exp_tab;
     int PL, EL, P, KP, NCH, NCHM, NT, SEG, OUTOFF, rank, nranks;
+    SkMagic skm;
 };
 
 struct RewardDev {
@@ -131,10 +152,12 @@
 int mm_pair_sk_capacity(int KP, bool vsep, bool allow_env = true);
 void mm_pair_sk_steps(int npad, int* tdiag, int* toff);
 int mm_sk_boundary(int w, int waves, int nd_steps, int total, int ud, int uo);
+void launch_sk_cut_probe(hipStream_t st, const MMModel& md, const MMWork& wk, int* out);
+SkMagic mm_sk_magic(const MMWork& wk, int npad);
 int mm_sk_maxw(const MMWork& wk);
 int mm_sk_max_pairs(int waves, int nd, int tdiag, int toff, int n_pairs, int ud, int uo);
 void mm_sk_pair_waves(int k, int waves, int nd, int tdiag, int toff, int total, int ud, int uo, int* wlo, int* fslot, int* whi);
-void launch_glue(hipStream_t st, const GlueArgs& g, bool with_reward_block = false);
+void launch_glue(hipStream_t st, const GlueArgs& g, bool with_reward_block = false, double* host_out = nullptr);
 size_t glue_lds_bytes(int E, int D);
 int mm_pair_nt(int npad, int variant, int PL);
 void mm_prep_chunks(int npad, int PL, int EL, int* nch, int* nchm);
diff --git a/pilco_amd/csrc/pair.hip b/pilco_amd/csrc/pair.hip
--- a/pilco_amd/csrc/pair.hip
+++ b/pilco_amd/csrc/pair.hip
@@ -48,6 +48,9 @@
 int mm_sk_boundary(int w, int waves, int nd_steps, int total, int ud, int uo) {
     return sk_boundary_of(w, waves, nd_steps, total, ud, uo);
 }
+SkMagic mm_sk_magic(const MMWork& wk, int npad) {
+    return sk_magic_of(sk_cut_make(wk.sk_waves, wk.sk_nd, wk.sk_tdiag, wk.sk_toff, wk.sk_total, wk.sk_ud, wk.sk_uo, npad));
+}
 int mm_sk_max_pairs(int waves, int nd, int tdiag, int toff, int n_pairs, int ud, int uo) {
     return sk_max_pairs_per_wave(waves, nd, tdiag, toff, n_pairs, ud, uo);
 }
@@ -62,6 +65,7 @@
     TabArrival ta;
     ta.request(wk.exp_tab, tab);
     const int lane = threadIdx.x & 63;
+    const SkArgPtr skp = sk_cut_argptr();
     int bpos = blockIdx.x;
     if ((gridDim.x & 7) == 0) bpos = (blockIdx.x & 7) * (gridDim.x >> 3) + (blockIdx.x >> 3);
     const int w = __builtin_amdgcn_readfirstlane(bpos * 4 + (threadIdx.x >> 6));
@@ -75,22 +79,21 @@
     }
 #endif
     DBG_STAMP(wk, 16, w == 0 && lane == 0);
+#ifdef PAIR_START_STAMP
+    DBG_STAMP(wk, 38, w == wk.sk_waves - 1 && lane == 0);
+    if (wk.dbg && lane == 0) ta.stamp = (w == 0) ? wk.dbg + 46 : (w == wk.sk_waves - 1) ? wk.dbg + 39 : nullptr;
+#endif
     if (wk.dbg && w == 0 && lane == 0) wk.dbg[32] = clock64();
-    const int nd_steps = wk.sk_nd * wk.sk_tdiag;
     double out0, out1;
     int p0, p1;
-    sk_wave_range<KC, VSEP>(md, wk, tab, w, lane, out0, out1, p0, p1, &ta, PAIR_FAIR != 0);
+    sk_wave_range<KC, VSEP>(md, wk, skp, tab, w, lane, out0, out1, p0, p1, &ta, PAIR_FAIR != 0);
     ta.land();
     for (int off = 32; off > 0; off >>= 1) {
         out0 += __shfl_down(out0, off);
         out1 += __shfl_down(out1, off);
     }
     if (lane == 0) {
-        if (p0 >= 0) {
-            const long S0 = (p0 < wk.sk_nd) ? (long)p0 * wk.sk_tdiag : (long)wk.sk_nd * wk.sk_tdiag + (long)(p0 - wk.sk_nd) * wk.sk_toff;
-            const int wlo = sk_wave_of(S0, wk.sk_waves, nd_steps, wk.sk_total, wk.sk_ud, wk.sk_uo);
-            wk.sk_part[(long)(w - wlo) * wk.sk_pls + p0] = out0;
-        }
+        if (p0 >= 0) wk.sk_part[(long)sk_first_slot(sk_cut_arg(skp), w, p0) * wk.sk_pls + p0] = out0;
         if (p1 >= 0) wk.sk_part[p1] = out1;
     }
     DBG_STAMP(wk, 17, w == 0 && lane == 0);
@@ -164,6 +167,33 @@
 }
 #endif
 
+__global__ __launch_bounds__(256) void k_sk_cut_probe(MMModel md, MMWork wk, int* out) {
+    const SkArgPtr skp = sk_cut_argptr();
+    const SkCut c = sk_cut_arg(skp);
+    const int w = blockIdx.x * 256 + threadIdx.x;
+    if (w >= c.waves) return;
+    int* o = out + (long)w * PILCO_SK_PROBE_WORDS;
+    const int step = sk_boundary(c, w), end = sk_boundary(c, w + 1);
+    o[0] = step;
+    o[1] = end;
+    for (int i = 2; i < PILCO_SK_PROBE_WORDS; ++i) o[i] = -1;
+    if (step >= end) return;
+    int pl, ti, sidx, cnt, a, b;
+    sk_decode(c, step, pl, ti, sidx, cnt);
+    if (c.fast) sk_pair_ab_fast(pl * wk.nranks + wk.rank, md.E, a, b);
+    else local_pair_ab(wk, md.E, pl, a, b);
+    o[2] = pl;
+    o[3] = ti;
+    o[4] = sidx;
+    o[5] = cnt;
+    o[6] = sk_first_slot(sk_cut_arg(skp), w, pl);
+    o[7] = a;
+    o[8] = b;
+}
+void launch_sk_cut_probe(hipStream_t st, const MMModel& md, const MMWork& wk, int* out) {
+    hipLaunchKernelGGL(k_sk_cut_probe, dim3((wk.sk_waves + 255) / 256), dim3(256), 0, st, md, wk, out);
+}
+
 static int pair_njb(int npad, int PL) {
     const int nb = npad / 64;
     int njb = 1;
diff --git a/pilco_amd/csrc/pair_device.h b/pilco_amd/csrc/pair_device.h
--- a/pilco_amd/csrc/pair_device.h
+++ b/pilco_amd/csrc/pair_device.h
@@ -36,11 +36,17 @@
     double v[NV];
     double* lds;
     bool pending;
+#ifdef PAIR_START_STAMP
+    unsigned long long* stamp;
+#endif
     __device__ __forceinline__ void request(const double* __restrict__ g, double* l) {
 #pragma unroll
         for (int k = 0; k < NV; ++k) v[k] = (FEXP_TN % 256 == 0 || threadIdx.x + 256 * k < FEXP_TN) ? g[threadIdx.x + 256 * k] : 0.0;
         lds = l;
         pending = true;
+#ifdef PAIR_START_STAMP
+        stamp = nullptr;
+#endif
     }
     __device__ __forceinline__ void land() {
         if (pending) {
@@ -126,6 +132,9 @@
             }
         }
     }
+#ifdef PAIR_START_STAMP
+    if (ta && ta->pending && ta->stamp) *ta->stamp = wall_clock64();
+#endif
     if (ta) ta->land();
     auto step = [&](double (&rg)[KC + 2], const int j0) {
         double bf[KC];
@@ -269,16 +278,198 @@
     }
     return most;
 }
-__device__ __forceinline__ int sk_boundary(const MMWork& wk, int w) {
-    return sk_boundary_of(w, wk.sk_waves, wk.sk_nd * wk.sk_tdiag, wk.sk_total, wk.sk_ud, wk.sk_uo);
+#ifndef SK_SQRTF
+#ifdef __HIP_DEVICE_COMPILE__
+#define SK_SQRTF(x_) __builtin_amdgcn_sqrtf(x_)
+#else
+#define SK_SQRTF(x_) sqrtf(x_)
+#endif
+#endif
+__host__ __device__ inline unsigned sk_mulhi(unsigned a, unsigned b) { return (unsigned)(((unsigned long long)a * b) >> 32); }
+__host__ __device__ inline unsigned sk_div(unsigned n, unsigned m, unsigned sh) { return sk_mulhi(n, m) >> sh; }
+inline bool sk_magic_make(unsigned d, unsigned& m, unsigned& sh) {
+    m = 0;
+    sh = 0;
+    if (d < 2 || d > (1u << 30)) return false;
+    while ((2u << sh) < d) ++sh;
+    m = (unsigned)((((unsigned long long)1 << (32 + sh)) + d - 1) / d);
+    return true;
+}
+inline SkCut sk_cut_make(int waves, int nd, int tdiag, int toff, int total, int ud, int uo, int npad) {
+    SkCut c{};
+    c.waves = waves; c.total = total; c.nd = nd; c.tdiag = tdiag; c.toff = toff; c.ud = ud; c.uo = uo;
+    const long nd_steps = (long)nd * tdiag;
+    const long Ud = nd_steps * ud;
+    const long C = Ud + ((long)total - nd_steps) * uo;
+    c.nd_steps = (unsigned)nd_steps;
+    c.ns = (unsigned)(npad / 16);
+    const SkCut slow = c;
+    if (waves < 2 || waves > 46340 || C <= 0 || C + ud + uo >= (1L << 31) || total <= 0 || npad < 32 || npad % 16) return slow;
+    {
+        const double b = (double)(npad / 16) + 0.5 * PAIR_RT;
+        if (b * b > 16777216.0 || 2.0 * PAIR_RT * (double)tdiag > 16777216.0 || npad > 8192) return slow;
+    }
+    unsigned sw, sud, suo, std_, sto, sns;
+    bool ok = sk_magic_make((unsigned)waves, c.m_waves, sw);
+    ok = sk_magic_make((unsigned)ud, c.m_ud, sud) && ok;
+    ok = sk_magic_make((unsigned)uo, c.m_uo, suo) && ok;
+    ok = sk_magic_make((unsigned)tdiag, c.m_tdiag, std_) && ok;
+    ok = sk_magic_make((unsigned)toff, c.m_toff, sto) && ok;
+    ok = sk_magic_make((unsigned)(npad / 16), c.m_ns, sns) && ok;
+    if (!ok) return slow;
+    int s = 47;
+    while (s > 0 && (((unsigned long long)waves << s) / (unsigned long long)C) >> 32) --s;
+    if (C >= (1L << s)) return slow;
+    c.m_inv = (unsigned)(((unsigned long long)waves << s) / (unsigned long long)C);
+    c.cq = (unsigned)(C / waves);
+    c.cr = (unsigned)(C % waves);
+    c.Ud = (unsigned)Ud;
+    c.sh0 = sw | sud << 8 | suo << 16 | std_ << 24;
+    c.sh1 = sto | sns << 8 | (unsigned)s << 16;
+    c.fast = 1;
+    return c;
+}
+__host__ __device__ inline unsigned sk_cost_of_wave(const SkCut& c, unsigned w) {
+    return w * c.cq + sk_div(w * c.cr, c.m_waves, c.sh0 & 255u);
+}
+__host__ __device__ inline int sk_boundary_fast(const SkCut& c, int w) {
+    if (w >= c.waves) return c.total;
+    const unsigned x = sk_cost_of_wave(c, (unsigned)w);
+    if (x <= c.Ud) return (int)sk_div(x + (unsigned)c.ud - 1u, c.m_ud, (c.sh0 >> 8) & 255u);
+    return (int)(c.nd_steps + sk_div(x - c.Ud + (unsigned)c.uo - 1u, c.m_uo, (c.sh0 >> 16) & 255u));
+}
+__host__ __device__ inline int sk_wave_of_fast(const SkCut& c, unsigned x) {
+    const int waves = c.waves;
+    const unsigned cx = (x <= c.nd_steps) ? x * (unsigned)c.ud : c.Ud + (x - c.nd_steps) * (unsigned)c.uo;
+    unsigned w = (unsigned)(((unsigned long long)(cx + 1u) * c.m_inv) >> ((c.sh1 >> 16) & 255u)) + 1u;
+    if (w > (unsigned)waves - 1u) w = (unsigned)waves - 1u;
+#pragma unroll
+    for (int i = 0; i < 3; ++i)
+        if (sk_cost_of_wave(c, w) > cx) --w;
+    return (int)w;
+}
+__host__ __device__ inline unsigned sk_pair_start(const SkCut& c, int k) {
+    return (k < c.nd) ? (unsigned)k * (unsigned)c.tdiag : c.nd_steps + (unsigned)(k - c.nd) * (unsigned)c.toff;
+}
+__host__ __device__ inline int sk_tile_start(int t, int ns) { return t * ns - PAIR_RT * (t * (t - 1) / 2); }
+__host__ __device__ inline int sk_row_tile(int q, int ns) {
+    const float b = (float)ns + 0.5f * (float)PAIR_RT;
+    const float disc = b * b - (float)(2 * PAIR_RT) * (float)q;
+    int t = (int)((b - SK_SQRTF(disc > 0.0f ? disc : 0.0f)) * (1.0f / (float)PAIR_RT));
+    if (t < 0) t = 0;
+    if (sk_tile_start(t, ns) > q) --t;
+    if (sk_tile_start(t + 1, ns) <= q) ++t;
+    return t;
+}
+__host__ __device__ inline void sk_decode_fast(const SkCut& c, int step, int& pl, int& ti, int& sidx, int& cnt) {
+    const int ns = (int)c.ns, nd = c.nd, tdiag = c.tdiag, toff = c.toff;
+    if ((unsigned)step < c.nd_steps) {
+        pl = (int)sk_div((unsigned)step, c.m_tdiag, (c.sh0 >> 24) & 255u);
+        int q = step - pl * tdiag;
+        ti = sk_row_tile(q, ns);
+        q -= sk_tile_start(ti, ns);
+        sidx = ti * PAIR_RT + q;
+        cnt = ns - PAIR_RT * ti - q;
+    } else {
+        const unsigned r = (unsigned)step - c.nd_steps;
+        const unsigned k = sk_div(r, c.m_toff, c.sh1 & 255u);
+        const unsigned q = r - k * (unsigned)toff;
+        pl = nd + (int)k;
+        ti = (int)sk_div(q, c.m_ns, (c.sh1 >> 8) & 255u);
+        sidx = (int)q - ti * ns;
+        cnt = ns - sidx;
+    }
+}
+__host__ __device__ inline void sk_decode_ref(const SkCut& g, int step, int& pl, int& ti, int& sidx, int& cnt) {
+    const int NS = (int)g.ns, nd = g.nd, tdiag = g.tdiag, toff = g.toff, nd_steps = (int)g.nd_steps;
+    int q;
+    if (step < nd_steps) {
+        pl = step / tdiag;
+        q = step - pl * tdiag;
+        ti = 0;
+        int c = NS;
+        while (q >= c) {
+            q -= c;
+            ++ti;
+            c -= PAIR_RT;
+        }
+        sidx = ti * PAIR_RT + q;
+        cnt = c - q;
+    } else {
+        const int r = step - nd_steps;
+        pl = nd + r / toff;
+        q = r - (pl - nd) * toff;
+        ti = q / NS;
+        sidx = q - ti * NS;
+        cnt = NS - sidx;
+    }
+}
+__host__ __device__ inline void sk_pair_ab_fast(int kk, int E, int& a, int& b) {
+    if (kk < E) {
+        a = b = kk;
+        return;
+    }
+    const int q = kk - E;
+    int t = (int)((1.0f + SK_SQRTF((float)(8 * q + 1))) * 0.5f);
+    if (t < 1) t = 1;
+    if (t * (t - 1) / 2 > q) --t;
+    if ((t + 1) * t / 2 <= q) ++t;
+    a = t;
+    b = q - t * (t - 1) / 2;
+}
+inline SkMagic sk_magic_of(const SkCut& c) {
+    SkMagic m{};
+    m.fast = c.fast; m.cq = c.cq; m.cr = c.cr; m.Ud = c.Ud; m.m_waves = c.m_waves; m.m_ud = c.m_ud; m.m_uo = c.m_uo;
+    m.m_tdiag = c.m_tdiag; m.m_toff = c.m_toff; m.m_ns = c.m_ns; m.m_inv = c.m_inv; m.sh0 = c.sh0; m.sh1 = c.sh1;
+    return m;
+}
+typedef const __attribute__((address_space(4))) char* SkArgPtr;
+__device__ __forceinline__ SkArgPtr sk_cut_argptr() { return (SkArgPtr)__builtin_amdgcn_kernarg_segment_ptr(); }
+__device__ __forceinline__ SkCut sk_cut_arg(SkArgPtr ka) {
+    asm volatile("" : "+s"(ka));
+    typedef const __attribute__((address_space(4))) int* IP;
+    typedef const __attribute__((address_space(4))) unsigned* UP;
+    static_assert(std::is_standard_layout<MMModel>::value && std::is_standard_layout<MMWork>::value, "offsetof into the argument segment");
+    static_assert(std::is_trivially_copyable<MMModel>::value && std::is_trivially_copyable<MMWork>::value, "passed by value, bit for bit");
+    static_assert(alignof(MMModel) == 8 && alignof(MMWork) == 8, "the second parameter starts at round_up(sizeof(MMModel), 8)");
+    static_assert(sizeof(MMWork) - (offsetof(MMWork, skm) + sizeof(SkMagic)) < alignof(MMWork) && offsetof(MMWork, skm) % 4 == 0, "SkMagic is the last block of MMWork");
+    static_assert(sizeof(((MMWork*)nullptr)->sk_waves) == 4 && sizeof(((MMModel*)nullptr)->npad) == 4, "read as 32-bit words");
+    constexpr size_t WK = (sizeof(MMModel) + alignof(MMWork) - 1) / alignof(MMWork) * alignof(MMWork);
+    SkCut c;
+    c.waves = *(IP)(ka + WK + offsetof(MMWork, sk_waves));
+    c.total = *(IP)(ka + WK + offsetof(MMWork, sk_total));
+    c.nd = *(IP)(ka + WK + offsetof(MMWork, sk_nd));
+    c.tdiag = *(IP)(ka + WK + offsetof(MMWork, sk_tdiag));
+    c.toff = *(IP)(ka + WK + offsetof(MMWork, sk_toff));
+    c.ud = *(IP)(ka + WK + offsetof(MMWork, sk_ud));
+    c.uo = *(IP)(ka + WK + offsetof(MMWork, sk_uo));
+    c.ns = (unsigned)(*(IP)(ka + offsetof(MMModel, npad))) >> 4;
+    c.nd_steps = (unsigned)(c.nd * c.tdiag);
+    const UP m = (UP)(ka + WK + offsetof(MMWork, skm));
+    c.fast = m[0]; c.cq = m[1]; c.cr = m[2]; c.Ud = m[3]; c.m_waves = m[4]; c.m_ud = m[5]; c.m_uo = m[6];
+    c.m_tdiag = m[7]; c.m_toff = m[8]; c.m_ns = m[9]; c.m_inv = m[10]; c.sh0 = m[11]; c.sh1 = m[12];
+    return c;
+}
+__host__ __device__ inline int sk_boundary(const SkCut& c, int w) {
+    if (c.fast) return sk_boundary_fast(c, w);
+    return sk_boundary_of(w, c.waves, (int)c.nd_steps, c.total, c.ud, c.uo);
+}
+__host__ __device__ inline void sk_decode(const SkCut& c, int step, int& pl, int& ti, int& sidx, int& cnt) {
+    if (c.fast) sk_decode_fast(c, step, pl, ti, sidx, cnt);
+    else sk_decode_ref(c, step, pl, ti, sidx, cnt);
+}
+__host__ __device__ inline int sk_first_slot(const SkCut& c, int w, int p0) {
+    if (c.fast) return w - sk_wave_of_fast(c, sk_pair_start(c, p0));
+    const long S0 = (p0 < c.nd) ? (long)p0 * c.tdiag : (long)c.nd * c.tdiag + (long)(p0 - c.nd) * c.toff;
+    return w - sk_wave_of(S0, c.waves, (int)c.nd_steps, c.total, c.ud, c.uo);
 }
 template <int KC, bool VSEP, bool FENCE = false>
-__device__ __forceinline__ void sk_wave_range(const MMModel& md, const MMWork& wk, const double* __restrict__ tab, int w, int lane,
+__device__ __forceinline__ void sk_wave_range(const MMModel& md, const MMWork& wk, SkArgPtr skp, const double* __restrict__ tab, int w, int lane,
                                               double& out0, double& out1, int& p0, int& p1, TabArrival* ta = nullptr, bool fair = false) {
-    const int npad = md.npad, NS = npad / 16;
-    const int nd_steps = wk.sk_nd * wk.sk_tdiag;
-    int step = sk_boundary(wk, w);
-    const int end = sk_boundary(wk, w + 1);
+    const int npad = md.npad;
+    SkCut c = sk_cut_arg(skp);
+    int step = sk_boundary(c, w);
+    const int end = sk_boundary(c, w + 1);
     WaveProgress prog{0, end - step, -1};
     WaveProgress* wp = fair ? &prog : nullptr;
     out0 = 0.0;
@@ -288,28 +479,9 @@
     double cur = 0.0;
     int cur_pl = -1;
     while (step < end) {
-        int pl, q, ti, sidx, cnt;
-        const bool dg = step < nd_steps;
-        if (dg) {
-            pl = step / wk.sk_tdiag;
-            q = step - pl * wk.sk_tdiag;
-            ti = 0;
-            int c = NS;
-            while (q >= c) {
-                q -= c;
-                ++ti;
-                c -= PAIR_RT;
-            }
-            sidx = ti * PAIR_RT + q;
-            cnt = c - q;
-        } else {
-            const int r = step - nd_steps;
-            pl = wk.sk_nd + r / wk.sk_toff;
-            q = r - (pl - wk.sk_nd) * wk.sk_toff;
-            ti = q / NS;
-            sidx = q - ti * NS;
-            cnt = NS - sidx;
-        }
+        int pl, ti, sidx, cnt;
+        const bool dg = step < (int)c.nd_steps;
+        sk_decode(c, step, pl, ti, sidx, cnt);
         const int seg = (cnt < end - step) ? cnt : (end - step);
         if (pl != cur_pl) {
             if (cur_pl >= 0) {
@@ -320,7 +492,8 @@
             cur = 0.0;
         }
         int a, b;
-        local_pair_ab(wk, md.E, pl, a, b);
+        if (c.fast) sk_pair_ab_fast(pl * wk.nranks + wk.rank, md.E, a, b);
+        else local_pair_ab(wk, md.E, pl, a, b);
         const PairOps po = pair_ops(wk, md.D, npad, pl, b);
         const double* beta_a = md.beta + mm_beta_row(md, a) * npad;
         const double* beta_b = md.beta + mm_beta_row(md, b) * npad;
@@ -330,6 +503,7 @@
         else
             cur += pair_wave<KC, false, VSEP, FENCE>(po, nullptr, nullptr, nullptr, beta_a, beta_b, nullptr, tab, npad, i0, jbeg, jend, lane, 0, 0, 0, ta, wp);
         step += seg;
+        if (step < end) c = sk_cut_arg(skp);
     }
     if (cur_pl >= 0) {
         if (p0 < 0) {
diff --git a/pilco_amd/csrc/rollout.hip b/pilco_amd/csrc/rollout.hip
--- a/pilco_amd/csrc/rollout.hip
+++ b/pilco_amd/csrc/rollout.hip
@@ -203,6 +203,10 @@
     return PILCO_OK;
 }
 
+static bool results_to_host(const RolloutPlan& plan, int H) {
+    return H > 0 && plan.host_out && (plan.route.step == STEP_FUSED || plan.route.step == STEP_SMALL);
+}
+
 static PrepReward reward_arg(const RolloutPlan& plan, const double* m_x = nullptr) {
     PrepReward pr{};
     pr.n = plan.g.n_rewards;
@@ -281,7 +285,7 @@
     }
     GlueArgs gf = closing_args(plan, g, H, GF_PACK | GF_ASSEMBLE | GF_PROPAGATE | GF_TRAJ);
     gf.wk = wkb[(H - 1) & 1];
-    launch_glue(ctx->st, gf);
+    launch_glue(ctx->st, gf, false, results_to_host(plan, H) ? plan.host_out : nullptr);
     return PILCO_OK;
 }
 
@@ -485,7 +489,7 @@
         (unsigned long long)(uintptr_t)ctx->slot[1].var.p,
         (unsigned long long)(uintptr_t)plan.jrec, (unsigned long long)plan.jstride, (unsigned long long)(uintptr_t)s.jac_rowmom.p,
         (unsigned long long)(uintptr_t)s.jac_cpart.p, (unsigned long long)(uintptr_t)s.jac_part.p, (unsigned long long)(uintptr_t)s.jac_head.p,
-        (unsigned long long)(uintptr_t)s.jac_np.p};
+        (unsigned long long)(uintptr_t)s.jac_np.p, (unsigned long long)(uintptr_t)plan.host_out};
     const Slot& ps = ctx->slot[PILCO_SLOT_POLICY];
     for (long v : {(long)s.N, (long)s.M, (long)s.n, (long)s.npad, (long)s.Npad, (long)s.D, (long)s.E, (long)plan.U, (long)s.wk.PL,
                    (long)s.wk.EL, (long)s.wk.P, (long)s.wk.sk_total, (long)s.wk.sk_nd, (long)s.ignore_iK, (long)ps.n, (long)ps.npad,
@@ -583,9 +587,12 @@
         HIPCHK(hipMemcpyAsync(plan.st[0], pin_in, sizeof(double) * nst, hipMemcpyHostToDevice, ctx->st));
         return PILCO_OK;
     };
+    plan.host_out = pin_out;
     if (int r = run_rollout(ctx, plan, H, upload)) return r;
-    HIPCHK(hipMemcpyAsync(pin_out, plan.st[H & 1], sizeof(double) * nst, hipMemcpyDeviceToHost, ctx->st));
-    HIPCHK(hipMemcpyAsync(pin_out + nst, plan.g.reward, sizeof(double), hipMemcpyDeviceToHost, ctx->st));
+    if (!results_to_host(plan, H)) {
+        HIPCHK(hipMemcpyAsync(pin_out, plan.st[H & 1], sizeof(double) * nst, hipMemcpyDeviceToHost, ctx->st));
+        HIPCHK(hipMemcpyAsync(pin_out + nst, plan.g.reward, sizeof(double), hipMemcpyDeviceToHost, ctx->st));
+    }
     if (traj)
         HIPCHK(hipMemcpyAsync(traj, ctx->traj.p, sizeof(double) * (size_t)(H + 1) * (E + E * E), hipMemcpyDeviceToHost, ctx->st));
     rc.peer = plan.route.step == STEP_PEER;
@@ -900,3 +907,23 @@
     for (int i = 0; i < std::min(n, (int)PILCO_GEOMETRY_WORDS); ++i) out[i] = v[i];
     return PILCO_OK;
 }
+
+int pilco_debug_sk_cut_probe(pilco_ctx* ctx, int* out, int n) {
+    if (!ctx || !out || n < PILCO_SK_PROBE_HEAD) return PILCO_E_SHAPE;
+    HIPCHK(hipSetDevice(ctx->device));
+    Slot& s = ctx->slot[PILCO_SLOT_DYNAMICS];
+    if (!s.wk_valid || s.wk.sk_waves <= 0) return fail(ctx, PILCO_E_STATE, "debug_sk_cut_probe: the dynamics slot has no stream-K cut (run a rollout with the stream-K pair kernel first)");
+    const MMWork& wk = s.wk;
+    const size_t words = (size_t)wk.sk_waves * PILCO_SK_PROBE_WORDS;
+    if ((size_t)n < PILCO_SK_PROBE_HEAD + words) return fail(ctx, PILCO_E_SHAPE, "debug_sk_cut_probe: the buffer is too small");
+    const int head[PILCO_SK_PROBE_HEAD] = {wk.sk_waves, wk.sk_nd, wk.sk_tdiag, wk.sk_toff, wk.sk_total, wk.sk_ud, wk.sk_uo, wk.PL, (int)wk.skm.fast, s.npad};
+    for (int i = 0; i < PILCO_SK_PROBE_HEAD; ++i) out[i] = head[i];
+    int* dev = nullptr;
+    HIPCHK(hipMalloc((void**)&dev, sizeof(int) * words));
+    launch_sk_cut_probe(ctx->st, model_of(s), wk, dev);
+    hipError_t e = hipMemcpyAsync(out + PILCO_SK_PROBE_HEAD, dev, sizeof(int) * words, hipMemcpyDeviceToHost, ctx->st);
+    if (e == hipSuccess) e = hipStreamSynchronize(ctx->st);
+    (void)hipFree(dev);
+    HIPCHK(e);
+    return PILCO_OK;
+}
```

Measured after the change: 430.9 rollouts/s (median of 6 runs). 2.1% higher.
